# Jim-Maar/Gaussian-Processes-after-pre-processing-with-Normalising-Flows-2

Hardware: NVIDIA B200
Metric: mAR-SCF CIFAR10 MixLogCDF fwd+logdet images/s (higher is better)
Workload: dtype f32

## Files before the change

gaussian-processes-after-pre-processing-with-normalising-flows-2_b200/_lib.py:

```python
import ctypes
import os
import re

_HERE = os.path.dirname(os.path.abspath(__file__))
LIB_PATH = os.path.join(_HERE, "libflowk.so")
HEADER_PATH = os.path.join(os.path.dirname(_HERE), "include", "flowk.h")

FLOWK_OK = 0
FLOWK_ERR_SHAPE = 1
FLOWK_ERR_ALIGN = 2
FLOWK_ERR_ARG = 3
FLOWK_ERR_CUDA_BASE = 1000

_fp = ctypes.c_void_p
_i = ctypes.c_int
_f = ctypes.c_float
_st = ctypes.c_void_p

SIGNATURES = {
    "flowk_abi_version": ([], _i),
    "flowk_error_string": ([_i], ctypes.c_char_p),
    "flowk_ldj_workspace_bytes": ([_i], ctypes.c_size_t),
    "flowk_squeeze2d": ([_fp, _fp, _i, _i, _i, _i, _i, _st], _i),
    "flowk_unsqueeze2d": ([_fp, _fp, _i, _i, _i, _i, _i, _st], _i),
    "flowk_actnorm_init": ([_fp, _fp, _fp, _i, _i, _i, _f, _f, _st], _i),
    "flowk_channel_scale": ([_fp, _fp, _fp, _fp, _fp, _fp, _fp, _fp, _i, _i, _i, _st], _i),
    "flowk_channel_mix": ([_fp, _fp, _fp, _fp, _fp, _fp, _fp, _i, _i, _i, _i, _i, _i, _st], _i),
    "flowk_affine_coupling_fwd": ([_fp, _fp, _fp, _fp, _fp, _fp, _i, _i, _i, _st], _i),
    "flowk_affine_coupling_inv": ([_fp, _fp, _fp, _fp, _fp, _fp, _i, _i, _i, _st], _i),
    "flowk_affine_coupling_bwd": ([_fp, _fp, _fp, _fp, _fp, _fp, _i, _i, _i, _st], _i),
    "flowk_mixlogcdf_fwd": ([_fp, _fp, _fp, _fp, _fp, _fp, _fp, _i, _i, _i, _i, _i, _st], _i),
    "flowk_mixlogcdf_inv": ([_fp, _fp, _fp, _fp, _fp, _fp, _fp, _i, _i, _i, _i, _i, _st], _i),
    "flowk_mixlogcdf_bwd": ([_fp, _fp, _fp, _fp, _fp, _fp, _fp, _fp, _i, _i, _i, _i, _i, _st], _i),
    "flowk_mixture_log_cdf": ([_fp, _fp, _fp, _fp, _fp, _i, _i, _i, _st], _i),
    "flowk_mixture_log_pdf": ([_fp, _fp, _fp, _fp, _fp, _i, _i, _i, _st], _i),
    "flowk_mixture_inv_cdf": ([_fp, _fp, _fp, _fp, _fp, _i, _i, _i, _st], _i),
    "flowk_conv_gemm": ([ctypes.c_void_p, _st], _i),
    "flowk_nchw_to_nhwc_hilo": ([_fp, ctypes.c_longlong, _i, _i, _i, _i, _fp, _fp, _st], _i),
    "flowk_split_hilo": ([_fp, _fp, _fp, ctypes.c_longlong, _st], _i),
    "flowk_nchw_to_nhwc_hilo_f16": ([_fp, ctypes.c_longlong, _i, _i, _i, _i, _fp, _fp, _st], _i),
    "flowk_split_hilo_f16": ([_fp, _fp, _fp, ctypes.c_longlong, ctypes.c_float, _st], _i),
    "flowk_attention_f16": ([_fp, _fp, _fp, _i, _i, _i, _i, _st], _i),
    "flowk_std_normal_logp": ([_fp, ctypes.c_longlong, _fp, _fp, _i, ctypes.c_longlong, _st], _i),
    "flowk_pack_weight_f16": ([_fp, _fp, _i, ctypes.c_float, _fp, _fp, _i, _i, _i, _i, _fp, _fp, _fp, _st], _i),
    "flowk_fold_actnorm_invconv": ([_fp] * 7 + [_i, _i, _i, _i, _fp, _fp, _fp, _st], _i),
    "flowk_patch_attention": ([_fp, _fp, _fp, _fp, _fp, _fp, _i, _i, _i, _i, _i, _i, _st], _i),
    "flowk_patch_attention_train_fwd": ([_fp] * 7 + [_i] * 5 + [_st], _i),
    "flowk_patch_attention_bwd": ([_fp] * 8 + [_i] * 5 + [_st], _i),
    "flowk_attention_tc": ([_fp, _fp, _fp, _i, _i, _i, _i, _i, _fp, _fp, _st], _i),
    "flowk_attention_tc_v2": ([_fp, _fp, _fp, _i, _i, _i, _i, _i, _fp, _fp, _st], _i),
    "flowk_attention_tc_v2_occupancy": ([_i, _i, _i, ctypes.POINTER(ctypes.c_int), ctypes.POINTER(ctypes.c_int)], _i),
    "flowk_attention_inproj_tc": ([_fp, _fp, _fp, _fp, _f, _fp, _fp, _i, _i, _i, _i, _fp, _fp, _st], _i),
    "flowk_attention_inproj_tc_occupancy": ([_i, _i, _i, ctypes.POINTER(ctypes.c_int), ctypes.POINTER(ctypes.c_int)], _i),
    "flowk_attention": ([_fp, _fp, _fp, _i, _i, _i, _i, _st], _i),
    "flowk_concat_elu_fwd": ([_fp, _fp, _fp, ctypes.c_longlong, _i, ctypes.c_longlong, _st], _i),
    "flowk_concat_elu_bwd": ([_fp, _fp, _fp, _fp, ctypes.c_longlong, _i, ctypes.c_longlong, _st], _i),
    "flowk_glu_fwd": ([_fp, _fp, ctypes.c_longlong, _i, ctypes.c_longlong, _st], _i),
    "flowk_weight_norm_operands": ([_fp, _fp, _i, _i, _i, _i, _i, _fp, _fp, _fp, _fp, _fp, _fp, _st], _i),
    "flowk_weight_norm_operands_batched": ([_fp, _i, _i, _st], _i),
    "flowk_weight_norm_bwd": ([_fp, _fp, _fp, _fp, _fp, _fp, _i, _i, _st], _i),
    "flowk_add_layernorm_workspace_bytes": ([ctypes.c_longlong, _i], ctypes.c_longlong),
    "flowk_add_layernorm_fwd": ([_fp, _fp, _fp, _fp, _fp, _fp, _fp, _fp, ctypes.c_longlong, _i, _i, _i, _i,
                                 ctypes.c_float, _st], _i),
    "flowk_add_layernorm_bwd": ([_fp, _fp, _fp, _fp, _fp, _fp, _fp, _fp, _fp, ctypes.c_longlong, _i, _i, _i, _i, _st], _i),
    "flowk_channel_sum_workspace_bytes": ([_i], ctypes.c_longlong),
    "flowk_channel_sum": ([_fp, _fp, _fp, ctypes.c_longlong, _i, ctypes.c_longlong, _st], _i),
    "flowk_conv_wgrad_splits": ([_i, _i, _i, _i, _i, _i, ctypes.POINTER(ctypes.c_int)], _i),
    "flowk_conv_wgrad": ([_fp, _fp, _fp, _fp, _fp, _fp, _i, _i, _i, _i, _i, _i, _st], _i),
    "flowk_linear_wgrad_splits": ([ctypes.c_longlong, _i, _i, ctypes.POINTER(ctypes.c_int)], _i),
    "flowk_linear_wgrad": ([_fp, _fp, _fp, _fp, ctypes.c_longlong, _i, _i, _st], _i),
    "flowk_shift_columns": ([_fp, _fp, _fp, ctypes.c_longlong, _i, _st], _i),
    "flowk_weight_norm_bwd_partials": ([_fp, _fp, _fp, _fp, _fp, _fp, _i, _i, _i, _i, _i, _st], _i),
    "flowk_conv_gemm_splitk_slices": ([_fp], _i),
    "flowk_attention_train_fwd": ([_fp, _fp, _fp, _fp, ctypes.c_uint, ctypes.c_float, _i, _i, _i, _i, _st], _i),
    "flowk_attention_train_bwd": ([_i, _fp, _fp, _fp, _fp, _fp, _fp, ctypes.c_uint, ctypes.c_float, _i, _i, _i, _i, _st], _i),
    "flowk_attention_dropout_mask": ([_fp, ctypes.c_uint, ctypes.c_float, _i, _i, _fp, _st], _i),
    "flowk_adamax_step": ([_fp, _i, _fp, ctypes.c_float, ctypes.c_float, ctypes.c_float, _st], _i),
    "flowk_glu_bwd": ([_fp, _fp, _fp, ctypes.c_longlong, _i, ctypes.c_longlong, _st], _i),
    "flowk_mar_step": ([ctypes.c_void_p, _st], _i),
}


class ConvGemmArgs(ctypes.Structure):
    _fields_ = [(n, ctypes.c_void_p) for n in
                ("a_hi", "a_lo", "w_hi", "w_lo", "bias", "res", "gamma", "beta", "pos",
                 "out_f32", "out_hi", "out_lo", "out_nchw", "status", "trace")] + \
               [(n, ctypes.c_int) for n in ("B", "H", "W", "Cin", "N", "taps", "pre", "out_mask")] + \
               [(n, ctypes.c_void_p) for n in ("w2_hi", "w2_lo", "out2_f32")] + [("N2", ctypes.c_int)] + \
               [("splitk_ws", ctypes.c_void_p), ("operand_format", ctypes.c_int), ("acc_scale", ctypes.c_float),
                ("dilation", ctypes.c_int), ("acc_scale2", ctypes.c_float), ("acc_scale_ptr", ctypes.c_void_p)]


class MarStepArgs(ctypes.Structure):
    _fields_ = [(n, ctypes.c_void_p) for n in ("a_hi", "a_lo", "w_hi", "w_lo", "bias", "dst0_hi", "dst0_lo", "dst1_hi",
                                                "dst1_lo", "c", "noise", "z")] + \
               [("z_stride", ctypes.c_longlong), ("status", ctypes.c_void_p)] + \
               [(n, ctypes.c_int) for n in ("mode", "B", "H", "W", "Cin", "taps", "dilation", "hid", "dst0_pitch",
                                            "dst0_col", "dst1_pitch", "dst1_col")] + [("acc_scale", ctypes.c_float)]


class WnJob(ctypes.Structure):
    _fields_ = [(n, ctypes.c_void_p) for n in ("v", "g", "norm", "w", "fwd_hi", "fwd_lo", "dg_hi", "dg_lo")] + \
               [(n, ctypes.c_int) for n in ("N", "cin", "taps", "cin_pad", "n_pad", "fwd_f16")]


class AdamaxChunk(ctypes.Structure):
    _fields_ = [(n, ctypes.c_void_p) for n in ("p", "g", "m", "u")] + [("n", ctypes.c_longlong)]


OPERAND_TF32, OPERAND_F16 = 0, 1
PRE_BIAS, PRE_GLU_RES_LN, PRE_LSTM = 0, 1, 2
MAR_EMBED, MAR_LSTM, MAR_SAMPLE = 0, 1, 2
PACK_PLAIN, PACK_WEIGHT_NORM, PACK_EXP_GAIN = 0, 1, 2
OUT_F32, OUT_HILO, OUT_HILO_POS, OUT_HILO_CELU, OUT_NCHW, OUT_HILO_RELU = 1, 2, 4, 8, 16, 32


DIMS = {
    "flowk_squeeze2d": slice(2, 6), "flowk_unsqueeze2d": slice(2, 6), "flowk_actnorm_init": slice(3, 6),
    "flowk_channel_scale": slice(8, 11), "flowk_channel_mix": slice(7, 11),
    "flowk_affine_coupling_fwd": slice(6, 9), "flowk_affine_coupling_inv": slice(6, 9),
    "flowk_affine_coupling_bwd": slice(6, 9),
    "flowk_mixlogcdf_fwd": slice(7, 10), "flowk_mixlogcdf_inv": slice(7, 10), "flowk_mixlogcdf_bwd": slice(8, 11),
    "flowk_mixture_log_cdf": slice(5, 8), "flowk_mixture_log_pdf": slice(5, 8), "flowk_mixture_inv_cdf": slice(5, 8),
    "flowk_nchw_to_nhwc_hilo": slice(2, 6), "flowk_split_hilo": slice(3, 4), "flowk_attention": slice(3, 7),
    "flowk_nchw_to_nhwc_hilo_f16": slice(2, 6), "flowk_split_hilo_f16": slice(3, 4), "flowk_attention_f16": slice(3, 7),
    "flowk_attention_tc": slice(4, 8), "flowk_attention_tc_v2": slice(4, 8), "flowk_attention_inproj_tc": slice(7, 11),
    "flowk_patch_attention": slice(6, 10),
    "flowk_patch_attention_train_fwd": slice(7, 11), "flowk_patch_attention_bwd": slice(8, 12),
    "flowk_pack_weight_f16": slice(6, 10), "flowk_fold_actnorm_invconv": slice(7, 11),
}


def declared_symbols(header_path=HEADER_PATH):
    with open(header_path) as f:
        text = re.sub(r"/\*.*?\*/", "", f.read(), flags=re.S)
    return sorted(set(re.findall(r"\b(flowk_[a-z0-9_]+)\s*\(", text)))


def _load():
    if not os.path.exists(LIB_PATH):
        raise ImportError(
            "libflowk.so not found at %s - the CUDA extension is the product and there is no fallback; "
            "build it with `python __graft_entry__.py build`" % LIB_PATH)
    import torch
    lib = ctypes.CDLL(LIB_PATH)
    for name, (argtypes, restype) in SIGNATURES.items():
        fn = getattr(lib, name)
        fn.argtypes = argtypes
        fn.restype = restype
    return lib


lib = _load()

GENERATION = 0


def bump_generation():
    global GENERATION
    GENERATION += 1


def check_device(t, what="flowk"):
    import torch
    if t.is_cuda and t.device.index != torch.cuda.current_device():
        raise RuntimeError("%s: tensor lives on %s but the current CUDA device is cuda:%d; select the tensor's device "
                           "first (torch.cuda.set_device or `with torch.cuda.device(t.device)`)"
                           % (what, t.device, torch.cuda.current_device()))


ALLOW_LIBRARY = os.environ.get("FLOWK_ALLOW_LIBRARY", "0") == "1"
LIBRARY_FALLBACKS = 0


def library_fallback(what, t=None):
    global LIBRARY_FALLBACKS
    if t is not None and (not t.is_cuda or t.dtype != torch_float32()):
        return
    if not ALLOW_LIBRARY:
        raise RuntimeError("flowk: %s has no flowk kernel for this shape/mode and would fall back to a library kernel; "
                           "set FLOWK_ALLOW_LIBRARY=1 to allow it" % what)
    LIBRARY_FALLBACKS += 1


def torch_float32():
    import torch
    return torch.float32


def param_key(params):
    return (GENERATION,) + tuple((p.data_ptr(), p._version) for p in params)

LAUNCHES = 0
TIMING = None


def check(status, what=""):
    if status == FLOWK_OK:
        return
    msg = "%s: %s (flowk status %d)" % (what, lib.flowk_error_string(status).decode(), status)
    if status == FLOWK_ERR_SHAPE:
        raise AssertionError(msg)
    raise RuntimeError(msg)


def call(name, *args, meta=None):
    global LAUNCHES
    LAUNCHES += 1
    if TIMING is None:
        check(getattr(lib, name)(*args), name)
        return
    import torch
    start, end = torch.cuda.Event(enable_timing=True), torch.cuda.Event(enable_timing=True)
    start.record()
    status = getattr(lib, name)(*args)
    end.record()
    check(status, name)
    TIMING.setdefault(name, []).append((start, end, meta if meta is not None else tuple(args[DIMS.get(name, slice(0, 0))])))
```

gaussian-processes-after-pre-processing-with-normalising-flows-2_b200/csrc/attention_tc.cu:

```cuda
#include <cuda.h>
#include "common.cuh"
#include "umma.cuh"

namespace flowk {
namespace tc {

constexpr int ATT_THREADS = 512;
constexpr int ROW_B = 128;

__device__ __forceinline__ uint32_t sw_off(int r, int chunk) { return (uint32_t)(r * ROW_B + ((chunk ^ (r & 7)) << 4)); }

__device__ __forceinline__ uint32_t pack_h2(float a, float b) {
  uint32_t r;
  asm("cvt.rn.f16x2.f32 %0, %1, %2;" : "=r"(r) : "f"(b), "f"(a));
  return r;
}
__device__ __forceinline__ void unpack_h2(uint32_t v, float& a, float& b) {
  unsigned short lo16 = (unsigned short)(v & 0xffffu), hi16 = (unsigned short)(v >> 16);
  asm("cvt.f32.f16 %0, %1;" : "=f"(a) : "h"(lo16));
  asm("cvt.f32.f16 %0, %1;" : "=f"(b) : "h"(hi16));
}
__device__ __forceinline__ void cvt8(const float* v, uint4& hi, uint4& lo) {
  uint32_t h[4], l[4];
#pragma unroll
// ... 362 lines not shown
    const int kb = key >> 6, kk = key & 63;
    uint8_t* tile = v_t + (size_t)kb * vt_tile;
#pragma unroll
    for (int jj = 0; jj < 8; ++jj) {
      const int dim = ch * 8 + jj;
      unsigned short hh, ll;
      split_f16(v[jj], hh, ll);
      *reinterpret_cast<unsigned short*>(tile + sw_off(dim, kk >> 3) + ((kk & 7) << 1)) = hh;
      *reinterpret_cast<unsigned short*>(tile + sw_off(DK + dim, kk >> 3) + ((kk & 7) << 1)) = ll;
    }
  };
  if constexpr (INPROJ) {
    constexpr int STAGE_B = pj_stage_bytes(HW);
    const int nsl = p.kslices;
    const uint32_t leader = warp == 0 ? elect_one() : 0u;
    auto load_slice = [&](int ks) {
      uint8_t* st = smem + (ks & 1) * STAGE_B;
      uint64_t* bar = &bar_full[ks & 1];
      mbar_expect_tx(bar, (uint32_t)STAGE_B);
      tma_load_2d(st, &map_p_hi, bar, ks * 32, b * HW);
      tma_load_2d(st + HW * V2_ROW_B, &map_p_lo, bar, ks * 32, b * HW);
#pragma unroll
      for (int g = 0; g < 3; ++g) {
        tma_load_2d(st + 2 * HW * V2_ROW_B + g * 32 * V2_ROW_B, &map_w_hi, bar, ks * 32, g * C + h * D);
        tma_load_2d(st + 2 * HW * V2_ROW_B + PJ_W_B + g * 32 * V2_ROW_B, &map_w_lo, bar, ks * 32, g * C + h * D);
      }
    };
    if (warp == 0) {
      if (leader) {
        load_slice(0);
        if (nsl > 1) load_slice(1);
      }
      const uint32_t idesc = make_idesc_f16(PJ_N);
      for (int ks = 0; ks < nsl; ++ks) {
        mbar_wait(&bar_full[ks & 1], (uint32_t)((ks >> 1) & 1), failed);
        tc_fence_after();
        const uint8_t* st = smem + (ks & 1) * STAGE_B;
        const uint64_t dw_hi = make_smem_desc_sw64(smem_u32(st + 2 * HW * V2_ROW_B));
        const uint64_t dw_lo = make_smem_desc_sw64(smem_u32(st + 2 * HW * V2_ROW_B + PJ_W_B));
#pragma unroll
        for (int t = 0; t < tiles; ++t) {
          const uint64_t dp_hi = make_smem_desc_sw64(smem_u32(st + t * 128 * V2_ROW_B));
          const uint64_t dp_lo = make_smem_desc_sw64(smem_u32(st + (HW + t * 128) * V2_ROW_B));
          const uint32_t d = tmem_base + (uint32_t)(t * PJ_N);
#pragma unroll
          for (int k = 0; k < 2; ++k) {
            const uint64_t ko = (uint64_t)(k * 2);
            umma_elect<true>(d, dp_hi + ko, dw_hi + ko, idesc, (ks | k) == 0 ? 0u : 1u, leader);
            umma_elect<true>(d, dp_lo + ko, dw_hi + ko, idesc, 1u, leader);
            umma_elect<true>(d, dp_hi + ko, dw_lo + ko, idesc, 1u, leader);
          }
        }
        umma_commit_elect(&bar_empty[ks & 1], leader);
        if (ks >= 1 && ks + 1 < nsl) {
          mbar_wait(&bar_empty[(ks + 1) & 1], (uint32_t)(((ks - 1) >> 1) & 1), failed);
          if (leader) load_slice(ks + 1);
        }
      }
      umma_commit_elect(&bar_proj, leader);
    }
    mbar_wait(&bar_proj, 0, failed);
    tc_fence_after();
    if (tracing) p.trace[1] = clock64();
    const int lane_grp = warp & 3, ch = warp >> 2;
    const int row = lane_grp * 32 + lane;
    const uint32_t lane_addr = tmem_base + ((uint32_t)(lane_grp * 32) << 16);
    const float sc = p.acc_scale;
#pragma unroll 1
    for (int t = 0; t < tiles; ++t) {
      const uint32_t col = lane_addr + (uint32_t)(t * PJ_N + ch * 8);
      const int key = t * 128 + row;
      float v[8];
      uint4 hi, lo;
      if (ch < chunks) {
        tmem_ld8(col, v);
#pragma unroll
        for (int i = 0; i < 8; ++i) v[i] *= sc;
      } else {
#pragma unroll
        for (int i = 0; i < 8; ++i) v[i] = 0.f;
      }
      cvt8(v, hi, lo);
      *reinterpret_cast<uint4*>(k_hi + sw64_off(key, ch)) = hi;
      *reinterpret_cast<uint4*>(k_lo + sw64_off(key, ch)) = lo;
      if (ch < chunks) {
        tmem_ld8(col + 64, v);
#pragma unroll
        for (int i = 0; i < 8; ++i) v[i] = v[i] * sc * p.qscale;
      }
      cvt8(v, hi, lo);
      *reinterpret_cast<uint4*>(q_t + t * V2_QTILE_B + sw64_off(row, ch)) = hi;
      *reinterpret_cast<uint4*>(q_t + t * V2_QTILE_B + 128 * V2_ROW_B + sw64_off(row, ch)) = lo;
      if (ch < chunks) {
        tmem_ld8(col + 32, v);
#pragma unroll
        for (int i = 0; i < 8; ++i) v[i] *= sc;
      }
      store_vt(key, ch, v);
    }
    tc_fence_before();
  } else {
    const float* base = p.qkv + (size_t)b * HW * row_stride + h * D;
    const int nk = HW * KCH, total = 3 * nk;
    constexpr int MAXI = 3;
    for (int i0 = threadIdx.x; i0 < total; i0 += MAXI * V2_THREADS) {
      float4 a[MAXI], c[MAXI];
#pragma unroll
      for (int u = 0; u < MAXI; ++u) {
        const int i = i0 + u * V2_THREADS;
        a[u] = c[u] = make_float4(0.f, 0.f, 0.f, 0.f);
        if (i < total) {
          int r, ch, col;
          if (i < nk) { r = i / KCH; ch = i % KCH; col = 2 * C; }
          else if (i < 2 * nk) { r = (i - nk) / KCH; ch = (i - nk) % KCH; col = 0; }
          else { r = (i - 2 * nk) & (HW - 1); ch = (i - 2 * nk) >> hw_shift; col = C; }
          if (ch < chunks) {
            const float4* g = reinterpret_cast<const float4*>(base + (size_t)r * row_stride + col + ch * 8);
            a[u] = __ldg(g);
            c[u] = __ldg(g + 1);
          }
        }
      }
#pragma unroll
      for (int u = 0; u < MAXI; ++u) {
        const int i = i0 + u * V2_THREADS;
        if (i >= total) continue;
        if (i < 2 * nk) {
          const bool isq = i < nk;
          const int j = isq ? i : i - nk;
          const int r = j / KCH, ch = j % KCH;
          const float sc = isq ? p.qscale : 1.f;
          const float v[8] = {a[u].x * sc, a[u].y * sc, a[u].z * sc, a[u].w * sc, c[u].x * sc, c[u].y * sc, c[u].z * sc, c[u].w * sc};
          uint4 hi, lo;
          cvt8(v, hi, lo);
          uint8_t* dst_hi = isq ? q_t + (r >> 7) * V2_QTILE_B : k_hi;
          uint8_t* dst_lo = isq ? dst_hi + 128 * V2_ROW_B : k_lo;
          const int rr = isq ? (r & 127) : r;
          *reinterpret_cast<uint4*>(dst_hi + sw64_off(rr, ch)) = hi;
          *reinterpret_cast<uint4*>(dst_lo + sw64_off(rr, ch)) = lo;
        } else {
          const int j = i - 2 * nk, key = j & (HW - 1), ch = j >> hw_shift;
          const float v[8] = {a[u].x, a[u].y, a[u].z, a[u].w, c[u].x, c[u].y, c[u].z, c[u].w};
          store_vt(key, ch, v);
        }
      }
    }
  }
  fence_proxy_async();
  __syncthreads();
  if (tracing) p.trace[TR + 1] = clock64();

  const uint32_t leader = warp == 0 ? elect_one() : 0u;
  const int lane_grp = warp & 3, quarter = warp >> 2;
  const int row = lane_grp * 32 + lane;
  const uint32_t lane_addr = tmem_base + ((uint32_t)(lane_grp * 32) << 16);
  auto o_col = [&](int t, int kb) { return (uint32_t)(128 + (t * tiles + kb) * DK); };

  auto issue_s = [&](int t, int kb) {
    tc_fence_after();
    const uint32_t idesc = make_idesc_f16(128);
    const uint64_t dq_hi = make_smem_desc_sw64(smem_u32(q_t + t * V2_QTILE_B));
    const uint64_t dq_lo = make_smem_desc_sw64(smem_u32(q_t + t * V2_QTILE_B + 128 * V2_ROW_B));
    const uint64_t dk_hi = make_smem_desc_sw64(smem_u32(k_hi + kb * 128 * V2_ROW_B));
    const uint64_t dk_lo = make_smem_desc_sw64(smem_u32(k_lo + kb * 128 * V2_ROW_B));
#pragma unroll
    for (int ks = 0; ks < DK / 16; ++ks) {
      const uint64_t ko = (uint64_t)(ks * 2);
      umma_elect<true>(tmem_base, dq_hi + ko, dk_hi + ko, idesc, ks == 0 ? 0u : 1u, leader);
      umma_elect<true>(tmem_base, dq_lo + ko, dk_hi + ko, idesc, 1u, leader);
      umma_elect<true>(tmem_base, dq_hi + ko, dk_lo + ko, idesc, 1u, leader);
    }
    umma_commit_elect(&bar_s, leader);
  };

  if (warp == 0) issue_s(0, 0);
  int it = 0;
#pragma unroll 1
  for (int t = 0; t < tiles; ++t) {
    float m0 = 0.f, m1 = 0.f, l0 = 0.f, l1 = 0.f;
    for (int kb = 0; kb < tiles; ++kb, ++it) {
      mbar_wait(&bar_s, (uint32_t)(it & 1), failed);
      tc_fence_after();
      if (tracing && it == 0) p.trace[TR + 2] = clock64();
      float s[32];
      tmem_ld32(lane_addr + (uint32_t)(quarter * 32), s);
      float mx = s[0];
#pragma unroll
      for (int i = 1; i < 32; ++i) mx = fmaxf(mx, s[i]);
      red_max[quarter][row] = mx;
      tc_fence_before();
      __syncthreads();
      tc_fence_after();
      if (tracing && it == 0) p.trace[TR + 3] = clock64();
      mx = fmaxf(fmaxf(red_max[0][row], red_max[1][row]), fmaxf(red_max[2][row], red_max[3][row]));
      float sum = 0.f;
#pragma unroll
      for (int half = 0; half < 2; ++half) {
        uint32_t ph[8], pl[8];
#pragma unroll
        for (int i = 0; i < 8; ++i) {
          const float e0 = ex2_fast(s[16 * half + 2 * i] - mx), e1 = ex2_fast(s[16 * half + 2 * i + 1] - mx);
          sum += e0 + e1;
          ph[i] = pack_h2(e0, e1);
          float a0, a1;
          unpack_h2(ph[i], a0, a1);
          pl[i] = pack_h2(e0 - a0, e1 - a1);
        }
        tmem_st8u(lane_addr + (uint32_t)(quarter * 16 + half * 8), ph);
        tmem_st8u(lane_addr + (uint32_t)(64 + quarter * 16 + half * 8), pl);
      }
      red_sum[quarter][row] = sum;
      asm volatile("tcgen05.wait::st.sync.aligned;" ::: "memory");
      tc_fence_before();
      __syncthreads();
      if (tracing && it == 0) p.trace[TR + 4] = clock64();
      const float l = (red_sum[0][row] + red_sum[1][row]) + (red_sum[2][row] + red_sum[3][row]);
      if (kb == 0) { m0 = mx; l0 = l; }
      else { m1 = mx; l1 = l; }

      if (warp == 0) {
        tc_fence_after();
        const uint32_t idesc = make_idesc_f16(DK);
        const uint32_t d = tmem_base + o_col(t, kb);
#pragma unroll
        for (int j = 0; j < 8; ++j) {
          const int key = kb * 128 + j * 16;
          const uint8_t* vb = v_t + (size_t)(key >> 6) * vt_tile;
          const uint64_t ko = (uint64_t)(((key & 63) >> 4) * 2);
          const uint64_t dv_hi = make_smem_desc(smem_u32(vb)) + ko, dv_lo = make_smem_desc(smem_u32(vb + DK * ROW_B)) + ko;
          const uint32_t a_hi = tmem_base + (uint32_t)(j * 8), a_lo = tmem_base + (uint32_t)(64 + j * 8);
          umma_f16_ts_elect(d, a_hi, dv_hi, idesc, j == 0 ? 0u : 1u, leader);
          umma_f16_ts_elect(d, a_lo, dv_hi, idesc, 1u, leader);
          umma_f16_ts_elect(d, a_hi, dv_lo, idesc, 1u, leader);
        }
        umma_commit_elect(&bar_o, leader);
        const int nt = kb + 1 < tiles ? t : t + 1, nkb = kb + 1 < tiles ? kb + 1 : 0;
        if (nt < tiles) {
          mbar_wait(&bar_o, (uint32_t)(it & 1), failed);
          issue_s(nt, nkb);
        }
      }
    }
    if (tracing && t == tiles - 1) p.trace[TR + 5] = clock64();

    mbar_wait(&bar_o, (uint32_t)((it - 1) & 1), failed);
    tc_fence_after();
    float w0 = 1.f, w1 = 0.f;
    if (tiles == 2) {
      const float m = fmaxf(m0, m1);
      w0 = ex2_fast(m0 - m);
      w1 = ex2_fast(m1 - m);
    }
    const float inv = 1.0f / (l0 * w0 + l1 * w1);
    w0 *= inv;
    w1 *= inv;
    const int q0 = t * 128;
    const size_t out0 = (size_t)(cta_index() / p.heads) * HW * C + (size_t)(cta_index() % p.heads) * D;
    const size_t o0 = out0 + (size_t)(q0 + row) * C;
    uint8_t* stage = q_t + t * V2_QTILE_B;
    for (int ch = quarter; ch < chunks; ch += 4) {
      float a[8], c[8];
      tmem_ld8(lane_addr + o_col(t, 0) + ch * 8, a);
      if (tiles == 2) tmem_ld8(lane_addr + o_col(t, 1) + ch * 8, c);
      else {
#pragma unroll
        for (int i = 0; i < 8; ++i) c[i] = 0.f;
      }
#pragma unroll
      for (int i = 0; i < 8; ++i) c[i] = a[i] * w0 + c[i] * w1;
      if (p.out_f16) {
        uint4 hi, lo;
        cvt8(c, hi, lo);
        *reinterpret_cast<uint4*>(stage + ((size_t)row * chunks + ch) * 16) = hi;
        *reinterpret_cast<uint4*>(stage + ((size_t)(128 + row) * chunks + ch) * 16) = lo;
      } else {
#pragma unroll
        for (int i = 0; i < 8; i += 2) store_pair(p.out_hi, p.out_lo, o0 + ch * 8 + i, c[i], c[i + 1], 0);
      }
    }
    if (p.out_f16) {
      __syncthreads();
      const int items = 2 * 128 * chunks;
      for (int i = threadIdx.x; i < items; i += V2_THREADS) {
        const int mat = i / (128 * chunks), rr = (i / chunks) % 128, ch = i % chunks;
        const uint4 v = *reinterpret_cast<const uint4*>(stage + (size_t)i * 16);
        unsigned short* dst = reinterpret_cast<unsigned short*>(mat ? p.out_lo : p.out_hi);
        *reinterpret_cast<uint4*>(dst + out0 + (size_t)(q0 + rr) * C + ch * 8) = v;
      }
    }
  }
  tc_fence_before();
  __syncthreads();
  if (tracing) p.trace[TR + 6] = clock64();
  if (warp == 0) tmem_dealloc(tmem_base, (uint32_t)V2_TMEM_COLS);
  if (threadIdx.x == 0 && failed_flag && p.status) *p.status = 1;
}

}
}

using namespace flowk;
using namespace flowk::tc;

extern "C" int flowk_attention_tc(const float* qkv, void* out_hi, void* out_lo, int out_f16, int B, int HW, int C, int heads,
                                  int* status, long long* trace, flowk_stream_t stream) {
  if (B < 0 || HW < 1 || C < 1 || heads < 1 || C % heads) return FLOWK_ERR_SHAPE;
  const int D = C / heads;
  if ((HW != 128 && HW != 256) || D % 8 || D > 64 || C % 4) return FLOWK_ERR_SHAPE;
  if (B == 0) return FLOWK_OK;
  if (!qkv || !out_hi || !out_lo) return FLOWK_ERR_ARG;
  if ((long long)B * heads > 0x7fffffffLL) return FLOWK_ERR_SHAPE;
  AttParams p{};
  p.qkv = qkv;
  p.out_hi = reinterpret_cast<float*>(out_hi);
  p.out_lo = reinterpret_cast<float*>(out_lo);
  p.out_f16 = out_f16;
  p.HW = HW;
  p.C = C;
  p.heads = heads;
  p.D = D;
  p.dk = (D + 15) / 16 * 16;
  p.qscale = 1.4426950408889634f / sqrtf((float)D);
  p.status = status;
  p.trace = trace;
  const int p_bytes = 2 * (HW / 64) * 128 * ROW_B;
  const int qk_bytes = 2 * HW * ROW_B + 2 * HW * ROW_B;
  const int first = p_bytes > qk_bytes ? p_bytes : qk_bytes;
  p.p_off = 0;
  p.q_off = 0;
  p.k_off = 2 * HW * ROW_B;
  p.v_off = first;
  p.o_off = first + 2 * (HW / 64) * p.dk * ROW_B;
  const size_t smem = (size_t)p.o_off + (size_t)2 * 128 * (D / 8) * 16 + 1024;
  if (smem + 8 * 1024 > 227 * 1024) return FLOWK_ERR_SHAPE;
#define FLOWK_LAUNCH_ATT(KCH_)                                                                                          \
  do {                                                                                                                 \
    static size_t smem_set = 0;                                                                                        \
    if (smem > smem_set) {                                                                                             \
      FLOWK_CUDA_OK(cudaFuncSetAttribute(attention_tc_kernel<KCH_>, cudaFuncAttributeMaxDynamicSharedMemorySize, (int)smem)); \
      smem_set = smem;                                                                                                 \
    }                                                                                                                  \
    FLOWK_CUDA_OK(launch_pdl(attention_tc_kernel<KCH_>, dim3(B * heads), dim3(ATT_THREADS), smem, stream, p));          \
  } while (0)
  switch (p.dk >> 3) {
    case 2: FLOWK_LAUNCH_ATT(2); break;
    case 4: FLOWK_LAUNCH_ATT(4); break;
    case 6: FLOWK_LAUNCH_ATT(6); break;
    default: FLOWK_LAUNCH_ATT(8); break;
  }
#undef FLOWK_LAUNCH_ATT
  return launch_status();
}

namespace {
bool attention_tc_v2_plan(int HW, int C, int heads, bool inproj, AttParams& p, size_t& smem) {
  if (HW != 128 && HW != 256) return false;
  if (heads < 1 || C < 1 || C % heads) return false;
  const int D = C / heads;
  if (D != 24 && D != 32) return false;
  p.HW = HW;
  p.C = C;
  p.heads = heads;
  p.D = D;
  p.dk = (D + 15) / 16 * 16;
  p.qscale = 1.4426950408889634f / sqrtf((float)D);
  p.q_off = 0;
  p.k_off = (HW / 128) * V2_QTILE_B;
  p.v_off = p.k_off + 2 * HW * V2_ROW_B;
  p.kslices = (C + 31) / 32;
  size_t bytes = (size_t)p.v_off + (size_t)2 * (HW / 64) * p.dk * ROW_B;
  if (inproj && (size_t)2 * pj_stage_bytes(HW) > bytes) bytes = (size_t)2 * pj_stage_bytes(HW);
  smem = bytes + 1024;
  return true;
}

template <int KCH, int TILES, bool INPROJ>
cudaError_t attention_tc_v2_prepare(size_t smem) {
  static size_t smem_set = 0;
  if (smem > smem_set) {
    cudaError_t e = cudaFuncSetAttribute(attention_tc_v2_kernel<KCH, TILES, INPROJ>,
                                         cudaFuncAttributeMaxDynamicSharedMemorySize, (int)smem);
    if (e != cudaSuccess) return e;
    e = cudaFuncSetAttribute(attention_tc_v2_kernel<KCH, TILES, INPROJ>, cudaFuncAttributePreferredSharedMemoryCarveout,
                             (int)cudaSharedmemCarveoutMaxShared);
    if (e != cudaSuccess) return e;
    smem_set = smem;
  }
  return cudaSuccess;
}

template <bool INPROJ>
int attention_tc_v2_launch(const AttParams& p, int B, size_t smem, const CUtensorMap* maps, cudaStream_t stream) {
#define FLOWK_LAUNCH_ATT_V2(KCH_, TILES_)                                                                             \
  do {                                                                                                                 \
    FLOWK_CUDA_OK((attention_tc_v2_prepare<KCH_, TILES_, INPROJ>(smem)));                                               \
    FLOWK_CUDA_OK(launch_pdl(attention_tc_v2_kernel<KCH_, TILES_, INPROJ>, dim3(B * p.heads), dim3(V2_THREADS), smem,    \
                             stream, p, maps[0], maps[1], maps[2], maps[3]));                                          \
  } while (0)
  if (p.HW == 256) FLOWK_LAUNCH_ATT_V2(4, 2);
  else FLOWK_LAUNCH_ATT_V2(4, 1);
#undef FLOWK_LAUNCH_ATT_V2
  return launch_status();
}

bool make_map_sw64(CUtensorMap* map, const void* base, long long rows, long long cols, int box_rows) {
  if (!encode_fn()) return false;
  cuuint64_t dims[2] = {(cuuint64_t)cols, (cuuint64_t)rows};
  cuuint64_t strides[1] = {(cuuint64_t)cols * 2};
  cuuint32_t box[2] = {32u, (cuuint32_t)box_rows};
  cuuint32_t estr[2] = {1, 1};
  return encode_fn()(map, CU_TENSOR_MAP_DATA_TYPE_FLOAT16, 2, const_cast<void*>(base), dims, strides, box, estr,
                     CU_TENSOR_MAP_INTERLEAVE_NONE, CU_TENSOR_MAP_SWIZZLE_64B, CU_TENSOR_MAP_L2_PROMOTION_L2_256B,
                     CU_TENSOR_MAP_FLOAT_OOB_FILL_NONE) == CUDA_SUCCESS;
}
}

extern "C" int flowk_attention_tc_v2(const float* qkv, void* out_hi, void* out_lo, int out_f16, int B, int HW, int C,
                                     int heads, int* status, long long* trace, flowk_stream_t stream) {
  AttParams p{};
  size_t smem = 0;
  if (B < 0 || !attention_tc_v2_plan(HW, C, heads, false, p, smem)) return FLOWK_ERR_SHAPE;
  if (B == 0) return FLOWK_OK;
  if (!qkv || !out_hi || !out_lo) return FLOWK_ERR_ARG;
  if ((long long)B * heads > 0x7fffffffLL) return FLOWK_ERR_SHAPE;
  p.qkv = qkv;
  p.out_hi = reinterpret_cast<float*>(out_hi);
  p.out_lo = reinterpret_cast<float*>(out_lo);
  p.out_f16 = out_f16;
  p.status = status;
  p.trace = trace;
  const CUtensorMap unused[4] = {};
  return attention_tc_v2_launch<false>(p, B, smem, unused, stream);
}

extern "C" int flowk_attention_inproj_tc(const void* p_hi, const void* p_lo, const void* w_hi, const void* w_lo,
                                         float acc_scale, void* out_hi, void* out_lo, int B, int HW, int C, int heads,
                                         int* status, long long* trace, flowk_stream_t stream) {
  AttParams p{};
  size_t smem = 0;
  if (B < 0 || !attention_tc_v2_plan(HW, C, heads, true, p, smem)) return FLOWK_ERR_SHAPE;
  if (B == 0) return FLOWK_OK;
  if (!p_hi || !p_lo || !w_hi || !w_lo || !out_hi || !out_lo || !(acc_scale > 0.f)) return FLOWK_ERR_ARG;
  if (!aligned16(p_hi) || !aligned16(p_lo) || !aligned16(w_hi) || !aligned16(w_lo)) return FLOWK_ERR_ALIGN;
  if ((long long)B * HW > 0x7fffffffLL) return FLOWK_ERR_SHAPE;
  p.out_hi = reinterpret_cast<float*>(out_hi);
  p.out_lo = reinterpret_cast<float*>(out_lo);
  p.out_f16 = 1;
  p.acc_scale = acc_scale;
  p.status = status;
  p.trace = trace;
  const long long rows = (long long)B * HW, kw = (C + 63) / 64 * 64;
  CUtensorMap maps[4];
  if (!make_map_sw64(&maps[0], p_hi, rows, C, HW) || !make_map_sw64(&maps[1], p_lo, rows, C, HW) ||
      !make_map_sw64(&maps[2], w_hi, 3LL * C, kw, 32) || !make_map_sw64(&maps[3], w_lo, 3LL * C, kw, 32))
    return FLOWK_ERR_ARG;
  return attention_tc_v2_launch<true>(p, B, smem, maps, stream);
}

namespace {
template <int KCH, int TILES, bool INPROJ>
int attention_tc_v2_fit(size_t smem, int* blocks_per_sm) {
  FLOWK_CUDA_OK((attention_tc_v2_prepare<KCH, TILES, INPROJ>(smem)));
  cudaFuncAttributes fa;
  FLOWK_CUDA_OK(cudaFuncGetAttributes(&fa, attention_tc_v2_kernel<KCH, TILES, INPROJ>));
  int dev = 0, regs_sm = 0, smem_sm = 0, reserved = 0, threads_sm = 0;
  FLOWK_CUDA_OK(cudaGetDevice(&dev));
  FLOWK_CUDA_OK(cudaDeviceGetAttribute(&regs_sm, cudaDevAttrMaxRegistersPerMultiprocessor, dev));
  FLOWK_CUDA_OK(cudaDeviceGetAttribute(&smem_sm, cudaDevAttrMaxSharedMemoryPerMultiprocessor, dev));
  FLOWK_CUDA_OK(cudaDeviceGetAttribute(&reserved, cudaDevAttrReservedSharedMemoryPerBlock, dev));
  FLOWK_CUDA_OK(cudaDeviceGetAttribute(&threads_sm, cudaDevAttrMaxThreadsPerMultiProcessor, dev));
  const int warp_regs = (fa.numRegs * 32 + 255) / 256 * 256;
  const int by_regs = regs_sm / (warp_regs * (V2_THREADS / 32));
  const int by_smem = smem_sm / (int)(smem + fa.sharedSizeBytes + (size_t)reserved);
  const int by_threads = threads_sm / V2_THREADS;
  *blocks_per_sm = by_regs < by_smem ? (by_regs < by_threads ? by_regs : by_threads) : (by_smem < by_threads ? by_smem : by_threads);
  return FLOWK_OK;
}

template <bool INPROJ>
int attention_tc_v2_occupancy(int HW, int C, int heads, int* blocks_per_sm, int* smem_bytes) {
  AttParams p{};
  size_t smem = 0;
  if (!attention_tc_v2_plan(HW, C, heads, INPROJ, p, smem)) return FLOWK_ERR_SHAPE;
  if (!blocks_per_sm) return FLOWK_ERR_ARG;
  if (smem_bytes) *smem_bytes = (int)smem;
  return HW == 256 ? attention_tc_v2_fit<4, 2, INPROJ>(smem, blocks_per_sm) : attention_tc_v2_fit<4, 1, INPROJ>(smem, blocks_per_sm);
}
}

extern "C" int flowk_attention_tc_v2_occupancy(int HW, int C, int heads, int* blocks_per_sm, int* smem_bytes) {
  return attention_tc_v2_occupancy<false>(HW, C, heads, blocks_per_sm, smem_bytes);
}

extern "C" int flowk_attention_inproj_tc_occupancy(int HW, int C, int heads, int* blocks_per_sm, int* smem_bytes) {
  return attention_tc_v2_occupancy<true>(HW, C, heads, blocks_per_sm, smem_bytes);
}
```

gaussian-processes-after-pre-processing-with-normalising-flows-2_b200/csrc/common.cuh:

```cuda
#pragma once
#include <cuda_runtime.h>
#include <stdint.h>
#include "flowk.h"

namespace flowk {

constexpr int kMaxParts = 64;
constexpr int kThreads = 128;

#define FLOWK_CUDA_OK(expr)                                          \
  do {                                                               \
    cudaError_t e_ = (expr);                                         \
    if (e_ != cudaSuccess) return FLOWK_ERR_CUDA_BASE + (int)e_;     \
  } while (0)

inline int launch_status() {
  cudaError_t e = cudaGetLastError();
  return e == cudaSuccess ? FLOWK_OK : FLOWK_ERR_CUDA_BASE + (int)e;
}

inline bool aligned16(const void* p) { return (reinterpret_cast<uintptr_t>(p) & 15u) == 0; }
inline bool aligned4(const void* p) { return (reinterpret_cast<uintptr_t>(p) & 3u) == 0; }

constexpr int kSlotWords = kMaxParts + 1;
struct LdjWs {
  unsigned* base;
  __host__ __device__ unsigned* ticket(int b) const { return base + (size_t)b * kSlotWords; }
  __host__ __device__ float* partial(int b) const { return reinterpret_cast<float*>(base + (size_t)b * kSlotWords + 1); }
};
inline LdjWs carve_ws(void* ws, int ) {
  LdjWs w;
  w.base = reinterpret_cast<unsigned*>(ws);
  return w;
}

__device__ __forceinline__ float warp_sum(float v) {
#pragma unroll
  for (int o = 16; o > 0; o >>= 1) v += __shfl_xor_sync(0xffffffffu, v, o);
  return v;
}

__device__ __forceinline__ float ld_stream(const float* p) { return __ldcs(p); }
__device__ __forceinline__ float4 ld_stream4(const float* p) { return __ldcs(reinterpret_cast<const float4*>(p)); }
__device__ __forceinline__ void st_stream4(float* p, float4 v) { __stcs(reinterpret_cast<float4*>(p), v); }

__device__ __forceinline__ float ex2_fast(float x) {
  float y;
  asm("ex2.approx.ftz.f32 %0, %1;" : "=f"(y) : "f"(x));
  return y;
}
__device__ __forceinline__ float rcp_fast(float x) {
  float y;
  asm("rcp.approx.ftz.f32 %0, %1;" : "=f"(y) : "f"(x));
  return y;
}
__device__ __forceinline__ void split_f16(float x, unsigned short& hi, unsigned short& lo) {
  unsigned short h, l;
  asm("cvt.rn.satfinite.f16.f32 %0, %1;" : "=h"(h) : "f"(x));
  float hf;
  asm("cvt.f32.f16 %0, %1;" : "=f"(hf) : "h"(h));
  asm("cvt.rn.satfinite.f16.f32 %0, %1;" : "=h"(l) : "f"(x - hf));
  hi = h;
  lo = l;
}
__device__ __forceinline__ void store_pair(float* out_hi, float* out_lo, size_t off, float v0, float v1, int out_f16) {
  if (out_f16) {
    unsigned short h0, l0, h1, l1;
    split_f16(v0, h0, l0);
    split_f16(v1, h1, l1);
    *reinterpret_cast<uint32_t*>(reinterpret_cast<unsigned short*>(out_hi) + off) = (uint32_t)h0 | ((uint32_t)h1 << 16);
    *reinterpret_cast<uint32_t*>(reinterpret_cast<unsigned short*>(out_lo) + off) = (uint32_t)l0 | ((uint32_t)l1 << 16);
  } else {
    const float a0 = __uint_as_float((__float_as_uint(v0) + 0x1000u) & 0xffffe000u);
    const float a1 = __uint_as_float((__float_as_uint(v1) + 0x1000u) & 0xffffe000u);
    const float b0 = __uint_as_float((__float_as_uint(v0 - a0) + 0x1000u) & 0xffffe000u);
    const float b1 = __uint_as_float((__float_as_uint(v1 - a1) + 0x1000u) & 0xffffe000u);
    *reinterpret_cast<float2*>(out_hi + off) = make_float2(a0, a1);
    *reinterpret_cast<float2*>(out_lo + off) = make_float2(b0, b1);
  }
}

constexpr float kLog2e = 1.4426950408889634f;
constexpr float kLn2 = 0.6931471805599453f;

template <int THREADS>
__device__ __forceinline__ void finish_sample_ldj(float local, const float* __restrict__ ldj_in,
                                                  float* __restrict__ ldj_out, float sign, LdjWs ws) {
  __shared__ float warp_part[THREADS / 32];
  __shared__ bool is_last;
  const int b = blockIdx.y, part = blockIdx.x, parts = gridDim.x;
  local = warp_sum(local);
  if ((threadIdx.x & 31) == 0) warp_part[threadIdx.x >> 5] = local;
  __syncthreads();
  if (threadIdx.x == 0) {
    float s = 0.f;
#pragma unroll
    for (int w = 0; w < THREADS / 32; ++w) s += warp_part[w];
    if (parts == 1) {
      ldj_out[b] = (ldj_in ? ldj_in[b] : 0.f) + sign * s;
      is_last = false;
    } else {
      __stcg(ws.partial(b) + part, s);
      __threadfence();
      unsigned ticket = atomicAdd(ws.ticket(b), 1u);
      is_last = (ticket == (unsigned)parts - 1u);
    }
  }
  __syncthreads();
  if (is_last && threadIdx.x == 0) {
    __threadfence();
    float tot = 0.f;
    for (int p = 0; p < parts; ++p) tot += __ldcg(ws.partial(b) + p);
    ldj_out[b] = (ldj_in ? ldj_in[b] : 0.f) + sign * tot;
    *ws.ticket(b) = 0u;
  }
}

__device__ __forceinline__ void griddep_wait() { asm volatile("griddepcontrol.wait;" ::: "memory"); }
__device__ __forceinline__ void griddep_launch() { asm volatile("griddepcontrol.launch_dependents;" ::: "memory"); }

template <typename... KArgs, typename... Args>
inline cudaError_t launch_pdl(void (*kernel)(KArgs...), dim3 grid, dim3 block, size_t smem, cudaStream_t stream,
                              Args... args) {
  cudaLaunchConfig_t cfg = {};
  cfg.gridDim = grid;
  cfg.blockDim = block;
  cfg.dynamicSmemBytes = smem;
  cfg.stream = stream;
  cudaLaunchAttribute attr[1];
  attr[0].id = cudaLaunchAttributeProgrammaticStreamSerialization;
  attr[0].val.programmaticStreamSerializationAllowed = 1;
  cfg.attrs = attr;
  cfg.numAttrs = 1;
  return cudaLaunchKernelEx(&cfg, kernel, static_cast<KArgs>(args)...);
}

template <typename... KArgs, typename... Args>
inline cudaError_t launch_pdl_cluster(void (*kernel)(KArgs...), dim3 grid, dim3 block, size_t smem, cudaStream_t stream,
                                      int cluster_x, Args... args) {
  cudaLaunchConfig_t cfg = {};
  cfg.gridDim = grid;
  cfg.blockDim = block;
  cfg.dynamicSmemBytes = smem;
  cfg.stream = stream;
  cudaLaunchAttribute attr[2];
  attr[0].id = cudaLaunchAttributeProgrammaticStreamSerialization;
  attr[0].val.programmaticStreamSerializationAllowed = 1;
  cfg.numAttrs = 1;
  if (cluster_x > 1) {
    attr[1].id = cudaLaunchAttributeClusterDimension;
    attr[1].val.clusterDim.x = (unsigned)cluster_x;
    attr[1].val.clusterDim.y = 1;
    attr[1].val.clusterDim.z = 1;
    cfg.numAttrs = 2;
  }
  cfg.attrs = attr;
  return cudaLaunchKernelEx(&cfg, kernel, static_cast<KArgs>(args)...);
}

inline int parts_for(long long work_items, int per_cta) {
  long long p = (work_items + per_cta - 1) / per_cta;
  if (p < 1) p = 1;
  if (p > kMaxParts) p = kMaxParts;
  return (int)p;
}

}
```

gaussian-processes-after-pre-processing-with-normalising-flows-2_b200/csrc/tc_gemm.cu:

```cuda
#include <cuda.h>
#include <stdlib.h>
#include "common.cuh"
#include "umma.cuh"

namespace flowk {
namespace tc {

constexpr int ROW_BYTES = 128;
constexpr int A_TILE_BYTES = BLOCK_M * ROW_BYTES;
constexpr int EPI_WARPS = 16;
constexpr int NUM_THREADS = 64 + 32 * EPI_WARPS;
constexpr int MAX_CHUNKS = 2;

__device__ __forceinline__ float elu1(float x) { return x > 0.f ? x : ex2_fast(x * kLog2e) - 1.f; }
__device__ __forceinline__ float sigmoid_fast(float x) { return __fdividef(1.f, 1.f + ex2_fast(-x * kLog2e)); }

enum { PRE_BIAS = 0, PRE_GLU_RES_LN = 1, PRE_LSTM = 2 };
enum { PRE_MAR_EMBED = 3, PRE_MAR_LSTM = 4, PRE_MAR_SAMPLE = 5 };
enum { OUT_F32 = 1, OUT_HILO = 2, OUT_HILO_POS = 4, OUT_HILO_CELU = 8, OUT_NCHW = 16, OUT_HILO_RELU = 32 };

struct Params {
  int M, N, HW, W, H;
  int taps, kblocks_per_tap;
  int ksz, dil;
  int wt, ht, bt;
  int n_chunk, n_chunks;
  int tmem_cols, stages;
  int bar_offset;
  int dxsplit, a_slots, w_slots;
  int pair, w_unit, pair_nmma;
  int pre, out_mask;
  const float* bias;
  const float* res;
  const float* gamma;
  const float* beta;
  const float* pos;
  float* out_f32;
  float* out_hi;
  float* out_lo;
  float* out_nchw;
  int chain, n2, n2_chunk, n2_chunks, a3_offset, w2_offset;
  float* out2_f32;
  float acc_scale;
  float acc_scale2;
  const float* acc_scale_ptr;
  int ksplit;
  int* status;
  long long* trace;
  void* dst_hi[2];
  void* dst_lo[2];
  int dst_pitch[2], dst_col[2];
  float* cell;
  const float* noise;
  float* z;
  long long z_stride;
};

template <int PRE, int NV, bool F16, bool PAIR = false>
__global__ void __launch_bounds__(NUM_THREADS, 1)
conv_gemm_kernel(const __grid_constant__ CUtensorMap map_a_hi, const __grid_constant__ CUtensorMap map_a_lo,
                 const __grid_constant__ CUtensorMap map_w_hi, const __grid_constant__ CUtensorMap map_w_lo,
                 const __grid_constant__ CUtensorMap map_w2_hi, const __grid_constant__ CUtensorMap map_w2_lo,
                 const Params p) {
  extern __shared__ __align__(1024) uint8_t smem_raw[];
  uint8_t* smem = reinterpret_cast<uint8_t*>((reinterpret_cast<uintptr_t>(smem_raw) + 1023) & ~(uintptr_t)1023);
  constexpr int BK = F16 ? 64 : BLOCK_K;
  const int w_tile_bytes = p.n_chunk * p.n_chunks * ROW_BYTES;
  const int stage_bytes = 2 * A_TILE_BYTES + 2 * w_tile_bytes;
  uint64_t* full_bar = reinterpret_cast<uint64_t*>(smem + p.bar_offset);
  uint64_t* empty_bar = full_bar + (p.dxsplit ? p.a_slots : p.stages);
  uint64_t* wfull_bar = empty_bar + p.a_slots;
  uint64_t* wempty_bar = wfull_bar + p.w_slots;
  uint64_t* tmem_full_bar = p.dxsplit ? wempty_bar + p.w_slots : empty_bar + p.stages;
  uint64_t* a3_full_bar = tmem_full_bar + 1;
  uint64_t* w2_full_bar = tmem_full_bar + 2;
  uint64_t* w2_empty_bar = tmem_full_bar + 3;
  uint64_t* acc2_full_bar = tmem_full_bar + 4;
  uint32_t* tmem_slot = reinterpret_cast<uint32_t*>(tmem_full_bar + 5);
  volatile int* failed = reinterpret_cast<volatile int*>(tmem_slot + 1);

  const int warp = threadIdx.x >> 5, lane = threadIdx.x & 31;
  const int m_tile = blockIdx.x, n_tile = blockIdx.y;
  const int n_base = n_tile * p.n_chunk * p.n_chunks;
  const int ksp = p.ksplit > 1 ? p.ksplit : 1;
  const int cb0 = (int)((long long)p.kblocks_per_tap * blockIdx.z / ksp);
  const int kpt = (int)((long long)p.kblocks_per_tap * (blockIdx.z + 1) / ksp) - cb0;
  const int num_kb = p.taps * kpt;
  float* const out_f32 = p.out_f32 ? p.out_f32 + (size_t)blockIdx.z * p.M * p.N : nullptr;

  if (threadIdx.x == 0) {
    *failed = 0;
    if (p.dxsplit) {
      for (int s = 0; s < p.a_slots; ++s) { mbar_init(&full_bar[s], 1); mbar_init(&empty_bar[s], 1); }
      for (int s = 0; s < p.w_slots; ++s) { mbar_init(&wfull_bar[s], 1); mbar_init(&wempty_bar[s], 1); }
    } else {
      for (int s = 0; s < p.stages; ++s) { mbar_init(&full_bar[s], 1); mbar_init(&empty_bar[s], 1); }
    }
    mbar_init(tmem_full_bar, 1);
    mbar_init(a3_full_bar, EPI_WARPS);
    mbar_init(w2_full_bar, 1);
    mbar_init(w2_empty_bar, 1);
    mbar_init(acc2_full_bar, 1);
    fence_barrier_init();
    prefetch_tmap(&map_a_hi);
    prefetch_tmap(&map_a_lo);
    prefetch_tmap(&map_w_hi);
    prefetch_tmap(&map_w_lo);
  }
  const uint32_t cta_rank = PAIR ? cluster_ctarank() : 0u;
  if (warp == 1) {
    if (PAIR) tmem_alloc_pair(tmem_slot, (uint32_t)p.tmem_cols);
    else tmem_alloc(tmem_slot, (uint32_t)p.tmem_cols);
  }
  tc_fence_before();
  if (PAIR) cluster_sync_all();
  else __syncthreads();
  tc_fence_after();
  const uint32_t tmem_base = *tmem_slot;
  const bool tracing = p.trace && blockIdx.x == 0 && blockIdx.y == 0;
  if (tracing && threadIdx.x == 0) p.trace[0] = clock64();
  griddep_launch();

  if (warp == 0) {
    if (lane == 0) {
      const int tiles_per_img = (p.H * p.W) / (p.ht * p.wt);
      int b0, h0;
      if (p.bt > 1) { b0 = m_tile * p.bt; h0 = 0; }
      else { b0 = m_tile / tiles_per_img; h0 = (m_tile % tiles_per_img) * p.ht; }
      griddep_wait();
      if (PAIR && p.dxsplit) {
        uint8_t* w_ring = smem + (size_t)p.a_slots * 2 * A_TILE_BYTES;
        const int groups = 3 * p.kblocks_per_tap;
        const int n_total = 3 * p.n_chunk;
        int n_mma = (n_total + 255) / 256;
        if ((n_total / n_mma) % 16 || n_total % n_mma) n_mma = 3;
        if (p.pair_nmma) n_mma = p.pair_nmma;
        const int half = n_total / n_mma / 2;
        const int lo_off = (n_total / 2) * ROW_BYTES;
        for (int g = 0; g < groups; ++g) {
          const int dyi = g / p.kblocks_per_tap, cb = g % p.kblocks_per_tap;
          const int sa = g % p.a_slots;
          mbar_wait(&empty_bar[sa], (((uint32_t)(g / p.a_slots)) & 1u) ^ 1u, failed);
          uint8_t* at = smem + (size_t)sa * 2 * A_TILE_BYTES;
          const uint32_t afull = mapa_rank(&full_bar[sa], 0);
          if (cta_rank == 0) mbar_expect_tx(&full_bar[sa], 4u * A_TILE_BYTES);
          tma_load_4d_pair(at, &map_a_hi, afull, cb * BK, 0, h0 + dyi - 1, b0);
          tma_load_4d_pair(at + A_TILE_BYTES, &map_a_lo, afull, cb * BK, 0, h0 + dyi - 1, b0);
          const int sw = g % p.w_slots;
          mbar_wait(&wempty_bar[sw], (((uint32_t)(g / p.w_slots)) & 1u) ^ 1u, failed);
          uint8_t* wt = w_ring + (size_t)sw * 3 * w_tile_bytes;
          const uint32_t wfull = mapa_rank(&wfull_bar[sw], 0);
          if (cta_rank == 0) mbar_expect_tx(&wfull_bar[sw], 6u * (uint32_t)w_tile_bytes);
          for (int q = 0; q < n_mma; ++q)
            for (int j = 0; j < half; j += p.w_unit) {
              const int r = q * 2 * half + (int)cta_rank * half + j;
              const int dxi = r / p.n_chunk, n = r - dxi * p.n_chunk;
              const int kcol = ((dyi * 3 + dxi) * p.kblocks_per_tap + cb) * BK;
              uint8_t* dst = wt + (size_t)(q * half + j) * ROW_BYTES;
              tma_load_2d_pair(dst, &map_w_hi, wfull, kcol, n_base + n);
              tma_load_2d_pair(dst + lo_off, &map_w_lo, wfull, kcol, n_base + n);
            }
        }
      } else if (p.dxsplit) {
        uint8_t* w_ring = smem + (size_t)p.a_slots * 2 * A_TILE_BYTES;
        const int groups = 3 * p.kblocks_per_tap;
        for (int g = 0; g < groups; ++g) {
          const int dyi = g / p.kblocks_per_tap, cb = g % p.kblocks_per_tap;
          const int sa = g % p.a_slots;
          mbar_wait(&empty_bar[sa], (((uint32_t)(g / p.a_slots)) & 1u) ^ 1u, failed);
          uint8_t* at = smem + (size_t)sa * 2 * A_TILE_BYTES;
          mbar_expect_tx(&full_bar[sa], 2u * A_TILE_BYTES);
          tma_load_4d(at, &map_a_hi, &full_bar[sa], cb * BK, 0, h0 + dyi - 1, b0);
          tma_load_4d(at + A_TILE_BYTES, &map_a_lo, &full_bar[sa], cb * BK, 0, h0 + dyi - 1, b0);
          const int sw = g % p.w_slots;
          mbar_wait(&wempty_bar[sw], (((uint32_t)(g / p.w_slots)) & 1u) ^ 1u, failed);
          uint8_t* wt = w_ring + (size_t)sw * 6 * w_tile_bytes;
          mbar_expect_tx(&wfull_bar[sw], 6u * (uint32_t)w_tile_bytes);
          for (int dxi = 0; dxi < 3; ++dxi) {
            const int kcol = ((dyi * 3 + dxi) * p.kblocks_per_tap + cb) * BK;
            tma_load_2d(wt + dxi * w_tile_bytes, &map_w_hi, &wfull_bar[sw], kcol, n_base);
            tma_load_2d(wt + (3 + dxi) * w_tile_bytes, &map_w_lo, &wfull_bar[sw], kcol, n_base);
          }
        }
      } else
      for (int kb = 0; kb < num_kb; ++kb) {
        const int s = kb % p.stages;
        const uint32_t ph = (uint32_t)(kb / p.stages) & 1u;
        mbar_wait(&empty_bar[s], ph ^ 1u, failed);
        uint8_t* st = smem + (size_t)s * stage_bytes;
        const int tap = kb / kpt, cb = cb0 + kb % kpt;
        const int dy = (tap / p.ksz - (p.ksz >> 1)) * p.dil, dx = (tap % p.ksz - (p.ksz >> 1)) * p.dil;
        mbar_expect_tx(&full_bar[s], (uint32_t)stage_bytes);
        tma_load_4d(st, &map_a_hi, &full_bar[s], cb * BK, dx, h0 + dy, b0);
        tma_load_4d(st + A_TILE_BYTES, &map_a_lo, &full_bar[s], cb * BK, dx, h0 + dy, b0);
        const int kcol = (tap * p.kblocks_per_tap + cb) * BK;
        for (int c = 0; c < p.n_chunks; ++c) {
          const int chunk_bytes = p.n_chunk * ROW_BYTES;
          tma_load_2d(st + 2 * A_TILE_BYTES + c * chunk_bytes, &map_w_hi, &full_bar[s], kcol, n_base + c * p.n_chunk);
          tma_load_2d(st + 2 * A_TILE_BYTES + w_tile_bytes + c * chunk_bytes, &map_w_lo, &full_bar[s], kcol,
                      n_base + c * p.n_chunk);
        }
      }
      if (p.chain) {
        mbar_wait(tmem_full_bar, 0, failed);
        const int w2_chunk_bytes = p.n2_chunk * ROW_BYTES, w2_half = w2_chunk_bytes * p.n2_chunks;
        const int kb2 = ((p.N >> 1) + BK - 1) / BK;
        for (int kb = 0; kb < kb2; ++kb) {
          mbar_wait(w2_empty_bar, ((uint32_t)kb & 1u) ^ 1u, failed);
          mbar_expect_tx(w2_full_bar, 2u * (uint32_t)w2_half);
          for (int c = 0; c < p.n2_chunks; ++c) {
            tma_load_2d(smem + p.w2_offset + c * w2_chunk_bytes, &map_w2_hi, w2_full_bar, kb * BK, c * p.n2_chunk);
            tma_load_2d(smem + p.w2_offset + w2_half + c * w2_chunk_bytes, &map_w2_lo, w2_full_bar, kb * BK,
                        c * p.n2_chunk);
          }
        }
      }
    }
  } else if (warp == 1) {
    const uint32_t leader = elect_one();
    {
      const uint32_t idesc = make_idesc_t<F16>(p.n_chunk);
      if (PAIR && p.dxsplit) {
        if (cta_rank == 0) {
          const uint32_t w_ring = smem_u32(smem + (size_t)p.a_slots * 2 * A_TILE_BYTES);
          const int groups = 3 * p.kblocks_per_tap;
          const int n_total = 3 * p.n_chunk;
          int n_mma = (n_total + 255) / 256;
          if ((n_total / n_mma) % 16 || n_total % n_mma) n_mma = 3;
          if (p.pair_nmma) n_mma = p.pair_nmma;
          const int n_per = n_total / n_mma;
          const uint32_t idesc_w = make_idesc_f16_pair(n_per);
          const uint64_t per_units = (uint64_t)((uint32_t)((n_per / 2) * ROW_BYTES) >> 4);
          const uint64_t lo_units = (uint64_t)((uint32_t)((n_total / 2) * ROW_BYTES) >> 4);
          for (int g = 0; g < groups; ++g) {
            const int sa = g % p.a_slots, sw = g % p.w_slots;
            mbar_wait(&full_bar[sa], ((uint32_t)(g / p.a_slots)) & 1u, failed);
            mbar_wait(&wfull_bar[sw], ((uint32_t)(g / p.w_slots)) & 1u, failed);
            tc_fence_after();
            if (tracing && lane == 0 && g == 0) p.trace[1] = clock64();
            if (tracing && lane == 0 && g == groups - 1) p.trace[2] = clock64();
            const uint32_t a_hi = smem_u32(smem + (size_t)sa * 2 * A_TILE_BYTES);
            const uint32_t w_hi = w_ring + (uint32_t)sw * 3u * (uint32_t)w_tile_bytes;
            const uint64_t da_hi = make_smem_desc(a_hi), da_lo = da_hi + (A_TILE_BYTES >> 4);
            const uint64_t db_hi = make_smem_desc(w_hi), db_lo = db_hi + lo_units;
#pragma unroll
            for (int k = 0; k < 4; ++k) {
              const uint64_t ko = (uint64_t)(k * 2);
              for (int q = 0; q < n_mma; ++q) {
                const uint64_t bo = ko + q * per_units;
                const uint32_t d = tmem_base + q * n_per;
                umma_f16_pair_elect(d, da_hi + ko, db_hi + bo, idesc_w, (g | k) == 0 ? 0u : 1u, leader);
                umma_f16_pair_elect(d, da_lo + ko, db_hi + bo, idesc_w, 1u, leader);
                umma_f16_pair_elect(d, da_hi + ko, db_lo + bo, idesc_w, 1u, leader);
              }
            }
            umma_commit_pair_elect(&wempty_bar[sw], leader);
            umma_commit_pair_elect(&empty_bar[sa], leader);
          }
          umma_commit_pair_elect(tmem_full_bar, leader);
        }
      } else if (p.dxsplit) {
        const uint32_t w_ring = smem_u32(smem + (size_t)p.a_slots * 2 * A_TILE_BYTES);
        const int groups = 3 * p.kblocks_per_tap;
        const int n_total = 3 * p.n_chunk;
        int n_mma = (n_total + 255) / 256;
        if ((n_total / n_mma) % 16 || n_total % n_mma) n_mma = 3;
        const int n_per = n_total / n_mma;
        const uint32_t idesc_w = make_idesc_t<F16>(n_per);
        const uint64_t per_units = (uint64_t)((uint32_t)(n_per * ROW_BYTES) >> 4);
        for (int g = 0; g < groups; ++g) {
          const int sa = g % p.a_slots, sw = g % p.w_slots;
          mbar_wait(&full_bar[sa], ((uint32_t)(g / p.a_slots)) & 1u, failed);
          mbar_wait(&wfull_bar[sw], ((uint32_t)(g / p.w_slots)) & 1u, failed);
          tc_fence_after();
          if (tracing && lane == 0 && g == 0) p.trace[1] = clock64();
          if (tracing && lane == 0 && g == groups - 1) p.trace[2] = clock64();
          const uint32_t a_hi = smem_u32(smem + (size_t)sa * 2 * A_TILE_BYTES);
          const uint32_t w_hi = w_ring + (uint32_t)sw * 6u * (uint32_t)w_tile_bytes;
          const uint64_t da_hi = make_smem_desc(a_hi), da_lo = da_hi + (A_TILE_BYTES >> 4);
          const uint64_t db_hi = make_smem_desc(w_hi), db_lo = db_hi + ((3u * (uint32_t)w_tile_bytes) >> 4);
#pragma unroll
          for (int k = 0; k < 4; ++k) {
            const uint64_t ko = (uint64_t)(k * 2);
            for (int q = 0; q < n_mma; ++q) {
              const uint64_t bo = ko + q * per_units;
              const uint32_t d = tmem_base + q * n_per;
              umma_elect<F16>(d, da_hi + ko, db_hi + bo, idesc_w, (g | k) == 0 ? 0u : 1u, leader);
              umma_elect<F16>(d, da_lo + ko, db_hi + bo, idesc_w, 1u, leader);
              umma_elect<F16>(d, da_hi + ko, db_lo + bo, idesc_w, 1u, leader);
            }
          }
          umma_commit_elect(&wempty_bar[sw], leader);
          umma_commit_elect(&empty_bar[sa], leader);
        }
        umma_commit_elect(tmem_full_bar, leader);
      } else {
      for (int kb = 0; kb < num_kb; ++kb) {
        const int s = kb % p.stages;
        const uint32_t ph = (uint32_t)(kb / p.stages) & 1u;
        mbar_wait(&full_bar[s], ph, failed);
        tc_fence_after();
        if (tracing && lane == 0 && kb == 0) p.trace[1] = clock64();
        if (tracing && lane == 0 && kb == num_kb - 1) p.trace[2] = clock64();
        const uint32_t a_hi = smem_u32(smem + (size_t)s * stage_bytes);
        const uint64_t da_hi0 = make_smem_desc(a_hi), da_lo0 = da_hi0 + (A_TILE_BYTES >> 4);
        const uint64_t db_hi0 = da_hi0 + (2 * A_TILE_BYTES >> 4), db_lo0 = db_hi0 + ((uint32_t)w_tile_bytes >> 4);
        const uint64_t chunk_units = (uint64_t)((uint32_t)(p.n_chunk * ROW_BYTES) >> 4);
#pragma unroll
        for (int k = 0; k < 4; ++k) {
          const uint64_t ko = (uint64_t)(k * 2);
          for (int c = 0; c < p.n_chunks; ++c) {
            const uint64_t co = ko + c * chunk_units;
            const uint32_t d = tmem_base + c * p.n_chunk;
            umma_elect<F16>(d, da_hi0 + ko, db_hi0 + co, idesc, (kb | k) == 0 ? 0u : 1u, leader);
            umma_elect<F16>(d, da_lo0 + ko, db_hi0 + co, idesc, 1u, leader);
            umma_elect<F16>(d, da_hi0 + ko, db_lo0 + co, idesc, 1u, leader);
          }
        }
        umma_commit_elect(&empty_bar[s], leader);
      }
      umma_commit_elect(tmem_full_bar, leader);
      }
      if (p.chain) {
        mbar_wait(a3_full_bar, 0, failed);
        tc_fence_after();
        const uint32_t idesc2 = make_idesc_t<F16>(p.n2_chunk);
        const int kb2 = ((p.N >> 1) + BK - 1) / BK;
        const uint32_t w2_half = (uint32_t)(p.n2_chunk * ROW_BYTES * p.n2_chunks);
        const uint64_t chunk2_units = (uint64_t)((uint32_t)(p.n2_chunk * ROW_BYTES) >> 4);
        for (int kb = 0; kb < kb2; ++kb) {
          mbar_wait(w2_full_bar, (uint32_t)kb & 1u, failed);
          tc_fence_after();
          const uint64_t da_hi = make_smem_desc(smem_u32(smem + p.a3_offset + (size_t)kb * 2 * A_TILE_BYTES));
          const uint64_t da_lo = da_hi + (A_TILE_BYTES >> 4);
          const uint64_t db_hi = make_smem_desc(smem_u32(smem + p.w2_offset)), db_lo = db_hi + (w2_half >> 4);
#pragma unroll
          for (int k = 0; k < 4; ++k) {
            const uint64_t ko = (uint64_t)(k * 2);
            for (int c = 0; c < p.n2_chunks; ++c) {
              const uint64_t co = ko + c * chunk2_units;
              const uint32_t d = tmem_base + p.N + c * p.n2_chunk;
              umma_elect<F16>(d, da_hi + ko, db_hi + co, idesc2, (kb | k) == 0 ? 0u : 1u, leader);
              umma_elect<F16>(d, da_lo + ko, db_hi + co, idesc2, 1u, leader);
              umma_elect<F16>(d, da_hi + ko, db_lo + co, idesc2, 1u, leader);
            }
          }
          umma_commit_elect(w2_empty_bar, leader);
        }
        umma_commit_elect(acc2_full_bar, leader);
      }
    }
  } else {
    const int lane_grp = warp & 3;
    const int sub = (warp - 2) >> 2;
    const int slab_row0 = m_tile * BLOCK_M + lane_grp * 32;
    const uint32_t trow = tmem_base + ((uint32_t)(lane_grp * 32) << 16);
    const int ncols_cta = p.n_chunk * p.n_chunks;
    mbar_wait(tmem_full_bar, 0, failed);
    tc_fence_after();
    const float sc = F16 ? (p.acc_scale_ptr ? __ldg(p.acc_scale_ptr) : p.acc_scale) : 1.f;
    if (tracing && threadIdx.x == 64) p.trace[3] = clock64();

    if (PRE == PRE_BIAS) {
      if (p.out_mask & OUT_NCHW) {
        const int m = slab_row0 + lane;
        const bool valid = m < p.M;
        const int hw = valid ? m % p.HW : 0, img = valid ? m / p.HW : 0;
        for (int j = sub * 16; j < ncols_cta; j += 16 * (EPI_WARPS / 4)) {
          const int n0 = n_base + j;
          if (n0 >= p.N) break;
          float v[16];
          if (p.dxsplit) {
            float vm[16], vp[16];
            tmem_ld16(trow + j, vm);
            tmem_ld16(trow + p.n_chunk + j, v);
            tmem_ld16(trow + 2 * p.n_chunk + j, vp);
            const int wcol = (slab_row0 + lane) % p.W;
            const bool has_l = wcol > 0, has_r = wcol < p.W - 1;
#pragma unroll
            for (int i = 0; i < 16; ++i) {
              const float l = __shfl_up_sync(0xffffffffu, vm[i], 1), r = __shfl_down_sync(0xffffffffu, vp[i], 1);
              v[i] += (has_l ? l : 0.f) + (has_r ? r : 0.f);
            }
          } else {
            tmem_ld16(trow + j, v);
          }
          if (!valid) continue;
          float* o = p.out_nchw + ((size_t)img * p.N + n0) * p.HW + hw;
#pragma unroll
          for (int i = 0; i < 16; ++i)
            if (n0 + i < p.N) o[(size_t)i * p.HW] = fmaf(v[i], sc, p.bias ? __ldg(p.bias + n0 + i) : 0.f);
        }
      }
      if (p.out_mask & (OUT_F32 | OUT_HILO | OUT_HILO_CELU | OUT_HILO_RELU)) {
        const int pitch = ncols_cta + 4;
        float* slab = reinterpret_cast<float*>(smem) + lane_grp * (32 * pitch);
        const int bar_id = 1 + lane_grp;
        for (int j = sub * 16; j < ncols_cta; j += 16 * (EPI_WARPS / 4)) {
          float v[16];
          if (p.dxsplit) {
            float vm[16], vp[16];
            tmem_ld16(trow + j, vm);
            tmem_ld16(trow + p.n_chunk + j, v);
            tmem_ld16(trow + 2 * p.n_chunk + j, vp);
            const int wcol = (slab_row0 + lane) % p.W;
            const bool has_l = wcol > 0, has_r = wcol < p.W - 1;
#pragma unroll
            for (int i = 0; i < 16; ++i) {
              const float l = __shfl_up_sync(0xffffffffu, vm[i], 1), r = __shfl_down_sync(0xffffffffu, vp[i], 1);
              v[i] += (has_l ? l : 0.f) + (has_r ? r : 0.f);
            }
          } else {
            tmem_ld16(trow + j, v);
          }
#pragma unroll
          for (int i = 0; i < 16; i += 4) {
            const int n = n_base + j + i;
            float4 bv = make_float4(0.f, 0.f, 0.f, 0.f);
            if (p.bias && n < p.N) bv = __ldg(reinterpret_cast<const float4*>(p.bias + n));
            *reinterpret_cast<float4*>(slab + lane * pitch + j + i) =
                make_float4(fmaf(v[i], sc, bv.x), fmaf(v[i + 1], sc, bv.y), fmaf(v[i + 2], sc, bv.z), fmaf(v[i + 3], sc, bv.w));
          }
        }
        asm volatile("bar.sync %0, 128;" ::"r"(bar_id) : "memory");
        for (int c4 = lane * 4; c4 < ncols_cta; c4 += 128) {
          const int n = n_base + c4;
          if (n >= p.N) break;
#pragma unroll
          for (int rr = 0; rr < 8; ++rr) {
            const int r = sub * 8 + rr, m = slab_row0 + r;
            if (m >= p.M) break;
            const float4 y = *reinterpret_cast<const float4*>(slab + r * pitch + c4);
            const float ys[4] = {y.x, y.y, y.z, y.w};
            const size_t o = (size_t)m * p.N + n;
            if (p.out_mask & OUT_F32) *reinterpret_cast<float4*>(out_f32 + o) = y;
            if (p.out_mask & (OUT_HILO | OUT_HILO_RELU)) {
              float t[4];
#pragma unroll
              for (int i = 0; i < 4; ++i) t[i] = (p.out_mask & OUT_HILO_RELU) ? fmaxf(ys[i], 0.f) : ys[i];
              store_hilo4<F16>(p.out_hi, p.out_lo, o, t);
            }
            if (p.out_mask & OUT_HILO_CELU) {
              const size_t o2 = (size_t)m * 2 * p.N + n;
              float t[4], t2[4];
#pragma unroll
              for (int i = 0; i < 4; ++i) {
                t[i] = elu1(ys[i]);
                t2[i] = elu1(-ys[i]);
              }
              store_hilo4<F16>(p.out_hi, p.out_lo, o2, t);
              store_hilo4<F16>(p.out_hi, p.out_lo, o2 + p.N, t2);
            }
          }
        }
      }
    } else if (PRE == PRE_LSTM) {
      const int hid = p.N >> 2;
      const int m = slab_row0 + lane;
      if (sub == 0 && m < p.M) {
        const float* gi = p.res + (size_t)m * p.N;
        const float* cp = p.gamma + (size_t)m * hid;
        for (int j = 0; j < hid; j += 8) {
          float acc[4][8];
#pragma unroll
          for (int gte = 0; gte < 4; ++gte) {
            tmem_ld8(trow + gte * hid + j, acc[gte]);
            const float4 g0 = __ldg(reinterpret_cast<const float4*>(gi + gte * hid + j));
            const float4 g1 = __ldg(reinterpret_cast<const float4*>(gi + gte * hid + j + 4));
            const float4 b0 = __ldg(reinterpret_cast<const float4*>(p.bias + gte * hid + j));
            const float4 b1 = __ldg(reinterpret_cast<const float4*>(p.bias + gte * hid + j + 4));
            const float gv[8] = {g0.x, g0.y, g0.z, g0.w, g1.x, g1.y, g1.z, g1.w};
            const float bv[8] = {b0.x, b0.y, b0.z, b0.w, b1.x, b1.y, b1.z, b1.w};
#pragma unroll
            for (int i = 0; i < 8; ++i) acc[gte][i] = fmaf(acc[gte][i], sc, bv[i]) + gv[i];
          }
          const float4 c0 = __ldg(reinterpret_cast<const float4*>(cp + j)), c1 = __ldg(reinterpret_cast<const float4*>(cp + j + 4));
          const float cv[8] = {c0.x, c0.y, c0.z, c0.w, c1.x, c1.y, c1.z, c1.w};
          float cn[8], hn[8];
#pragma unroll
          for (int i = 0; i < 8; ++i) {
            const float ig = 1.f / (1.f + expf(-acc[0][i])), fg = 1.f / (1.f + expf(-acc[1][i]));
            const float gg = tanhf(acc[2][i]), og = 1.f / (1.f + expf(-acc[3][i]));
            cn[i] = fg * cv[i] + ig * gg;
            hn[i] = og * tanhf(cn[i]);
          }
          float* co = out_f32 + (size_t)m * hid + j;
          *reinterpret_cast<float4*>(co) = make_float4(cn[0], cn[1], cn[2], cn[3]);
          *reinterpret_cast<float4*>(co + 4) = make_float4(cn[4], cn[5], cn[6], cn[7]);
          store_hilo4<F16>(p.out_hi, p.out_lo, (size_t)m * hid + j, hn);
          store_hilo4<F16>(p.out_hi, p.out_lo, (size_t)m * hid + j + 4, hn + 4);
        }
      }
    } else if (PRE == PRE_MAR_EMBED || PRE == PRE_MAR_LSTM) {
      const int m = slab_row0 + lane;
      const bool row_ok = m < p.M;
      const int hid = PRE == PRE_MAR_LSTM ? p.N >> 2 : p.N;
      for (int j = sub * 8; j < hid; j += 32) {
        __syncwarp();
        float hn[8];
        if (PRE == PRE_MAR_EMBED) {
          tmem_ld8(trow + j, hn);
#pragma unroll
          for (int i = 0; i < 8; ++i) hn[i] = fmaf(hn[i], sc, __ldg(p.bias + j + i));
        } else {
          float acc[4][8];
#pragma unroll
          for (int gte = 0; gte < 4; ++gte) {
            tmem_ld8(trow + gte * hid + j, acc[gte]);
#pragma unroll
            for (int i = 0; i < 8; ++i) acc[gte][i] = fmaf(acc[gte][i], sc, __ldg(p.bias + gte * hid + j + i));
          }
          if (row_ok) {
            float* cp = p.cell + (size_t)m * hid + j;
            const float4 c0 = *reinterpret_cast<const float4*>(cp), c1 = *reinterpret_cast<const float4*>(cp + 4);
            const float cv[8] = {c0.x, c0.y, c0.z, c0.w, c1.x, c1.y, c1.z, c1.w};
            float cn[8];
#pragma unroll
            for (int i = 0; i < 8; ++i) {
              const float ig = 1.f / (1.f + expf(-acc[0][i])), fg = 1.f / (1.f + expf(-acc[1][i]));
              const float gg = tanhf(acc[2][i]), og = 1.f / (1.f + expf(-acc[3][i]));
              cn[i] = fg * cv[i] + ig * gg;
              hn[i] = og * tanhf(cn[i]);
            }
            *reinterpret_cast<float4*>(cp) = make_float4(cn[0], cn[1], cn[2], cn[3]);
            *reinterpret_cast<float4*>(cp + 4) = make_float4(cn[4], cn[5], cn[6], cn[7]);
          }
        }
        if (row_ok) {
#pragma unroll
          for (int d = 0; d < 2; ++d) {
            if (!p.dst_hi[d]) continue;
            const size_t o = (size_t)m * p.dst_pitch[d] + p.dst_col[d] + j;
            store_hilo4_f16(reinterpret_cast<float*>(p.dst_hi[d]), reinterpret_cast<float*>(p.dst_lo[d]), o, hn);
            store_hilo4_f16(reinterpret_cast<float*>(p.dst_hi[d]), reinterpret_cast<float*>(p.dst_lo[d]), o + 4, hn + 4);
          }
        }
      }
    } else if (PRE == PRE_MAR_SAMPLE) {
      if (sub == 0) {
        float v[8];
        tmem_ld8(trow, v);
        const int m = slab_row0 + lane;
        if (m < p.M) {
          const float mean = fmaf(v[0], sc, __ldg(p.bias)), logs = fmaf(v[1], sc, __ldg(p.bias + 1));
          const float s = __fadd_rn(__fmul_rn(__ldg(p.noise + m), expf(logs)), mean);
          p.z[(size_t)(m / p.HW) * p.z_stride + m % p.HW] = s;
          unsigned short h, l;
          split_f16(s, h, l);
          const size_t o = (size_t)m * p.dst_pitch[0] + p.dst_col[0];
          reinterpret_cast<unsigned short*>(p.dst_hi[0])[o] = h;
          reinterpret_cast<unsigned short*>(p.dst_lo[0])[o] = l;
        }
      }
    } else {
      const int C = p.N >> 1;
      const int pitch = C + 4;
      float* slab = reinterpret_cast<float*>(smem) + lane_grp * (32 * pitch);
      const int bar_id = 1 + lane_grp;
      const int nv = (C + 127) / 128;
      float g[8][NV][4], pe[8][NV][4];
      float mean[8], rstd[8];
      bool normalized = false;
      if (NV == 1) {
        __shared__ float ln_part[2][4][4][32];
        const int m_row = slab_row0 + lane;
        const bool row_ok = m_row < p.M;
        float gb[2][16];
        float psum = 0.f;
#pragma unroll
        for (int ci = 0; ci < 2; ++ci) {
          const int j = sub * 16 + ci * 64;
          if (j < C) {
            float a[16], b[16];
            tmem_ld16(trow + j, a);
            tmem_ld16(trow + C + j, b);
#pragma unroll
            for (int i = 0; i < 16; i += 4) {
              const float4 ba = __ldg(reinterpret_cast<const float4*>(p.bias + j + i));
              const float4 bb = __ldg(reinterpret_cast<const float4*>(p.bias + C + j + i));
              const float4 rs = row_ok ? __ldg(reinterpret_cast<const float4*>(p.res + (size_t)m_row * C + j + i))
                                       : make_float4(0.f, 0.f, 0.f, 0.f);
              gb[ci][i] = fmaf(a[i], sc, ba.x) * sigmoid_fast(fmaf(b[i], sc, bb.x)) + rs.x;
              gb[ci][i + 1] = fmaf(a[i + 1], sc, ba.y) * sigmoid_fast(fmaf(b[i + 1], sc, bb.y)) + rs.y;
              gb[ci][i + 2] = fmaf(a[i + 2], sc, ba.z) * sigmoid_fast(fmaf(b[i + 2], sc, bb.z)) + rs.z;
              gb[ci][i + 3] = fmaf(a[i + 3], sc, ba.w) * sigmoid_fast(fmaf(b[i + 3], sc, bb.w)) + rs.w;
              psum += (gb[ci][i] + gb[ci][i + 1]) + (gb[ci][i + 2] + gb[ci][i + 3]);
            }
          }
        }
        ln_part[0][lane_grp][sub][lane] = psum;
        asm volatile("bar.sync %0, 128;" ::"r"(bar_id) : "memory");
        const float mu = ((ln_part[0][lane_grp][0][lane] + ln_part[0][lane_grp][1][lane]) +
                          (ln_part[0][lane_grp][2][lane] + ln_part[0][lane_grp][3][lane])) / (float)C;
        float pvar = 0.f;
#pragma unroll
        for (int ci = 0; ci < 2; ++ci)
          if (sub * 16 + ci * 64 < C) {
#pragma unroll
            for (int i = 0; i < 16; ++i) pvar = fmaf(gb[ci][i] - mu, gb[ci][i] - mu, pvar);
          }
        ln_part[1][lane_grp][sub][lane] = pvar;
        asm volatile("bar.sync %0, 128;" ::"r"(bar_id) : "memory");
        const float rs_ = rsqrtf(((ln_part[1][lane_grp][0][lane] + ln_part[1][lane_grp][1][lane]) +
                                  (ln_part[1][lane_grp][2][lane] + ln_part[1][lane_grp][3][lane])) / (float)C + 1e-5f);
        if (tracing && threadIdx.x == 64) p.trace[6] = clock64();
#pragma unroll
        for (int ci = 0; ci < 2; ++ci) {
          const int j = sub * 16 + ci * 64;
          if (j < C) {
#pragma unroll
            for (int i = 0; i < 16; i += 4) {
              const float4 ga = __ldg(reinterpret_cast<const float4*>(p.gamma + j + i));
              const float4 be = __ldg(reinterpret_cast<const float4*>(p.beta + j + i));
              *reinterpret_cast<float4*>(slab + lane * pitch + j + i) =
                  make_float4(fmaf((gb[ci][i] - mu) * rs_, ga.x, be.x), fmaf((gb[ci][i + 1] - mu) * rs_, ga.y, be.y),
                              fmaf((gb[ci][i + 2] - mu) * rs_, ga.z, be.z), fmaf((gb[ci][i + 3] - mu) * rs_, ga.w, be.w));
            }
          }
        }
        asm volatile("bar.sync %0, 128;" ::"r"(bar_id) : "memory");
        if (tracing && threadIdx.x == 64) p.trace[7] = clock64();
        normalized = true;
#pragma unroll
        for (int rr = 0; rr < 8; ++rr) {
          const int r = sub * 8 + rr, m = slab_row0 + r;
          const int c4 = lane * 4;
          float4 ps = make_float4(0.f, 0.f, 0.f, 0.f), gv = ps;
          if (c4 < C) {
            gv = *reinterpret_cast<const float4*>(slab + r * pitch + c4);
            if (((p.out_mask & OUT_HILO_POS) || (p.chain && p.pos)) && m < p.M)
              ps = __ldg(reinterpret_cast<const float4*>(p.pos + (size_t)(m % p.HW) * C + c4));
          }
          g[rr][0][0] = gv.x; g[rr][0][1] = gv.y; g[rr][0][2] = gv.z; g[rr][0][3] = gv.w;
          pe[rr][0][0] = ps.x; pe[rr][0][1] = ps.y; pe[rr][0][2] = ps.z; pe[rr][0][3] = ps.w;
          mean[rr] = 0.f;
          rstd[rr] = 1.f;
        }
      } else {
        __shared__ float ln_part2[2][4][4][32];
        const int m_row = slab_row0 + lane;
        const bool row_ok = m_row < p.M;
        float gb[4][16];
        float psum = 0.f;
#pragma unroll
        for (int ci = 0; ci < 4; ++ci) {
          const int j = sub * 16 + ci * 64;
          if (j < C) {
            float a[16], b[16];
            tmem_ld16(trow + j, a);
            tmem_ld16(trow + C + j, b);
#pragma unroll
            for (int i = 0; i < 16; i += 4) {
              const float4 ba = __ldg(reinterpret_cast<const float4*>(p.bias + j + i));
              const float4 bb = __ldg(reinterpret_cast<const float4*>(p.bias + C + j + i));
              const float4 rs = row_ok ? __ldg(reinterpret_cast<const float4*>(p.res + (size_t)m_row * C + j + i))
                                       : make_float4(0.f, 0.f, 0.f, 0.f);
              gb[ci][i] = fmaf(a[i], sc, ba.x) * sigmoid_fast(fmaf(b[i], sc, bb.x)) + rs.x;
              gb[ci][i + 1] = fmaf(a[i + 1], sc, ba.y) * sigmoid_fast(fmaf(b[i + 1], sc, bb.y)) + rs.y;
              gb[ci][i + 2] = fmaf(a[i + 2], sc, ba.z) * sigmoid_fast(fmaf(b[i + 2], sc, bb.z)) + rs.z;
              gb[ci][i + 3] = fmaf(a[i + 3], sc, ba.w) * sigmoid_fast(fmaf(b[i + 3], sc, bb.w)) + rs.w;
              psum += (gb[ci][i] + gb[ci][i + 1]) + (gb[ci][i + 2] + gb[ci][i + 3]);
            }
          }
        }
        ln_part2[0][lane_grp][sub][lane] = psum;
        asm volatile("bar.sync %0, 128;" ::"r"(bar_id) : "memory");
        const float mu = ((ln_part2[0][lane_grp][0][lane] + ln_part2[0][lane_grp][1][lane]) +
                          (ln_part2[0][lane_grp][2][lane] + ln_part2[0][lane_grp][3][lane])) / (float)C;
        float pvar = 0.f;
#pragma unroll
        for (int ci = 0; ci < 4; ++ci)
          if (sub * 16 + ci * 64 < C) {
#pragma unroll
            for (int i = 0; i < 16; ++i) pvar = fmaf(gb[ci][i] - mu, gb[ci][i] - mu, pvar);
          }
        ln_part2[1][lane_grp][sub][lane] = pvar;
        asm volatile("bar.sync %0, 128;" ::"r"(bar_id) : "memory");
        const float rs_ = rsqrtf(((ln_part2[1][lane_grp][0][lane] + ln_part2[1][lane_grp][1][lane]) +
                                  (ln_part2[1][lane_grp][2][lane] + ln_part2[1][lane_grp][3][lane])) / (float)C + 1e-5f);
        if (tracing && threadIdx.x == 64) p.trace[6] = clock64();
#pragma unroll
        for (int ci = 0; ci < 4; ++ci) {
          const int j = sub * 16 + ci * 64;
          if (j < C) {
#pragma unroll
            for (int i = 0; i < 16; i += 4) {
              const float4 ga = __ldg(reinterpret_cast<const float4*>(p.gamma + j + i));
              const float4 be = __ldg(reinterpret_cast<const float4*>(p.beta + j + i));
              *reinterpret_cast<float4*>(slab + lane * pitch + j + i) =
                  make_float4(fmaf((gb[ci][i] - mu) * rs_, ga.x, be.x), fmaf((gb[ci][i + 1] - mu) * rs_, ga.y, be.y),
                              fmaf((gb[ci][i + 2] - mu) * rs_, ga.z, be.z), fmaf((gb[ci][i + 3] - mu) * rs_, ga.w, be.w));
            }
          }
        }
        asm volatile("bar.sync %0, 128;" ::"r"(bar_id) : "memory");
        if (tracing && threadIdx.x == 64) p.trace[7] = clock64();
        normalized = true;
#pragma unroll
        for (int rr = 0; rr < 8; ++rr) {
          mean[rr] = 0.f;
          rstd[rr] = 1.f;
        }
      }
      if (tracing && threadIdx.x == 64) p.trace[8] = clock64();
#pragma unroll
      for (int v = 0; v < NV; ++v) {
        const int c4 = v * 128 + lane * 4;
        if (v >= nv || c4 >= C) {
          if (F16 && p.chain && v < nv && c4 < ((C + 63) & ~63)) {
#pragma unroll
            for (int rr = 0; rr < 8; ++rr) {
              const int R = lane_grp * 32 + sub * 8 + rr;
              uint8_t* t = smem + p.a3_offset + (size_t)(c4 >> 6) * 2 * A_TILE_BYTES + R * 128 + ((((c4 & 63) >> 3) ^ (R & 7)) << 4) +
                           ((c4 & 7) << 1);
              *reinterpret_cast<uint2*>(t) = make_uint2(0u, 0u);
              *reinterpret_cast<uint2*>(t + A_TILE_BYTES) = make_uint2(0u, 0u);
            }
          }
          continue;
        }
        const float4 ga = __ldg(reinterpret_cast<const float4*>(p.gamma + c4));
        const float4 be = __ldg(reinterpret_cast<const float4*>(p.beta + c4));
        const float gs[4] = {ga.x, ga.y, ga.z, ga.w}, bs[4] = {be.x, be.y, be.z, be.w};
#pragma unroll
        for (int rr = 0; rr < 8; ++rr) {
          const int m = slab_row0 + sub * 8 + rr;
          if (m >= p.M) {
            if (p.chain) {
              const int R = lane_grp * 32 + sub * 8 + rr;
              if (F16) {
                uint8_t* t = smem + p.a3_offset + (size_t)(c4 >> 6) * 2 * A_TILE_BYTES + R * 128 +
                             ((((c4 & 63) >> 3) ^ (R & 7)) << 4) + ((c4 & 7) << 1);
                *reinterpret_cast<uint2*>(t) = make_uint2(0u, 0u);
                *reinterpret_cast<uint2*>(t + A_TILE_BYTES) = make_uint2(0u, 0u);
              } else {
                const int kb = c4 >> 5, chunk = (c4 & 31) >> 2;
                uint8_t* t = smem + p.a3_offset + (size_t)kb * 2 * A_TILE_BYTES + R * 128 + ((chunk ^ (R & 7)) << 4);
                *reinterpret_cast<float4*>(t) = make_float4(0.f, 0.f, 0.f, 0.f);
                *reinterpret_cast<float4*>(t + A_TILE_BYTES) = make_float4(0.f, 0.f, 0.f, 0.f);
              }
            }
            continue;
          }
          float y[4];
          if (NV == 1) {
#pragma unroll
            for (int i = 0; i < 4; ++i) y[i] = normalized ? g[rr][v][i] : (g[rr][v][i] - mean[rr]) * rstd[rr] * gs[i] + bs[i];
          } else {
            const float4 gv = *reinterpret_cast<const float4*>(slab + (sub * 8 + rr) * pitch + c4);
            float4 ps = make_float4(0.f, 0.f, 0.f, 0.f);
            if ((p.out_mask & OUT_HILO_POS) || (p.chain && p.pos))
              ps = __ldg(reinterpret_cast<const float4*>(p.pos + (size_t)(m % p.HW) * C + c4));
            y[0] = gv.x; y[1] = gv.y; y[2] = gv.z; y[3] = gv.w;
            pe[rr][v][0] = ps.x; pe[rr][v][1] = ps.y; pe[rr][v][2] = ps.z; pe[rr][v][3] = ps.w;
          }
          const size_t o = (size_t)m * C + c4;
          if (p.out_mask & OUT_F32) *reinterpret_cast<float4*>(out_f32 + o) = make_float4(y[0], y[1], y[2], y[3]);
          if (p.out_mask & (OUT_HILO | OUT_HILO_POS)) {
            float t[4];
#pragma unroll
            for (int i = 0; i < 4; ++i) t[i] = y[i] + pe[rr][v][i];
            store_hilo4<F16>(p.out_hi, p.out_lo, o, t);
          }
          if (p.out_mask & OUT_HILO_CELU) {
            const size_t o2 = (size_t)m * 2 * C + c4;
            float t[4], t2[4];
#pragma unroll
            for (int i = 0; i < 4; ++i) {
              t[i] = elu1(y[i]);
              t2[i] = elu1(-y[i]);
            }
            store_hilo4<F16>(p.out_hi, p.out_lo, o2, t);
            store_hilo4<F16>(p.out_hi, p.out_lo, o2 + C, t2);
          }
          if (p.chain) {
            const int R = lane_grp * 32 + sub * 8 + rr;
            if (F16) {
              unsigned short h[4], l[4];
#pragma unroll
              for (int i = 0; i < 4; ++i) split_f16(y[i] + pe[rr][v][i], h[i], l[i]);
              uint8_t* t = smem + p.a3_offset + (size_t)(c4 >> 6) * 2 * A_TILE_BYTES + R * 128 +
                           ((((c4 & 63) >> 3) ^ (R & 7)) << 4) + ((c4 & 7) << 1);
              *reinterpret_cast<uint2*>(t) = make_uint2((uint32_t)h[0] | ((uint32_t)h[1] << 16), (uint32_t)h[2] | ((uint32_t)h[3] << 16));
              *reinterpret_cast<uint2*>(t + A_TILE_BYTES) =
                  make_uint2((uint32_t)l[0] | ((uint32_t)l[1] << 16), (uint32_t)l[2] | ((uint32_t)l[3] << 16));
            } else {
              const int kb = c4 >> 5, chunk = (c4 & 31) >> 2;
              float h[4], l[4];
#pragma unroll
              for (int i = 0; i < 4; ++i) split_tf32(y[i] + pe[rr][v][i], h[i], l[i]);
              uint8_t* t = smem + p.a3_offset + (size_t)kb * 2 * A_TILE_BYTES + R * 128 + ((chunk ^ (R & 7)) << 4);
              *reinterpret_cast<float4*>(t) = make_float4(h[0], h[1], h[2], h[3]);
              *reinterpret_cast<float4*>(t + A_TILE_BYTES) = make_float4(l[0], l[1], l[2], l[3]);
            }
          }
        }
      }
      if (p.chain) {
        fence_proxy_async();
        __syncwarp();
        if (lane == 0) asm volatile("mbarrier.arrive.shared::cta.b64 _, [%0];" ::"r"(smem_u32(a3_full_bar)) : "memory");
        if (tracing && threadIdx.x == 64) p.trace[9] = clock64();
        mbar_wait(acc2_full_bar, 0, failed);
        tc_fence_after();
        if (tracing && threadIdx.x == 64) p.trace[10] = clock64();
        const int n2 = p.n2, pitch2 = n2 + 4;
        const float sc2 = F16 ? p.acc_scale2 : 1.f;
        float* slab2 = reinterpret_cast<float*>(smem) + lane_grp * (32 * pitch2);
        for (int j = sub * 16; j < n2; j += 16 * (EPI_WARPS / 4)) {
          float v16[16];
          tmem_ld16(trow + p.N + j, v16);
#pragma unroll
          for (int i = 0; i < 16; i += 4)
            *reinterpret_cast<float4*>(slab2 + lane * pitch2 + j + i) =
                make_float4(v16[i] * sc2, v16[i + 1] * sc2, v16[i + 2] * sc2, v16[i + 3] * sc2);
        }
        asm volatile("bar.sync %0, 128;" ::"r"(bar_id) : "memory");
        for (int c4 = lane * 4; c4 < n2; c4 += 128) {
#pragma unroll
          for (int rr = 0; rr < 8; ++rr) {
            const int r = sub * 8 + rr, m = slab_row0 + r;
            if (m >= p.M) break;
            *reinterpret_cast<float4*>(p.out2_f32 + (size_t)m * n2 + c4) = *reinterpret_cast<const float4*>(slab2 + r * pitch2 + c4);
          }
        }
      }
    }
  }
  if (tracing && threadIdx.x == 64) p.trace[4] = clock64();
  tc_fence_before();
  if (PAIR) cluster_sync_all();
  else __syncthreads();
  if (tracing && threadIdx.x == 0) p.trace[5] = clock64();
  if (warp == 1) {
    if (PAIR) tmem_dealloc_pair(tmem_base, (uint32_t)p.tmem_cols);
    else tmem_dealloc(tmem_base, (uint32_t)p.tmem_cols);
  }
  if (threadIdx.x == 0 && *failed && p.status) *p.status = 1;
}

template <bool F16>
__global__ void __launch_bounds__(256) nchw_to_nhwc_hilo_kernel(const float* __restrict__ x, long long batch_stride, int c,
                                                               int hw, int c_pad, float* __restrict__ hi,
                                                               float* __restrict__ lo) {
  __shared__ float tile[32][33];
  griddep_launch();
  griddep_wait();
  const int tx = threadIdx.x & 31, ty = threadIdx.x >> 5;
  const int p0 = blockIdx.x * 32, c0 = blockIdx.y * 32;
  const float* src = x + (size_t)blockIdx.z * batch_stride;
#pragma unroll
  for (int r = 0; r < 4; ++r) {
    const int ch = c0 + ty + 8 * r, p = p0 + tx;
    tile[ty + 8 * r][tx] = (ch < c && p < hw) ? __ldg(src + (size_t)ch * hw + p) : 0.f;
  }
  __syncthreads();
#pragma unroll
  for (int r = 0; r < 4; ++r) {
    const int p = p0 + ty + 8 * r, ch = c0 + tx;
    if (p < hw && ch < c_pad) {
      const size_t o = ((size_t)blockIdx.z * hw + p) * c_pad + ch;
      if (F16) {
        unsigned short h, l;
        split_f16(tile[tx][ty + 8 * r], h, l);
        reinterpret_cast<unsigned short*>(hi)[o] = h;
        reinterpret_cast<unsigned short*>(lo)[o] = l;
      } else {
        float h, l;
        split_tf32(tile[tx][ty + 8 * r], h, l);
        hi[o] = h;
        lo[o] = l;
      }
    }
  }
}

template <bool F16>
__global__ void split_hilo_kernel(const float* __restrict__ x, float* __restrict__ hi, float* __restrict__ lo,
                                  long long total, float scale) {
  griddep_launch();
  griddep_wait();
  for (long long i = blockIdx.x * (long long)blockDim.x + threadIdx.x; i < total;
       i += (long long)gridDim.x * blockDim.x) {
    if (F16) {
      unsigned short h, l;
      split_f16(x[i] * scale, h, l);
      reinterpret_cast<unsigned short*>(hi)[i] = h;
      reinterpret_cast<unsigned short*>(lo)[i] = l;
    } else {
      float h, l;
      split_tf32(x[i], h, l);
      hi[i] = h;
      lo[i] = l;
    }
  }
}

static bool make_map_act(CUtensorMap* map, const float* base, int B, int H, int W, int C, int bt, int ht, int wt, int es) {
  cuuint64_t dims[4] = {(cuuint64_t)C, (cuuint64_t)W, (cuuint64_t)H, (cuuint64_t)B};
  cuuint64_t strides[3] = {(cuuint64_t)C * es, (cuuint64_t)W * C * es, (cuuint64_t)H * W * C * es};
  cuuint32_t box[4] = {(cuuint32_t)(ROW_BYTES / es), (cuuint32_t)wt, (cuuint32_t)ht, (cuuint32_t)bt};
  cuuint32_t estr[4] = {1, 1, 1, 1};
  return encode_fn()(map, es == 2 ? CU_TENSOR_MAP_DATA_TYPE_FLOAT16 : CU_TENSOR_MAP_DATA_TYPE_FLOAT32, 4, const_cast<float*>(base), dims, strides, box, estr,
                     CU_TENSOR_MAP_INTERLEAVE_NONE, CU_TENSOR_MAP_SWIZZLE_128B, CU_TENSOR_MAP_L2_PROMOTION_L2_256B,
                     CU_TENSOR_MAP_FLOAT_OOB_FILL_NONE) == CUDA_SUCCESS;
}
static bool make_map_w(CUtensorMap* map, const float* base, int N, int Ktot, int rows, int es) {
  cuuint64_t dims[2] = {(cuuint64_t)Ktot, (cuuint64_t)N};
  cuuint64_t strides[1] = {(cuuint64_t)Ktot * es};
  cuuint32_t box[2] = {(cuuint32_t)(ROW_BYTES / es), (cuuint32_t)rows};
  cuuint32_t estr[2] = {1, 1};
  return encode_fn()(map, es == 2 ? CU_TENSOR_MAP_DATA_TYPE_FLOAT16 : CU_TENSOR_MAP_DATA_TYPE_FLOAT32, 2, const_cast<float*>(base), dims, strides, box, estr,
                     CU_TENSOR_MAP_INTERLEAVE_NONE, CU_TENSOR_MAP_SWIZZLE_128B, CU_TENSOR_MAP_L2_PROMOTION_L2_256B,
                     CU_TENSOR_MAP_FLOAT_OOB_FILL_NONE) == CUDA_SUCCESS;
}

__global__ void __launch_bounds__(256) splitk_reduce_kernel(const float* __restrict__ partial, const float* __restrict__ bias,
                                                            float* __restrict__ out_f32, float* __restrict__ out_nchw,
                                                            int M, int N, int HW, int splits) {
  __shared__ float tile[32][33];
  griddep_wait();
  const int tx = threadIdx.x & 31, ty = threadIdx.x >> 5;
  const int m0 = blockIdx.x * 32, n0 = blockIdx.y * 32;
  const size_t slice = (size_t)M * N;
#pragma unroll
  for (int r = 0; r < 4; ++r) {
    const int m = m0 + ty + 8 * r, n = n0 + tx;
    float acc = 0.f;
    if (m < M && n < N) {
      const float* q = partial + (size_t)m * N + n;
      acc = bias ? bias[n] : 0.f;
      for (int s = 0; s < splits; ++s) acc += q[s * slice];
      if (out_f32) out_f32[(size_t)m * N + n] = acc;
    }
    tile[ty + 8 * r][tx] = acc;
  }
  if (!out_nchw) return;
  __syncthreads();
#pragma unroll
  for (int r = 0; r < 4; ++r) {
    const int n = n0 + ty + 8 * r, m = m0 + tx;
    if (m < M && n < N) {
      const int b = m / HW, hw = m - b * HW;
      out_nchw[((size_t)b * N + n) * HW + hw] = tile[tx][ty + 8 * r];
    }
  }
}

static int plan_ksplit(int m_tiles, int n_tiles, int kpt, int taps) {
  const int ctas = m_tiles * n_tiles, num_kb = taps * kpt;
  if (ctas * 2 > 148 || num_kb < 32) return 1;
  int ks = 148 / ctas;
  if (ks > kpt) ks = kpt;
  if (ks > num_kb / 8) ks = num_kb / 8;
  return ks < 2 ? 1 : ks;
}

}
}

using namespace flowk;
using namespace flowk::tc;

static int conv_gemm_impl(const flowk_conv_gemm_args* a, flowk_stream_t stream, int* plan_only);

extern "C" int flowk_conv_gemm(const flowk_conv_gemm_args* a, flowk_stream_t stream) {
  return conv_gemm_impl(a, stream, nullptr);
}

extern "C" int flowk_conv_gemm_splitk_slices(const flowk_conv_gemm_args* a) {
  int ks = 1;
  const int st = conv_gemm_impl(a, nullptr, &ks);
  return st == FLOWK_OK ? ks : 1;
}

static int conv_gemm_impl(const flowk_conv_gemm_args* a, flowk_stream_t stream, int* plan_only) {
  if (!a) return FLOWK_ERR_ARG;
  if (!plan_only && (!a->a_hi || !a->a_lo || !a->w_hi || !a->w_lo)) return FLOWK_ERR_ARG;
  const int B = a->B, H = a->H, W = a->W, Cin = a->Cin, N = a->N;
  const bool f16 = a->operand_format == FLOWK_OPERAND_F16;
  if (a->operand_format != FLOWK_OPERAND_TF32 && !f16) return FLOWK_ERR_ARG;
  const int es = f16 ? 2 : 4, bk = ROW_BYTES / es;
  if (B < 1 || H < 1 || W < 1 || N < 1) return FLOWK_ERR_SHAPE;
  if (f16 ? (Cin < 8 || Cin % 8) : (Cin < BLOCK_K || Cin % BLOCK_K)) return FLOWK_ERR_SHAPE;
  if (f16 && !(a->acc_scale > 0.f)) return FLOWK_ERR_ARG;
  if (a->taps != 1 && a->taps != 9 && a->taps != 25) return FLOWK_ERR_ARG;
  const int dil = a->dilation > 0 ? a->dilation : 1;
  if (a->pre != PRE_BIAS && a->pre != PRE_GLU_RES_LN && a->pre != PRE_LSTM) return FLOWK_ERR_ARG;
  if (!plan_only && !encode_fn()) return FLOWK_ERR_ARG;
  int wt = W, ht, bt;
  if (W > BLOCK_M || BLOCK_M % W) return FLOWK_ERR_SHAPE;
  if (H * W >= BLOCK_M) {
    if ((H * W) % BLOCK_M) return FLOWK_ERR_SHAPE;
    ht = BLOCK_M / W;
    bt = 1;
  } else {
    if (BLOCK_M % (H * W)) return FLOWK_ERR_SHAPE;
    ht = H;
    bt = BLOCK_M / (H * W);
  }
  Params p{};
  p.M = B * H * W;
  p.N = N;
  p.HW = H * W;
  p.W = W;
  p.H = H;
  p.taps = a->taps;
  p.ksz = a->taps == 25 ? 5 : a->taps == 9 ? 3 : 1;
  p.dil = dil;
  p.kblocks_per_tap = (Cin + bk - 1) / bk;
  p.acc_scale = f16 ? a->acc_scale : 1.f;
  p.acc_scale_ptr = f16 ? a->acc_scale_ptr : nullptr;
  p.wt = wt;
  p.ht = ht;
  p.bt = bt;
  p.pre = a->pre;
  p.out_mask = a->out_mask;
  p.bias = a->bias;
  p.res = a->res;
  p.gamma = a->gamma;
  p.beta = a->beta;
  p.pos = a->pos;
  p.out_f32 = a->out_f32;
  p.out_hi = a->out_hi;
  p.out_lo = a->out_lo;
  p.out_nchw = a->out_nchw;
  p.status = a->status;
  p.trace = a->trace;
  p.out2_f32 = a->out2_f32;
  int n_tiles;
  if (a->pre == PRE_GLU_RES_LN) {
    const int C = N / 2;
    if ((N & 1) || C % 16 || C > 256 || !a->res || !a->gamma || !a->beta || !a->bias) return FLOWK_ERR_SHAPE;
    if (N <= 256) { p.n_chunk = N; p.n_chunks = 1; }
    else { p.n_chunk = C; p.n_chunks = 2; }
    n_tiles = 1;
  } else if (a->pre == PRE_LSTM) {
    if (N % 32 || N > 256 || !a->res || !a->gamma || !a->bias || !a->out_f32 || !a->out_hi || !a->out_lo) return FLOWK_ERR_SHAPE;
    p.n_chunk = N;
    p.n_chunks = 1;
    n_tiles = 1;
  } else {
    const int n16 = (N + 15) / 16 * 16;
    n_tiles = (n16 + 255) / 256;
    int per = (n16 / 16 + n_tiles - 1) / n_tiles * 16;
    p.n_chunk = per;
    p.n_chunks = 1;
    const int m_tiles = (B * H * W + BLOCK_M - 1) / BLOCK_M;
    if (n_tiles == 2 && !(a->out_mask & OUT_NCHW) && m_tiles * 2 > 148 && n16 <= 384) {
      n_tiles = 1;
      p.n_chunks = 2;
    }
    if (a->taps == 9 && !(a->out_mask & OUT_NCHW) && W <= 32 && 32 % W == 0 && p.n_chunks == 1)
      while (3 * p.n_chunk > 512 && p.n_chunk % 32 == 0) { p.n_chunk /= 2; n_tiles *= 2; }
    while (p.n_chunks == 1 && p.n_chunk % 32 == 0 && p.n_chunk >= 64 && m_tiles * n_tiles * 2 <= 148) {
      p.n_chunk /= 2;
      n_tiles *= 2;
    }
    if (a->taps == 9 && p.n_chunks == 1 && N % 16 == 0 && p.n_chunk * n_tiles == N) {
      const int units = N / 16;
      for (int d = units; d > n_tiles; --d)
        if (units % d == 0 && m_tiles * d <= 148) {
          n_tiles = d;
          p.n_chunk = N / d;
          break;
        }
    }
  }
  if (p.n_chunk % 16 || p.n_chunk > 256) return FLOWK_ERR_SHAPE;
  p.ksplit = 1;
  if (a->pre == PRE_BIAS && p.n_chunks == 1 && (a->out_mask == OUT_NCHW || a->out_mask == OUT_F32) && !(N & 3) &&
      (plan_only || a->splitk_ws))
    p.ksplit = plan_ksplit((B * H * W + BLOCK_M - 1) / BLOCK_M, n_tiles, p.kblocks_per_tap, a->taps);
  if (plan_only) {
    *plan_only = p.ksplit;
    return FLOWK_OK;
  }
  if (p.ksplit > 1) {
    p.out_mask = OUT_F32;
    p.out_f32 = a->splitk_ws;
    p.out_nchw = nullptr;
    p.bias = nullptr;
  }
  const int cols = p.n_chunk * p.n_chunks;
  p.tmem_cols = cols <= 32 ? 32 : cols <= 64 ? 64 : cols <= 128 ? 128 : cols <= 256 ? 256 : 512;
  const int stage_bytes = 2 * A_TILE_BYTES + 2 * cols * ROW_BYTES;
  int stages = (int)((220 * 1024 - 2048) / stage_bytes);
  if (stages > 6) stages = 6;
  if (stages < 1) return FLOWK_ERR_SHAPE;
  static int smem_cap_kb = -1;
  if (smem_cap_kb < 0) { const char* e = getenv("FLOWK_GEMM_SMEM_CAP_KB"); smem_cap_kb = e ? atoi(e) : 0; }
  if (smem_cap_kb > 0 && p.tmem_cols <= 256)
    while (stages > 1 && (size_t)stages * stage_bytes > (size_t)smem_cap_kb * 1024) --stages;
  p.dxsplit = (a->taps == 9 && dil == 1 && a->pre == PRE_BIAS && W <= 32 && 32 % W == 0 && p.n_chunks == 1 &&
               3 * p.n_chunk <= 512 && p.ksplit == 1) ? 1 : 0;
  p.pair = 0;
  if (p.dxsplit && f16) {
    static int pair_env = -1, nmma_env = 0;
    if (pair_env < 0) {
      const char* e = getenv("FLOWK_PAIR");
      pair_env = e ? atoi(e) : 0;
      e = getenv("FLOWK_PAIR_NMMA");
      nmma_env = e ? atoi(e) : 0;
    }
    const int m_tiles = (p.M + BLOCK_M - 1) / BLOCK_M;
    const int n_total = 3 * p.n_chunk;
    int n_mma = (n_total + 255) / 256;
    if ((n_total / n_mma) % 16 || n_total % n_mma) n_mma = 3;
    if (nmma_env == 3) n_mma = p.pair_nmma = 3;
    const int half = n_total / n_mma / 2;
    int unit = half;
    while (unit > 0 && (half % unit || p.n_chunk % unit || unit % 8)) unit -= 8;
    if (pair_env && m_tiles % 2 == 0 && p.M % BLOCK_M == 0 && m_tiles * n_tiles >= 64 && (n_total / n_mma) % 16 == 0 &&
        half % 8 == 0 && unit >= 8) {
      p.pair = 1;
      p.w_unit = unit;
    }
  }
  if (p.dxsplit) {
    p.tmem_cols = 3 * p.n_chunk <= 256 ? 256 : 512;
    if (3 * p.n_chunk <= 128) p.tmem_cols = 128;
    const int w_slot_bytes = (p.pair ? 3 : 6) * cols * ROW_BYTES;
    p.a_slots = (220 * 1024 - 2048 - 4 * 2 * A_TILE_BYTES) / w_slot_bytes >= 3 ? 4 : 2;
    if (const char* e = getenv("FLOWK_A_SLOTS")) p.a_slots = atoi(e);
    int ws = (int)((220 * 1024 - 2048 - p.a_slots * 2 * A_TILE_BYTES) / w_slot_bytes);
    p.w_slots = ws > 4 ? 4 : ws;
    if (p.w_slots < 2) p.dxsplit = 0;
  }
  size_t epi_bytes = (size_t)4 * 32 * (cols + 4) * sizeof(float);
  if (a->pre == PRE_GLU_RES_LN) epi_bytes = (size_t)4 * 32 * (N / 2 + 4) * sizeof(float);
  if ((p.out_mask & (OUT_F32 | OUT_HILO | OUT_HILO_POS | OUT_HILO_CELU | OUT_HILO_RELU)) && (N & 3)) return FLOWK_ERR_SHAPE;
  while (stages > 1 && (size_t)stages * stage_bytes + 2048 > 227 * 1024) --stages;
  size_t region = (size_t)stages * stage_bytes;
  if (p.dxsplit) region = (size_t)p.a_slots * 2 * A_TILE_BYTES + (size_t)p.w_slots * (p.pair ? 3 : 6) * cols * ROW_BYTES;
  if (epi_bytes > region) region = (epi_bytes + 1023) / 1024 * 1024;
  if (region + 2048 > 227 * 1024) return FLOWK_ERR_SHAPE;
  p.chain = 0;
  if (a->w2_hi && a->w2_lo && a->out2_f32 && a->N2 > 0) {
    const int C = N / 2, n2 = a->N2;
    if (a->pre != PRE_GLU_RES_LN || p.n_chunks != 1 || C % (f16 ? 8 : BLOCK_K) || n2 % 16 || N + n2 > 512) return FLOWK_ERR_SHAPE;
    if (f16 && !(a->acc_scale2 > 0.f)) return FLOWK_ERR_ARG;
    const int kb2 = (C + bk - 1) / bk;
    p.acc_scale2 = f16 ? a->acc_scale2 : 1.f;
    p.n2 = n2;
    p.n2_chunks = n2 <= 256 ? 1 : 2;
    p.n2_chunk = n2 / p.n2_chunks;
    if (p.n2_chunk % 16 || p.n2_chunk > 256) return FLOWK_ERR_SHAPE;
    const size_t slab = (size_t)4 * 32 * (C + 4) * sizeof(float);
    p.a3_offset = (int)((slab + 1023) / 1024 * 1024);
    p.w2_offset = p.a3_offset + kb2 * 2 * A_TILE_BYTES;
    const size_t chain_end = (size_t)p.w2_offset + (size_t)2 * n2 * ROW_BYTES;
    const size_t slab2 = (size_t)4 * 32 * (n2 + 4) * sizeof(float);
    if (chain_end > region) region = (chain_end + 1023) / 1024 * 1024;
    if (slab2 > region) region = (slab2 + 1023) / 1024 * 1024;
    if (region + 2048 > 227 * 1024) return FLOWK_ERR_SHAPE;
    p.tmem_cols = 512;
    p.chain = 1;
  }
  p.stages = stages;
  p.bar_offset = (int)region;
  const size_t smem_bytes = region + 1024 + 256;

  alignas(64) CUtensorMap ma_hi, ma_lo, mw_hi, mw_lo, mw2_hi, mw2_lo;
  const int Ktot = a->taps * p.kblocks_per_tap * bk;
  if (!make_map_act(&ma_hi, a->a_hi, B, H, W, Cin, bt, ht, wt, es) || !make_map_act(&ma_lo, a->a_lo, B, H, W, Cin, bt, ht, wt, es) ||
      !make_map_w(&mw_hi, a->w_hi, N, Ktot, p.pair ? p.w_unit : p.n_chunk, es) ||
      !make_map_w(&mw_lo, a->w_lo, N, Ktot, p.pair ? p.w_unit : p.n_chunk, es))
    return FLOWK_ERR_ARG;
  if (p.chain) {
    const int k2tot = f16 ? ((N / 2 + bk - 1) / bk) * bk : N / 2;
    if (!make_map_w(&mw2_hi, a->w2_hi, p.n2, k2tot, p.n2_chunk, es) || !make_map_w(&mw2_lo, a->w2_lo, p.n2, k2tot, p.n2_chunk, es))
      return FLOWK_ERR_ARG;
  } else {
    mw2_hi = mw_hi;
    mw2_lo = mw_lo;
  }

  dim3 grid((p.M + BLOCK_M - 1) / BLOCK_M, n_tiles, p.ksplit);
#define FLOWK_LAUNCH_GEMM(PRE_, NV_, F16_, PAIR_)                                                                         \
  do {                                                                                                              \
    static size_t smem_set = 0;                                                                                     \
    if (smem_bytes > smem_set) {                                                                                    \
      FLOWK_CUDA_OK(cudaFuncSetAttribute(conv_gemm_kernel<PRE_, NV_, F16_, PAIR_>, cudaFuncAttributeMaxDynamicSharedMemorySize, \
                                         (int)smem_bytes));                                                         \
      smem_set = smem_bytes;                                                                                        \
    }                                                                                                               \
    FLOWK_CUDA_OK(launch_pdl_cluster(conv_gemm_kernel<PRE_, NV_, F16_, PAIR_>, grid, dim3(NUM_THREADS), smem_bytes, stream,          \
                                     PAIR_ ? 2 : 1, ma_hi, ma_lo, mw_hi, mw_lo, mw2_hi, mw2_lo, p));               \
  } while (0)
  if (a->pre == PRE_LSTM) {
    if (f16) FLOWK_LAUNCH_GEMM(PRE_LSTM, 1, true, false); else FLOWK_LAUNCH_GEMM(PRE_LSTM, 1, false, false);
  } else if (a->pre == PRE_GLU_RES_LN && N / 2 > 128) {
    if (f16) FLOWK_LAUNCH_GEMM(PRE_GLU_RES_LN, 2, true, false); else FLOWK_LAUNCH_GEMM(PRE_GLU_RES_LN, 2, false, false);
  } else if (a->pre == PRE_GLU_RES_LN) {
    if (f16) FLOWK_LAUNCH_GEMM(PRE_GLU_RES_LN, 1, true, false); else FLOWK_LAUNCH_GEMM(PRE_GLU_RES_LN, 1, false, false);
  } else if (p.pair) {
    FLOWK_LAUNCH_GEMM(PRE_BIAS, 1, true, true);
  } else {
    if (f16) FLOWK_LAUNCH_GEMM(PRE_BIAS, 1, true, false); else FLOWK_LAUNCH_GEMM(PRE_BIAS, 1, false, false);
  }
#undef FLOWK_LAUNCH_GEMM
  if (p.ksplit > 1) {
    FLOWK_CUDA_OK(launch_pdl(splitk_reduce_kernel, dim3((p.M + 31) / 32, (N + 31) / 32), dim3(256), 0, stream, (const float*)a->splitk_ws, a->bias,
                             a->out_mask == OUT_F32 ? a->out_f32 : (float*)nullptr,
                             a->out_mask == OUT_NCHW ? a->out_nchw : (float*)nullptr, p.M, N, p.HW, p.ksplit));
  }
  return launch_status();
}

static int check_mar_dst(const void* hi, const void* lo, int pitch, int col, int width) {
  if (!hi || !lo) return FLOWK_ERR_ARG;
  if (pitch < 1 || col < 0 || col + width > pitch || (width > 1 && (pitch % 4 || col % 4))) return FLOWK_ERR_SHAPE;
  return FLOWK_OK;
}

extern "C" int flowk_mar_step(const flowk_mar_step_args* a, flowk_stream_t stream) {
  if (!a) return FLOWK_ERR_ARG;
  const int mode = a->mode;
  if (mode != FLOWK_MAR_EMBED && mode != FLOWK_MAR_LSTM && mode != FLOWK_MAR_SAMPLE) return FLOWK_ERR_ARG;
  if (!a->a_hi || !a->a_lo || !a->w_hi || !a->w_lo || !a->bias) return FLOWK_ERR_ARG;
  if (mode == FLOWK_MAR_LSTM && !a->c) return FLOWK_ERR_ARG;
  if (mode == FLOWK_MAR_SAMPLE && (!a->noise || !a->z)) return FLOWK_ERR_ARG;
  if (a->taps != 1 && a->taps != 9 && a->taps != 25) return FLOWK_ERR_ARG;
  if (!(a->acc_scale > 0.f)) return FLOWK_ERR_ARG;
  const int B = a->B, H = a->H, W = a->W, Cin = a->Cin, hid = a->hid;
  if (B < 1 || H < 1 || W < 1 || Cin < 8 || Cin % 8) return FLOWK_ERR_SHAPE;
  if (hid < 8 || hid % 8 || 4 * hid > 256) return FLOWK_ERR_SHAPE;
  const int width = mode == FLOWK_MAR_SAMPLE ? 1 : hid;
  int st = check_mar_dst(a->dst0_hi, a->dst0_lo, a->dst0_pitch, a->dst0_col, width);
  if (st != FLOWK_OK) return st;
  const bool dst1 = mode == FLOWK_MAR_LSTM && (a->dst1_hi || a->dst1_lo);
  if (dst1 && (st = check_mar_dst(a->dst1_hi, a->dst1_lo, a->dst1_pitch, a->dst1_col, width)) != FLOWK_OK) return st;
  if (mode == FLOWK_MAR_SAMPLE && a->z_stride < (long long)H * W) return FLOWK_ERR_SHAPE;
  if (W > BLOCK_M || BLOCK_M % W) return FLOWK_ERR_SHAPE;
  if (H * W >= BLOCK_M ? (H * W) % BLOCK_M != 0 : BLOCK_M % (H * W) != 0) return FLOWK_ERR_SHAPE;
  if (!encode_fn()) return FLOWK_ERR_ARG;

  const int N = mode == FLOWK_MAR_LSTM ? 4 * hid : mode == FLOWK_MAR_EMBED ? hid : 2;
  constexpr int bk = 64;
  Params p{};
  p.M = B * H * W;
  p.N = N;
  p.HW = H * W;
  p.W = W;
  p.H = H;
  p.taps = a->taps;
  p.ksz = a->taps == 25 ? 5 : a->taps == 9 ? 3 : 1;
  p.dil = a->dilation > 0 ? a->dilation : 1;
  p.kblocks_per_tap = (Cin + bk - 1) / bk;
  p.wt = W;
  p.ht = H * W >= BLOCK_M ? BLOCK_M / W : H;
  p.bt = H * W >= BLOCK_M ? 1 : BLOCK_M / (H * W);
  p.n_chunk = (N + 15) / 16 * 16;
  p.n_chunks = 1;
  p.ksplit = 1;
  p.pre = PRE_MAR_EMBED + mode;
  p.bias = a->bias;
  p.acc_scale = a->acc_scale;
  p.status = a->status;
  p.dst_hi[0] = a->dst0_hi;
  p.dst_lo[0] = a->dst0_lo;
  p.dst_pitch[0] = a->dst0_pitch;
  p.dst_col[0] = a->dst0_col;
  if (dst1) {
    p.dst_hi[1] = a->dst1_hi;
    p.dst_lo[1] = a->dst1_lo;
    p.dst_pitch[1] = a->dst1_pitch;
    p.dst_col[1] = a->dst1_col;
  }
  p.cell = a->c;
  p.noise = a->noise;
  p.z = a->z;
  p.z_stride = a->z_stride;
  p.tmem_cols = p.n_chunk <= 32 ? 32 : p.n_chunk <= 64 ? 64 : p.n_chunk <= 128 ? 128 : 256;
  const int stage_bytes = 2 * A_TILE_BYTES + 2 * p.n_chunk * ROW_BYTES;
  int stages = (220 * 1024 - 2048) / stage_bytes;
  if (stages > 6) stages = 6;
  p.stages = stages;
  p.bar_offset = stages * stage_bytes;
  const size_t smem_bytes = (size_t)p.bar_offset + 1024 + 256;

  alignas(64) CUtensorMap ma_hi, ma_lo, mw_hi, mw_lo;
  const int Ktot = p.taps * p.kblocks_per_tap * bk;
  if (!make_map_act(&ma_hi, (const float*)a->a_hi, B, H, W, Cin, p.bt, p.ht, p.wt, 2) ||
      !make_map_act(&ma_lo, (const float*)a->a_lo, B, H, W, Cin, p.bt, p.ht, p.wt, 2) ||
      !make_map_w(&mw_hi, (const float*)a->w_hi, N, Ktot, p.n_chunk, 2) ||
      !make_map_w(&mw_lo, (const float*)a->w_lo, N, Ktot, p.n_chunk, 2))
    return FLOWK_ERR_ARG;
  const dim3 grid((p.M + BLOCK_M - 1) / BLOCK_M, 1, 1);
#define FLOWK_LAUNCH_MAR(PRE_)                                                                                          \
  do {                                                                                                                  \
    static size_t smem_set = 0;                                                                                         \
    if (smem_bytes > smem_set) {                                                                                        \
      FLOWK_CUDA_OK(cudaFuncSetAttribute(conv_gemm_kernel<PRE_, 1, true, false>,                                        \
                                         cudaFuncAttributeMaxDynamicSharedMemorySize, (int)smem_bytes));                \
      smem_set = smem_bytes;                                                                                            \
    }                                                                                                                   \
    FLOWK_CUDA_OK(launch_pdl_cluster(conv_gemm_kernel<PRE_, 1, true, false>, grid, dim3(NUM_THREADS), smem_bytes,       \
                                     stream, 1, ma_hi, ma_lo, mw_hi, mw_lo, mw_hi, mw_lo, p));                          \
  } while (0)
  if (mode == FLOWK_MAR_EMBED) FLOWK_LAUNCH_MAR(PRE_MAR_EMBED);
  else if (mode == FLOWK_MAR_LSTM) FLOWK_LAUNCH_MAR(PRE_MAR_LSTM);
  else FLOWK_LAUNCH_MAR(PRE_MAR_SAMPLE);
#undef FLOWK_LAUNCH_MAR
  return launch_status();
}

extern "C" int flowk_nchw_to_nhwc_hilo(const float* x, long long batch_stride, int B, int C, int HW, int C_pad,
                                       float* hi, float* lo, flowk_stream_t stream) {
  if (B < 0 || C < 1 || HW < 1 || C_pad < C) return FLOWK_ERR_SHAPE;
  if (B == 0) return FLOWK_OK;
  if (!x || !hi || !lo) return FLOWK_ERR_ARG;
  if (B > 65535) return FLOWK_ERR_SHAPE;
  FLOWK_CUDA_OK(launch_pdl(nchw_to_nhwc_hilo_kernel<false>, dim3((HW + 31) / 32, (C_pad + 31) / 32, B), dim3(256), 0, stream, x,
                           batch_stride, C, HW, C_pad, hi, lo));
  return launch_status();
}

extern "C" int flowk_nchw_to_nhwc_hilo_f16(const float* x, long long batch_stride, int B, int C, int HW, int C_pad,
                                           void* hi, void* lo, flowk_stream_t stream) {
  if (B < 0 || C < 1 || HW < 1 || C_pad < C || C_pad % 8) return FLOWK_ERR_SHAPE;
  if (B == 0) return FLOWK_OK;
  if (!x || !hi || !lo) return FLOWK_ERR_ARG;
  if (B > 65535) return FLOWK_ERR_SHAPE;
  FLOWK_CUDA_OK(launch_pdl(nchw_to_nhwc_hilo_kernel<true>, dim3((HW + 31) / 32, (C_pad + 31) / 32, B), dim3(256), 0, stream, x,
                           batch_stride, C, HW, C_pad, reinterpret_cast<float*>(hi), reinterpret_cast<float*>(lo)));
  return launch_status();
}

extern "C" int flowk_split_hilo(const float* x, float* hi, float* lo, long long n, flowk_stream_t stream) {
  if (n < 0) return FLOWK_ERR_SHAPE;
  if (n == 0) return FLOWK_OK;
  if (!x || !hi || !lo) return FLOWK_ERR_ARG;
  const int blocks = (int)((n + 255) / 256 < 148 * 8 ? (n + 255) / 256 : 148 * 8);
  FLOWK_CUDA_OK(launch_pdl(split_hilo_kernel<false>, dim3(blocks), dim3(256), 0, stream, x, hi, lo, (long long)n, 1.f));
  return launch_status();
}

extern "C" int flowk_split_hilo_f16(const float* x, void* hi, void* lo, long long n, float scale, flowk_stream_t stream) {
  if (n < 0) return FLOWK_ERR_SHAPE;
  if (n == 0) return FLOWK_OK;
  if (!x || !hi || !lo) return FLOWK_ERR_ARG;
  const int blocks = (int)((n + 255) / 256 < 148 * 8 ? (n + 255) / 256 : 148 * 8);
  FLOWK_CUDA_OK(launch_pdl(split_hilo_kernel<true>, dim3(blocks), dim3(256), 0, stream, x, reinterpret_cast<float*>(hi),
                           reinterpret_cast<float*>(lo), (long long)n, scale));
  return launch_status();
}
```

gaussian-processes-after-pre-processing-with-normalising-flows-2_b200/tc.py:

```python
import ctypes

import torch

from . import _lib
from ._lib import (OUT_F32, OUT_HILO, OUT_HILO_CELU, OUT_HILO_POS, OUT_HILO_RELU, OUT_NCHW, PRE_BIAS,
                   PRE_GLU_RES_LN, PRE_LSTM)


def _stream():
    return torch.cuda.current_stream().cuda_stream


def split_hilo(t):
    t = t.contiguous().float()
    if t.is_cuda and t.numel():
        return split_rows(t)

    def rna(v):
        return ((v.view(torch.int32) + 0x1000) & -8192).view(torch.float32)
    hi = rna(t)
    return hi, rna(t - hi)


def conv_weight_operand(w, cin_pad=None):
    if w.dim() == 2:
        w = w[:, :, None, None]
    n, cin, kh, kw = w.shape
    cin_pad = cin_pad or ((cin + 31) // 32 * 32)
    wk = w.permute(0, 2, 3, 1)
    if cin_pad != cin:
        wk = torch.nn.functional.pad(wk, (0, cin_pad - cin))
    return split_hilo(wk.reshape(n, kh * kw * cin_pad))


def conv_weight_operand_f16(w, gain=None, mode=_lib.PACK_PLAIN, factor=1.0, bias=None):
    if w.dim() == 2:
        w = w[:, :, None, None]
    n, cin, kh, kw = w.shape
    cin_pad = (cin + 63) // 64 * 64
    taps = kh * kw
    w = w.detach().contiguous().float()
    _lib.check_device(w, "conv_weight_operand_f16")
    hi = torch.empty(n, taps * cin_pad, device=w.device, dtype=torch.float16)
    lo = torch.empty_like(hi)
    ws = torch.empty(n + 2, device=w.device, dtype=torch.float32)
    g = None if gain is None else gain.detach().reshape(-1).contiguous().float()
    b_in = None if bias is None else bias.detach().reshape(-1).contiguous().float()
    b_out = None if bias is None else torch.empty_like(b_in)
    assert g is None or g.numel() == n
    _lib.call("flowk_pack_weight_f16", w.data_ptr(), _p(g), int(mode), float(factor), _p(b_in), _p(b_out), n, cin, taps,
              cin_pad, hi.data_ptr(), lo.data_ptr(), ws.data_ptr(), _stream())
    acc_scale = float(ws[n + 1])
    return (hi, lo, acc_scale) if bias is None else (hi, lo, acc_scale, b_out)


def split_rows_f16(x, scale=1.0):
    hi = torch.empty(x.shape, device=x.device, dtype=torch.float16)
    lo = torch.empty_like(hi)
    _lib.call("flowk_split_hilo_f16", x.data_ptr(), hi.data_ptr(), lo.data_ptr(), x.numel(), float(scale), _stream())
    return hi, lo


def _p(t):
    return None if t is None else t.data_ptr()


def conv_gemm(a_hi, a_lo, w_hi, w_lo, B, H, W, Cin, N, taps, pre, out_mask, bias=None, res=None, gamma=None,
              beta=None, pos=None, out_f32=None, out_hi=None, out_lo=None, out_nchw=None, status=None, trace=None,
              w2_hi=None, w2_lo=None, out2_f32=None, n2=0, split_k=False, acc_scale=None, dilation=1, acc_scale2=None,
              acc_scale_ptr=None):
    _lib.check_device(a_hi, "conv_gemm")
    args = _lib.ConvGemmArgs(_p(a_hi), _p(a_lo), _p(w_hi), _p(w_lo), _p(bias), _p(res), _p(gamma), _p(beta), _p(pos),
                             _p(out_f32), _p(out_hi), _p(out_lo), _p(out_nchw), _p(status), _p(trace),
                             B, H, W, Cin, N, taps, pre, out_mask, _p(w2_hi), _p(w2_lo), _p(out2_f32), n2, None,
                             _lib.OPERAND_F16 if a_hi.dtype == torch.float16 else _lib.OPERAND_TF32,
                             1.0 if acc_scale is None else float(acc_scale), int(dilation),
                             1.0 if acc_scale2 is None else float(acc_scale2), _p(acc_scale_ptr))
    assert a_hi.dtype == a_lo.dtype == w_hi.dtype == w_lo.dtype, "operand pair formats must agree"
    assert out_hi is None or out_hi.dtype == a_hi.dtype, "out_hi/out_lo are written in the input operand format"
    if split_k:
        slices = _lib.lib.flowk_conv_gemm_splitk_slices(ctypes.addressof(args))
        if slices > 1:
            ws = torch.empty(slices * B * H * W * N, device=a_hi.device, dtype=torch.float32)
            args.splitk_ws = ws.data_ptr()
    _lib.call("flowk_conv_gemm", ctypes.addressof(args), _stream(), meta=(B, H, W, Cin, N, taps, pre))


def nchw_to_nhwc_hilo(x, c_pad, f16=False, out=None):
    b, c, h, w = x.shape
    assert x.stride(3) == 1 and x.stride(2) == w and x.stride(1) == h * w, "channel slice of a contiguous NCHW tensor"
    if out is None:
        hi = torch.empty(b * h * w, c_pad, device=x.device, dtype=torch.float16 if f16 else torch.float32)
        lo = torch.empty_like(hi)
    else:
        hi, lo = out
        assert hi.shape == lo.shape == (b * h * w, c_pad) and hi.is_contiguous() and lo.is_contiguous()
        assert hi.dtype == lo.dtype == (torch.float16 if f16 else torch.float32)
    _lib.call("flowk_nchw_to_nhwc_hilo_f16" if f16 else "flowk_nchw_to_nhwc_hilo", x.data_ptr(), x.stride(0), b, c, h * w,
              c_pad, hi.data_ptr(), lo.data_ptr(), _stream())
    return hi, lo


def mar_step_args(mode, a, w, bias, B, H, W, taps, hid, dst0, dilation=1, dst1=None, c=None, noise=None, z=None,
                  z_stride=0, status=None):
    assert a[0].dtype == a[1].dtype == w[0].dtype == w[1].dtype == torch.float16
    _lib.check_device(a[0], "mar_step")
    d1 = dst1 or (None, None, 0, 0)
    return _lib.MarStepArgs(_p(a[0]), _p(a[1]), _p(w[0]), _p(w[1]), _p(bias), _p(dst0[0]), _p(dst0[1]), _p(d1[0]),
                            _p(d1[1]), _p(c), _p(noise), _p(z), int(z_stride), _p(status), int(mode), B, H, W,
                            a[0].shape[1], taps, int(dilation), hid, dst0[2], dst0[3], d1[2], d1[3], float(w[2]))


def mar_step(args):
    _lib.call("flowk_mar_step", ctypes.addressof(args), _stream(), meta=(args.mode, args.B, args.H, args.W, args.hid))


def split_rows(x):
    hi = torch.empty_like(x)
    lo = torch.empty_like(x)
    _lib.call("flowk_split_hilo", x.data_ptr(), hi.data_ptr(), lo.data_ptr(), x.numel(), _stream())
    return hi, lo


ATTENTION_TC = __import__("os").environ.get("FLOWK_ATTENTION_TC", "1") != "0"


def attention_tc_supported(HW, C, heads):
    d = C // max(heads, 1)
    if not (ATTENTION_TC and C % heads == 0 and HW in (128, 256) and d % 8 == 0 and d <= 64 and C % 4 == 0):
        return False
    dk = (d + 15) // 16 * 16
    smem = max(4 * (HW // 64) * 128 * 64, 4 * HW * 128) + 2 * (HW // 64) * dk * 128 + 2 * 128 * (d // 8) * 16 + 9 * 1024
    return smem <= 227 * 1024


ATTENTION_TC_V2 = __import__("os").environ.get("FLOWK_ATTENTION_TC_V2", "1") != "0"


def attention_tc_v2_supported(HW, C, heads):
    if not (ATTENTION_TC and ATTENTION_TC_V2 and heads >= 1 and C % heads == 0):
        return False
    return HW in (128, 256) and C // heads in (24, 32)


def attention(qkv, B, HW, C, heads, f16=False, status=None, trace=None):
    hi = torch.empty(B * HW, C, device=qkv.device, dtype=torch.float16 if f16 else torch.float32)
    lo = torch.empty_like(hi)
    if attention_tc_v2_supported(HW, C, heads):
        _lib.call("flowk_attention_tc_v2", qkv.data_ptr(), hi.data_ptr(), lo.data_ptr(), int(f16), B, HW, C, heads,
                  _p(status), _p(trace), _stream())
        return hi, lo
    if attention_tc_supported(HW, C, heads):
        _lib.call("flowk_attention_tc", qkv.data_ptr(), hi.data_ptr(), lo.data_ptr(), int(f16), B, HW, C, heads,
                  _p(status), _p(trace), _stream())
        return hi, lo
    _lib.call("flowk_attention_f16" if f16 else "flowk_attention", qkv.data_ptr(), hi.data_ptr(), lo.data_ptr(), B, HW, C,
              heads, _stream())
    return hi, lo


ATTENTION_INPROJ = __import__("os").environ.get("FLOWK_ATTENTION_INPROJ", "1") != "0"


def attention_inproj_supported(HW, C, heads):
    return ATTENTION_INPROJ and attention_tc_v2_supported(HW, C, heads)


def attention_inproj(p_hi, p_lo, w_hi, w_lo, acc_scale, B, HW, C, heads, status=None, trace=None):
    assert p_hi.dtype == p_lo.dtype == w_hi.dtype == w_lo.dtype == torch.float16
    assert p_hi.shape == p_lo.shape == (B * HW, C) and p_hi.is_contiguous() and p_lo.is_contiguous(), \
        "p_hi / p_lo must be contiguous [B*HW, C]"
    assert w_hi.shape == w_lo.shape == (3 * C, (C + 63) // 64 * 64) and w_hi.is_contiguous() and w_lo.is_contiguous(), \
        "w_hi / w_lo must be the contiguous in_proj operand [3C, ceil64(C)]"
    _lib.check_device(p_hi, "attention_inproj")
    hi = torch.empty(B * HW, C, device=p_hi.device, dtype=torch.float16)
    lo = torch.empty_like(hi)
    _lib.call("flowk_attention_inproj_tc", p_hi.data_ptr(), p_lo.data_ptr(), w_hi.data_ptr(), w_lo.data_ptr(),
              float(acc_scale), hi.data_ptr(), lo.data_ptr(), B, HW, C, heads, _p(status), _p(trace), _stream())
    return hi, lo


def attention_supported(HW, C, heads):
    if attention_tc_supported(HW, C, heads):
        return True
    return C % heads == 0 and (C // heads) in (8, 16, 24, 32, 40, 64) and (HW <= 256 or HW % 256 == 0) and HW % 4 == 0 \
        and 2 * min(HW, 1 << 30) * (C // heads) * 4 * max(1, 256 // max(HW, 1)) <= 220 * 1024


def chain_supported(C, n2, f16=False):
    if C % (8 if f16 else 32) or n2 % 16 or 2 * C > 256 or 2 * C + n2 > 512:
        return False
    slab = ((4 * 32 * (C + 4) * 4 + 1023) // 1024) * 1024
    kblocks = (C + 63) // 64 if f16 else C // 32
    return slab + kblocks * 32768 + 2 * n2 * 128 + 2048 <= 227 * 1024
```

include/flowk.h:

```cpp
#ifndef FLOWK_H_
#define FLOWK_H_

#include <stddef.h>

#ifdef __cplusplus
extern "C" {
#endif

typedef struct CUstream_st* flowk_stream_t;

enum {
  FLOWK_OK = 0,
  FLOWK_ERR_SHAPE = 1,
  FLOWK_ERR_ALIGN = 2,
  FLOWK_ERR_ARG = 3,
  FLOWK_ERR_CUDA_BASE = 1000
};

int flowk_abi_version(void);
const char* flowk_error_string(int status);
size_t flowk_ldj_workspace_bytes(int B);

int flowk_squeeze2d(const float* x, float* y, int B, int C, int H, int W, int factor, flowk_stream_t stream);
int flowk_unsqueeze2d(const float* x, float* y, int B, int C, int H, int W, int factor, flowk_stream_t stream);

int flowk_actnorm_init(const float* x, float* bias, float* logs, int B, int C, int HW,
                       float scale, float eps, flowk_stream_t stream);

int flowk_channel_scale(const float* x, const float* pre, const float* mul, const float* post, float* y,
                        const float* ldj_in, const float* ldj_add, float* ldj_out,
                        int B, int C, int HW, flowk_stream_t stream);

int flowk_channel_mix(const float* x, const float* Wm, const float* bias, float* y,
                      const float* ldj_in, const float* ldj_add, float* ldj_out,
                      int B, int C, int H, int W, int in_squeeze, int out_unsqueeze,
                      flowk_stream_t stream);

int flowk_affine_coupling_fwd(const float* x, const float* h, float* y, const float* ldj_in, float* ldj_out,
                              void* ws, int B, int C, int HW, flowk_stream_t stream);
int flowk_affine_coupling_inv(const float* x, const float* h, float* y, const float* ldj_in, float* ldj_out,
                              void* ws, int B, int C, int HW, flowk_stream_t stream);
int flowk_affine_coupling_bwd(const float* x, const float* h, const float* gy, const float* gldj,
                              float* gx, float* gh, int B, int C, int HW, flowk_stream_t stream);

int flowk_mixlogcdf_fwd(const float* x, const float* raw, const float* rescale, float* y,
                        const float* ldj_in, float* ldj_out, void* ws,
                        int B, int C, int HW, int K, int flip, flowk_stream_t stream);
int flowk_mixlogcdf_inv(const float* x, const float* raw, const float* rescale, float* y,
                        const float* ldj_in, float* ldj_out, void* ws,
                        int B, int C, int HW, int K, int flip, flowk_stream_t stream);
int flowk_mixlogcdf_bwd(const float* x, const float* raw, const float* rescale,
                        const float* gy, const float* gldj, float* gx, float* graw, float* ga_tanh,
                        int B, int C, int HW, int K, int flip, flowk_stream_t stream);

int flowk_mixture_log_cdf(const float* x, const float* pi, const float* mu, const float* s, float* out,
                          int B, int K, int N, flowk_stream_t stream);
int flowk_mixture_log_pdf(const float* x, const float* pi, const float* mu, const float* s, float* out,
                          int B, int K, int N, flowk_stream_t stream);
int flowk_mixture_inv_cdf(const float* y, const float* pi, const float* mu, const float* s, float* out,
                          int B, int K, int N, flowk_stream_t stream);

enum { FLOWK_PRE_BIAS = 0, FLOWK_PRE_GLU_RES_LN = 1, FLOWK_PRE_LSTM = 2 };
enum { FLOWK_OUT_F32 = 1, FLOWK_OUT_HILO = 2, FLOWK_OUT_HILO_POS = 4, FLOWK_OUT_HILO_CELU = 8, FLOWK_OUT_NCHW = 16,
       FLOWK_OUT_HILO_RELU = 32 };

typedef struct flowk_conv_gemm_args {
  const float* a_hi;
  const float* a_lo;
  const float* w_hi;
  const float* w_lo;
  const float* bias;
  const float* res;
  const float* gamma;
  const float* beta;
  const float* pos;
  float* out_f32;
  float* out_hi;
  float* out_lo;
  float* out_nchw;
  int* status;
  long long* trace;
  int B, H, W, Cin, N, taps, pre, out_mask;
  const float* w2_hi;
  const float* w2_lo;
  float* out2_f32;
  int N2;
  float* splitk_ws;
  int operand_format;
  float acc_scale;
  int dilation;
  float acc_scale2;
  const float* acc_scale_ptr;
} flowk_conv_gemm_args;
enum { FLOWK_OPERAND_TF32 = 0, FLOWK_OPERAND_F16 = 1 };

int flowk_conv_gemm(const flowk_conv_gemm_args* args, flowk_stream_t stream);
int flowk_conv_gemm_splitk_slices(const flowk_conv_gemm_args* args);

enum { FLOWK_MAR_EMBED = 0, FLOWK_MAR_LSTM = 1, FLOWK_MAR_SAMPLE = 2 };
typedef struct flowk_mar_step_args {
  const void* a_hi;
  const void* a_lo;
  const void* w_hi;
  const void* w_lo;
  const float* bias;
  void* dst0_hi;
  void* dst0_lo;
  void* dst1_hi;
  void* dst1_lo;
  float* c;
  const float* noise;
  float* z;
  long long z_stride;
  int* status;
  int mode, B, H, W, Cin, taps, dilation, hid;
  int dst0_pitch, dst0_col, dst1_pitch, dst1_col;
  float acc_scale;
} flowk_mar_step_args;
int flowk_mar_step(const flowk_mar_step_args* args, flowk_stream_t stream);

int flowk_nchw_to_nhwc_hilo(const float* x, long long batch_stride, int B, int C, int HW, int C_pad,
                            float* hi, float* lo, flowk_stream_t stream);
int flowk_split_hilo(const float* x, float* hi, float* lo, long long n, flowk_stream_t stream);
int flowk_nchw_to_nhwc_hilo_f16(const float* x, long long batch_stride, int B, int C, int HW, int C_pad,
                                void* hi, void* lo, flowk_stream_t stream);
int flowk_split_hilo_f16(const float* x, void* hi, void* lo, long long n, float scale, flowk_stream_t stream);

enum { FLOWK_PACK_PLAIN = 0, FLOWK_PACK_WEIGHT_NORM = 1, FLOWK_PACK_EXP_GAIN = 2 };
int flowk_pack_weight_f16(const float* w, const float* gain, int mode, float factor, const float* bias_in, float* bias_out,
                          int N, int cin, int taps, int cin_pad, void* hi, void* lo, float* ws, flowk_stream_t stream);

int flowk_fold_actnorm_invconv(const float* l, const float* u, const float* log_s, const float* p, const float* sign_s,
                               const float* logs, const float* bias, int C, int H, int W, int reverse, float* mat,
                               float* bias_out, float* ldj, flowk_stream_t stream);

int flowk_concat_elu_fwd(const float* x, float* y, const float* mask, long long outer, int C, long long inner,
                         flowk_stream_t stream);
int flowk_concat_elu_bwd(const float* x, const float* gy, float* gx, const float* mask, long long outer, int C,
                         long long inner, flowk_stream_t stream);
int flowk_glu_fwd(const float* x, float* y, long long outer, int C, long long inner, flowk_stream_t stream);
int flowk_glu_bwd(const float* x, const float* gy, float* gx, long long outer, int C, long long inner,
                  flowk_stream_t stream);

int flowk_weight_norm_operands(const float* v, const float* g, int N, int cin, int taps, int cin_pad, int n_pad,
                               float* norm, float* w, float* fwd_hi, float* fwd_lo, float* dg_hi, float* dg_lo,
                               flowk_stream_t stream);
typedef struct flowk_wn_job {
  const float* v;
  const float* g;
  float* norm;
  float* w;
  float* fwd_hi;
  float* fwd_lo;
  float* dg_hi;
  float* dg_lo;
  int N, cin, taps, cin_pad, n_pad;
  int fwd_f16;
} flowk_wn_job;
int flowk_weight_norm_operands_batched(const flowk_wn_job* jobs_device, int njobs, int max_rows, flowk_stream_t stream);
int flowk_weight_norm_bwd(const float* v, const float* g, const float* norm, const float* gw, float* gv, float* gg,
                          int N, int cols, flowk_stream_t stream);

int flowk_std_normal_logp(const float* z, long long sample_stride, const float* in, float* out, int B, long long n,
                          flowk_stream_t stream);

long long flowk_add_layernorm_workspace_bytes(long long M, int C);
int flowk_add_layernorm_fwd(const float* a, const float* b, const float* gamma, const float* beta, float* y, float* s,
                            float* mean, float* rstd, long long M, int C, int HW, int in_nchw, int out_nchw, float eps,
                            flowk_stream_t stream);
int flowk_add_layernorm_bwd(const float* gy, const float* s, const float* mean, const float* rstd, const float* gamma,
                            float* gs, float* dgamma, float* dbeta, void* workspace, long long M, int C, int HW,
                            int in_nchw, int out_nchw, flowk_stream_t stream);

long long flowk_channel_sum_workspace_bytes(int C);
int flowk_channel_sum(const float* x, float* out, void* workspace, long long outer, int C, long long inner,
                      flowk_stream_t stream);

int flowk_conv_wgrad_splits(int B, int H, int W, int Cin, int N, int taps, int* transposed);
int flowk_conv_wgrad(const float* x, const float* x_left, const float* x_right, const float* gy, float* partial,
                     int* status, int B, int H, int W, int Cin, int N, int taps, flowk_stream_t stream);
int flowk_linear_wgrad_splits(long long M, int K, int N, int* transposed);
int flowk_linear_wgrad(const float* x, const float* gy, float* partial, int* status, long long M, int K, int N,
                       flowk_stream_t stream);
int flowk_shift_columns(const float* x, float* x_left, float* x_right, long long total, int W, flowk_stream_t stream);
int flowk_weight_norm_bwd_partials(const float* v, const float* g, const float* norm, const float* partial, float* gv,
                                   float* gg, int N, int cin, int taps, int splits, int transposed,
                                   flowk_stream_t stream);

int flowk_attention_train_fwd(const float* qkv, float* out, float* lse, const unsigned* seed_device, unsigned salt,
                              float p_drop, int B, int HW, int C, int heads, flowk_stream_t stream);
int flowk_attention_train_bwd(int which, const float* qkv, const float* out, const float* dout, const float* lse,
                              float* dqkv, const unsigned* seed_device, unsigned salt, float p_drop, int B, int HW, int C,
                              int heads, flowk_stream_t stream);
int flowk_attention_dropout_mask(const unsigned* seed_device, unsigned salt, float p_drop, int pairs, int HW, float* mask,
                                 flowk_stream_t stream);

typedef struct flowk_adamax_chunk {
  float* p;
  const float* g;
  float* m;
  float* u;
  long long n;
} flowk_adamax_chunk;
int flowk_adamax_step(const flowk_adamax_chunk* chunks_device, int nchunks, const float* clr_device, float beta1,
                      float beta2, float eps, flowk_stream_t stream);

int flowk_attention(const float* qkv, float* out_hi, float* out_lo, int B, int HW, int C, int heads,
                    flowk_stream_t stream);
int flowk_attention_f16(const float* qkv, void* out_hi, void* out_lo, int B, int HW, int C, int heads,
                        flowk_stream_t stream);

int flowk_patch_attention(const float* x, const float* G, const float* prm, float* y, const float* ldj_in, float* ldj_out,
                          int B, int C, int H, int W, int permute, int reverse, flowk_stream_t stream);

int flowk_patch_attention_train_fwd(const float* x, const float* G, const float* prm, float* y, const float* ldj_in,
                                    float* ldj_out, float* scores, int B, int C, int H, int W, int permute,
                                    flowk_stream_t stream);
int flowk_patch_attention_bwd(const float* x, const float* G, const float* prm, const float* scores, const float* gy,
                              const float* gldj, float* gx, float* partials, int B, int C, int H, int W, int permute,
                              flowk_stream_t stream);

int flowk_attention_tc(const float* qkv, void* out_hi, void* out_lo, int out_f16, int B, int HW, int C, int heads,
                       int* status, long long* trace, flowk_stream_t stream);
int flowk_attention_tc_v2(const float* qkv, void* out_hi, void* out_lo, int out_f16, int B, int HW, int C, int heads,
                          int* status, long long* trace, flowk_stream_t stream);
int flowk_attention_tc_v2_occupancy(int HW, int C, int heads, int* blocks_per_sm, int* smem_bytes);
int flowk_attention_inproj_tc(const void* p_hi, const void* p_lo, const void* w_hi, const void* w_lo, float acc_scale,
                              void* out_hi, void* out_lo, int B, int HW, int C, int heads, int* status, long long* trace,
                              flowk_stream_t stream);
int flowk_attention_inproj_tc_occupancy(int HW, int C, int heads, int* blocks_per_sm, int* smem_bytes);

#ifdef __cplusplus
}
#endif
#endif
```

Measured before the change: 12280.

## Add shared-SM conv GEMM variant with fewer epilogue warps for co-residency

Adds a conv_gemm kernel variant with 8 epilogue warps and launch bounds allowing two CTAs per SM, enabled by default through an env flag. The epilogue store loops are generalized to a variable warp count, with a flattened row/column store loop. The intent is to let independent GEMMs or streams co-reside on an SM rather than each occupying a full SM exclusively. Footprint query APIs and a coresidency probe script are also added. Fewer epilogue warps per CTA may lengthen single-kernel epilogue time.

After: 14710 (median of 6 runs). +19.8%, better.

```diff
diff --git a/gaussian-processes-after-pre-processing-with-normalising-flows-2_b200/_lib.py b/gaussian-processes-after-pre-processing-with-normalising-flows-2_b200/_lib.py
--- a/gaussian-processes-after-pre-processing-with-normalising-flows-2_b200/_lib.py
+++ b/gaussian-processes-after-pre-processing-with-normalising-flows-2_b200/_lib.py
@@ -78,6 +78,9 @@
     "flowk_adamax_step": ([_fp, _i, _fp, ctypes.c_float, ctypes.c_float, ctypes.c_float, _st], _i),
     "flowk_glu_bwd": ([_fp, _fp, _fp, ctypes.c_longlong, _i, ctypes.c_longlong, _st], _i),
     "flowk_mar_step": ([ctypes.c_void_p, _st], _i),
+    "flowk_conv_gemm_footprint": ([ctypes.c_void_p, ctypes.c_void_p], _i),
+    "flowk_conv_gemm_set_shared_sm": ([_i], None),
+    "flowk_attention_tc_footprint": ([_i, _i, _i, _i, ctypes.c_void_p], _i),
 }
 
 
@@ -89,6 +92,10 @@
                [(n, ctypes.c_void_p) for n in ("w2_hi", "w2_lo", "out2_f32")] + [("N2", ctypes.c_int)] + \
                [("splitk_ws", ctypes.c_void_p), ("operand_format", ctypes.c_int), ("acc_scale", ctypes.c_float),
                 ("dilation", ctypes.c_int), ("acc_scale2", ctypes.c_float), ("acc_scale_ptr", ctypes.c_void_p)]
+
+
+class SmFootprint(ctypes.Structure):
+    _fields_ = [(n, ctypes.c_int) for n in ("threads", "regs_per_thread", "smem_bytes", "tmem_cols", "blocks_per_sm")]
 
 
 class MarStepArgs(ctypes.Structure):
diff --git a/gaussian-processes-after-pre-processing-with-normalising-flows-2_b200/csrc/attention_tc.cu b/gaussian-processes-after-pre-processing-with-normalising-flows-2_b200/csrc/attention_tc.cu
--- a/gaussian-processes-after-pre-processing-with-normalising-flows-2_b200/csrc/attention_tc.cu
+++ b/gaussian-processes-after-pre-processing-with-normalising-flows-2_b200/csrc/attention_tc.cu
@@ -688,6 +688,19 @@
 using namespace flowk;
 using namespace flowk::tc;
 
+static size_t attention_tc_smem(AttParams& p) {
+  const int HW = p.HW;
+  const int p_bytes = 2 * (HW / 64) * 128 * ROW_B;
+  const int qk_bytes = 2 * HW * ROW_B + 2 * HW * ROW_B;
+  const int first = p_bytes > qk_bytes ? p_bytes : qk_bytes;
+  p.p_off = 0;
+  p.q_off = 0;
+  p.k_off = 2 * HW * ROW_B;
+  p.v_off = first;
+  p.o_off = first + 2 * (HW / 64) * p.dk * ROW_B;
+  return (size_t)p.o_off + (size_t)2 * 128 * (p.D / 8) * 16 + 1024;
+}
+
 extern "C" int flowk_attention_tc(const float* qkv, void* out_hi, void* out_lo, int out_f16, int B, int HW, int C, int heads,
                                   int* status, long long* trace, flowk_stream_t stream) {
   if (B < 0 || HW < 1 || C < 1 || heads < 1 || C % heads) return FLOWK_ERR_SHAPE;
@@ -709,15 +722,7 @@
   p.qscale = 1.4426950408889634f / sqrtf((float)D);
   p.status = status;
   p.trace = trace;
-  const int p_bytes = 2 * (HW / 64) * 128 * ROW_B;
-  const int qk_bytes = 2 * HW * ROW_B + 2 * HW * ROW_B;
-  const int first = p_bytes > qk_bytes ? p_bytes : qk_bytes;
-  p.p_off = 0;
-  p.q_off = 0;
-  p.k_off = 2 * HW * ROW_B;
-  p.v_off = first;
-  p.o_off = first + 2 * (HW / 64) * p.dk * ROW_B;
-  const size_t smem = (size_t)p.o_off + (size_t)2 * 128 * (D / 8) * 16 + 1024;
+  const size_t smem = attention_tc_smem(p);
   if (smem + 8 * 1024 > 227 * 1024) return FLOWK_ERR_SHAPE;
 #define FLOWK_LAUNCH_ATT(KCH_)                                                                                          \
   do {                                                                                                                 \
@@ -845,32 +850,31 @@
 
 namespace {
 template <int KCH, int TILES, bool INPROJ>
-int attention_tc_v2_fit(size_t smem, int* blocks_per_sm) {
+int attention_tc_v2_fit(size_t smem, flowk_sm_footprint* f) {
   FLOWK_CUDA_OK((attention_tc_v2_prepare<KCH, TILES, INPROJ>(smem)));
-  cudaFuncAttributes fa;
-  FLOWK_CUDA_OK(cudaFuncGetAttributes(&fa, attention_tc_v2_kernel<KCH, TILES, INPROJ>));
-  int dev = 0, regs_sm = 0, smem_sm = 0, reserved = 0, threads_sm = 0;
-  FLOWK_CUDA_OK(cudaGetDevice(&dev));
-  FLOWK_CUDA_OK(cudaDeviceGetAttribute(&regs_sm, cudaDevAttrMaxRegistersPerMultiprocessor, dev));
-  FLOWK_CUDA_OK(cudaDeviceGetAttribute(&smem_sm, cudaDevAttrMaxSharedMemoryPerMultiprocessor, dev));
-  FLOWK_CUDA_OK(cudaDeviceGetAttribute(&reserved, cudaDevAttrReservedSharedMemoryPerBlock, dev));
-  FLOWK_CUDA_OK(cudaDeviceGetAttribute(&threads_sm, cudaDevAttrMaxThreadsPerMultiProcessor, dev));
-  const int warp_regs = (fa.numRegs * 32 + 255) / 256 * 256;
-  const int by_regs = regs_sm / (warp_regs * (V2_THREADS / 32));
-  const int by_smem = smem_sm / (int)(smem + fa.sharedSizeBytes + (size_t)reserved);
-  const int by_threads = threads_sm / V2_THREADS;
-  *blocks_per_sm = by_regs < by_smem ? (by_regs < by_threads ? by_regs : by_threads) : (by_smem < by_threads ? by_smem : by_threads);
-  return FLOWK_OK;
+  return sm_footprint(reinterpret_cast<const void*>(attention_tc_v2_kernel<KCH, TILES, INPROJ>), V2_THREADS, smem,
+                      V2_TMEM_COLS, f);
+}
+
+template <bool INPROJ>
+int attention_tc_v2_footprint(int HW, int C, int heads, flowk_sm_footprint* f, int* smem_bytes) {
+  AttParams p{};
+  size_t smem = 0;
+  if (!attention_tc_v2_plan(HW, C, heads, INPROJ, p, smem)) return FLOWK_ERR_SHAPE;
+  if (smem_bytes) *smem_bytes = (int)smem;
+  return HW == 256 ? attention_tc_v2_fit<4, 2, INPROJ>(smem, f) : attention_tc_v2_fit<4, 1, INPROJ>(smem, f);
 }
 
 template <bool INPROJ>
 int attention_tc_v2_occupancy(int HW, int C, int heads, int* blocks_per_sm, int* smem_bytes) {
+  flowk_sm_footprint f{};
   AttParams p{};
   size_t smem = 0;
   if (!attention_tc_v2_plan(HW, C, heads, INPROJ, p, smem)) return FLOWK_ERR_SHAPE;
   if (!blocks_per_sm) return FLOWK_ERR_ARG;
-  if (smem_bytes) *smem_bytes = (int)smem;
-  return HW == 256 ? attention_tc_v2_fit<4, 2, INPROJ>(smem, blocks_per_sm) : attention_tc_v2_fit<4, 1, INPROJ>(smem, blocks_per_sm);
+  const int st = attention_tc_v2_footprint<INPROJ>(HW, C, heads, &f, smem_bytes);
+  if (st == FLOWK_OK) *blocks_per_sm = f.blocks_per_sm;
+  return st;
 }
 }
 
@@ -881,3 +885,24 @@
 extern "C" int flowk_attention_inproj_tc_occupancy(int HW, int C, int heads, int* blocks_per_sm, int* smem_bytes) {
   return attention_tc_v2_occupancy<true>(HW, C, heads, blocks_per_sm, smem_bytes);
 }
+
+extern "C" int flowk_attention_tc_footprint(int kernel, int HW, int C, int heads, flowk_sm_footprint* f) {
+  if (!f) return FLOWK_ERR_ARG;
+  if (kernel == 1) return attention_tc_v2_footprint<false>(HW, C, heads, f, nullptr);
+  if (kernel == 2) return attention_tc_v2_footprint<true>(HW, C, heads, f, nullptr);
+  if (kernel != 0) return FLOWK_ERR_ARG;
+  if (HW < 1 || C < 1 || heads < 1 || C % heads) return FLOWK_ERR_SHAPE;
+  AttParams p{};
+  p.HW = HW;
+  p.D = C / heads;
+  p.dk = (p.D + 15) / 16 * 16;
+  if ((HW != 128 && HW != 256) || p.D % 8 || p.D > 64 || C % 4) return FLOWK_ERR_SHAPE;
+  const size_t smem = attention_tc_smem(p);
+  if (smem + 8 * 1024 > 227 * 1024) return FLOWK_ERR_SHAPE;
+  const int tmem_cols = HW <= 128 ? 128 : 512;
+  const void* k = p.dk == 16 ? reinterpret_cast<const void*>(attention_tc_kernel<2>)
+                : p.dk == 32 ? reinterpret_cast<const void*>(attention_tc_kernel<4>)
+                : p.dk == 48 ? reinterpret_cast<const void*>(attention_tc_kernel<6>)
+                             : reinterpret_cast<const void*>(attention_tc_kernel<8>);
+  return sm_footprint(k, ATT_THREADS, smem, tmem_cols, f);
+}
diff --git a/gaussian-processes-after-pre-processing-with-normalising-flows-2_b200/csrc/common.cuh b/gaussian-processes-after-pre-processing-with-normalising-flows-2_b200/csrc/common.cuh
--- a/gaussian-processes-after-pre-processing-with-normalising-flows-2_b200/csrc/common.cuh
+++ b/gaussian-processes-after-pre-processing-with-normalising-flows-2_b200/csrc/common.cuh
@@ -17,6 +17,27 @@
 inline int launch_status() {
   cudaError_t e = cudaGetLastError();
   return e == cudaSuccess ? FLOWK_OK : FLOWK_ERR_CUDA_BASE + (int)e;
+}
+
+inline int sm_footprint(const void* kernel, int threads, size_t dyn_smem, int tmem_cols, flowk_sm_footprint* f) {
+  cudaFuncAttributes fa;
+  FLOWK_CUDA_OK(cudaFuncGetAttributes(&fa, kernel));
+  int dev = 0, regs_sm = 0, smem_sm = 0, reserved = 0, threads_sm = 0;
+  FLOWK_CUDA_OK(cudaGetDevice(&dev));
+  FLOWK_CUDA_OK(cudaDeviceGetAttribute(&regs_sm, cudaDevAttrMaxRegistersPerMultiprocessor, dev));
+  FLOWK_CUDA_OK(cudaDeviceGetAttribute(&smem_sm, cudaDevAttrMaxSharedMemoryPerMultiprocessor, dev));
+  FLOWK_CUDA_OK(cudaDeviceGetAttribute(&reserved, cudaDevAttrReservedSharedMemoryPerBlock, dev));
+  FLOWK_CUDA_OK(cudaDeviceGetAttribute(&threads_sm, cudaDevAttrMaxThreadsPerMultiProcessor, dev));
+  f->threads = threads;
+  f->regs_per_thread = fa.numRegs;
+  f->smem_bytes = (int)(dyn_smem + fa.sharedSizeBytes + (size_t)reserved);
+  f->tmem_cols = tmem_cols;
+  const int warp_regs = (fa.numRegs * 32 + 255) / 256 * 256;
+  const int by_regs = regs_sm / (warp_regs * ((threads + 31) / 32));
+  const int by_smem = smem_sm / f->smem_bytes;
+  const int by_threads = threads_sm / threads;
+  f->blocks_per_sm = by_regs < by_smem ? (by_regs < by_threads ? by_regs : by_threads) : (by_smem < by_threads ? by_smem : by_threads);
+  return FLOWK_OK;
 }
 
 inline bool aligned16(const void* p) { return (reinterpret_cast<uintptr_t>(p) & 15u) == 0; }
diff --git a/gaussian-processes-after-pre-processing-with-normalising-flows-2_b200/csrc/tc_gemm.cu b/gaussian-processes-after-pre-processing-with-normalising-flows-2_b200/csrc/tc_gemm.cu
--- a/gaussian-processes-after-pre-processing-with-normalising-flows-2_b200/csrc/tc_gemm.cu
+++ b/gaussian-processes-after-pre-processing-with-normalising-flows-2_b200/csrc/tc_gemm.cu
@@ -9,11 +9,18 @@
 constexpr int ROW_BYTES = 128;
 constexpr int A_TILE_BYTES = BLOCK_M * ROW_BYTES;
 constexpr int EPI_WARPS = 16;
-constexpr int NUM_THREADS = 64 + 32 * EPI_WARPS;
+constexpr int SHARED_EPI_WARPS = 8;
+constexpr int gemm_threads(int epi_warps) { return 64 + 32 * epi_warps; }
+constexpr int SHARED_REGION_BYTES = 108 * 1024;
 constexpr int MAX_CHUNKS = 2;
 
 __device__ __forceinline__ float elu1(float x) { return x > 0.f ? x : ex2_fast(x * kLog2e) - 1.f; }
 __device__ __forceinline__ float sigmoid_fast(float x) { return __fdividef(1.f, 1.f + ex2_fast(-x * kLog2e)); }
+template <int S>
+__device__ __forceinline__ float group_sum(const float (*part)[32], int lane) {
+  if constexpr (S == 4) return (part[0][lane] + part[1][lane]) + (part[2][lane] + part[3][lane]);
+  else return part[0][lane] + part[1][lane];
+}
 
 enum { PRE_BIAS = 0, PRE_GLU_RES_LN = 1, PRE_LSTM = 2 };
 enum { PRE_MAR_EMBED = 3, PRE_MAR_LSTM = 4, PRE_MAR_SAMPLE = 5 };
@@ -56,8 +63,8 @@
   long long z_stride;
 };
 
-template <int PRE, int NV, bool F16, bool PAIR = false>
-__global__ void __launch_bounds__(NUM_THREADS, 1)
+template <int PRE, bool F16, bool PAIR = false, int EW = EPI_WARPS>
+__global__ void __launch_bounds__(gemm_threads(EW), EW == EPI_WARPS ? 1 : 2)
 conv_gemm_kernel(const __grid_constant__ CUtensorMap map_a_hi, const __grid_constant__ CUtensorMap map_a_lo,
                  const __grid_constant__ CUtensorMap map_w_hi, const __grid_constant__ CUtensorMap map_w_lo,
                  const __grid_constant__ CUtensorMap map_w2_hi, const __grid_constant__ CUtensorMap map_w2_lo,
@@ -97,7 +104,7 @@
       for (int s = 0; s < p.stages; ++s) { mbar_init(&full_bar[s], 1); mbar_init(&empty_bar[s], 1); }
     }
     mbar_init(tmem_full_bar, 1);
-    mbar_init(a3_full_bar, EPI_WARPS);
+    mbar_init(a3_full_bar, EW);
     mbar_init(w2_full_bar, 1);
     mbar_init(w2_empty_bar, 1);
     mbar_init(acc2_full_bar, 1);
@@ -351,6 +358,7 @@
       }
     }
   } else {
+    constexpr int SUBS = EW / 4, RPW = 32 / SUBS;
     const int lane_grp = warp & 3;
     const int sub = (warp - 2) >> 2;
     const int slab_row0 = m_tile * BLOCK_M + lane_grp * 32;
@@ -366,7 +374,7 @@
         const int m = slab_row0 + lane;
         const bool valid = m < p.M;
         const int hw = valid ? m % p.HW : 0, img = valid ? m / p.HW : 0;
-        for (int j = sub * 16; j < ncols_cta; j += 16 * (EPI_WARPS / 4)) {
+        for (int j = sub * 16; j < ncols_cta; j += 16 * SUBS) {
           const int n0 = n_base + j;
           if (n0 >= p.N) break;
           float v[16];
@@ -396,7 +404,7 @@
         const int pitch = ncols_cta + 4;
         float* slab = reinterpret_cast<float*>(smem) + lane_grp * (32 * pitch);
         const int bar_id = 1 + lane_grp;
-        for (int j = sub * 16; j < ncols_cta; j += 16 * (EPI_WARPS / 4)) {
+        for (int j = sub * 16; j < ncols_cta; j += 16 * SUBS) {
           float v[16];
           if (p.dxsplit) {
             float vm[16], vp[16];
@@ -422,35 +430,32 @@
                 make_float4(fmaf(v[i], sc, bv.x), fmaf(v[i + 1], sc, bv.y), fmaf(v[i + 2], sc, bv.z), fmaf(v[i + 3], sc, bv.w));
           }
         }
-        asm volatile("bar.sync %0, 128;" ::"r"(bar_id) : "memory");
-        for (int c4 = lane * 4; c4 < ncols_cta; c4 += 128) {
-          const int n = n_base + c4;
-          if (n >= p.N) break;
-#pragma unroll
-          for (int rr = 0; rr < 8; ++rr) {
-            const int r = sub * 8 + rr, m = slab_row0 + r;
-            if (m >= p.M) break;
-            const float4 y = *reinterpret_cast<const float4*>(slab + r * pitch + c4);
-            const float ys[4] = {y.x, y.y, y.z, y.w};
-            const size_t o = (size_t)m * p.N + n;
-            if (p.out_mask & OUT_F32) *reinterpret_cast<float4*>(out_f32 + o) = y;
-            if (p.out_mask & (OUT_HILO | OUT_HILO_RELU)) {
-              float t[4];
-#pragma unroll
-              for (int i = 0; i < 4; ++i) t[i] = (p.out_mask & OUT_HILO_RELU) ? fmaxf(ys[i], 0.f) : ys[i];
-              store_hilo4<F16>(p.out_hi, p.out_lo, o, t);
+        asm volatile("bar.sync %0, %1;" ::"r"(bar_id), "n"(32 * SUBS) : "memory");
+        const int upr = (ncols_cta < p.N - n_base ? ncols_cta : p.N - n_base) >> 2;
+        for (int u = lane; u < RPW * upr; u += 32) {
+          const int rr = u / upr, c4 = (u - rr * upr) * 4;
+          const int r = sub * RPW + rr, m = slab_row0 + r, n = n_base + c4;
+          if (m >= p.M) break;
+          const float4 y = *reinterpret_cast<const float4*>(slab + r * pitch + c4);
+          const float ys[4] = {y.x, y.y, y.z, y.w};
+          const size_t o = (size_t)m * p.N + n;
+          if (p.out_mask & OUT_F32) *reinterpret_cast<float4*>(out_f32 + o) = y;
+          if (p.out_mask & (OUT_HILO | OUT_HILO_RELU)) {
+            float t[4];
+#pragma unroll
+            for (int i = 0; i < 4; ++i) t[i] = (p.out_mask & OUT_HILO_RELU) ? fmaxf(ys[i], 0.f) : ys[i];
+            store_hilo4<F16>(p.out_hi, p.out_lo, o, t);
+          }
+          if (p.out_mask & OUT_HILO_CELU) {
+            const size_t o2 = (size_t)m * 2 * p.N + n;
+            float t[4], t2[4];
+#pragma unroll
+            for (int i = 0; i < 4; ++i) {
+              t[i] = elu1(ys[i]);
+              t2[i] = elu1(-ys[i]);
             }
-            if (p.out_mask & OUT_HILO_CELU) {
-              const size_t o2 = (size_t)m * 2 * p.N + n;
-              float t[4], t2[4];
-#pragma unroll
-              for (int i = 0; i < 4; ++i) {
-                t[i] = elu1(ys[i]);
-                t2[i] = elu1(-ys[i]);
-              }
-              store_hilo4<F16>(p.out_hi, p.out_lo, o2, t);
-              store_hilo4<F16>(p.out_hi, p.out_lo, o2 + p.N, t2);
-            }
+            store_hilo4<F16>(p.out_hi, p.out_lo, o2, t);
+            store_hilo4<F16>(p.out_hi, p.out_lo, o2 + p.N, t2);
           }
         }
       }
@@ -495,7 +500,7 @@
       const int m = slab_row0 + lane;
       const bool row_ok = m < p.M;
       const int hid = PRE == PRE_MAR_LSTM ? p.N >> 2 : p.N;
-      for (int j = sub * 8; j < hid; j += 32) {
+      for (int j = sub * 8; j < hid; j += 8 * SUBS) {
         __syncwarp();
         float hn[8];
         if (PRE == PRE_MAR_EMBED) {
@@ -557,242 +562,142 @@
       const int pitch = C + 4;
       float* slab = reinterpret_cast<float*>(smem) + lane_grp * (32 * pitch);
       const int bar_id = 1 + lane_grp;
-      const int nv = (C + 127) / 128;
-      float g[8][NV][4], pe[8][NV][4];
-      float mean[8], rstd[8];
-      bool normalized = false;
-      if (NV == 1) {
-        __shared__ float ln_part[2][4][4][32];
+      __shared__ float ln_part[2][4][SUBS][32];
+      float* const srow = slab + lane * pitch;
+      {
         const int m_row = slab_row0 + lane;
         const bool row_ok = m_row < p.M;
-        float gb[2][16];
         float psum = 0.f;
-#pragma unroll
-        for (int ci = 0; ci < 2; ++ci) {
-          const int j = sub * 16 + ci * 64;
-          if (j < C) {
-            float a[16], b[16];
-            tmem_ld16(trow + j, a);
-            tmem_ld16(trow + C + j, b);
-#pragma unroll
-            for (int i = 0; i < 16; i += 4) {
-              const float4 ba = __ldg(reinterpret_cast<const float4*>(p.bias + j + i));
-              const float4 bb = __ldg(reinterpret_cast<const float4*>(p.bias + C + j + i));
-              const float4 rs = row_ok ? __ldg(reinterpret_cast<const float4*>(p.res + (size_t)m_row * C + j + i))
-                                       : make_float4(0.f, 0.f, 0.f, 0.f);
-              gb[ci][i] = fmaf(a[i], sc, ba.x) * sigmoid_fast(fmaf(b[i], sc, bb.x)) + rs.x;
-              gb[ci][i + 1] = fmaf(a[i + 1], sc, ba.y) * sigmoid_fast(fmaf(b[i + 1], sc, bb.y)) + rs.y;
-              gb[ci][i + 2] = fmaf(a[i + 2], sc, ba.z) * sigmoid_fast(fmaf(b[i + 2], sc, bb.z)) + rs.z;
-              gb[ci][i + 3] = fmaf(a[i + 3], sc, ba.w) * sigmoid_fast(fmaf(b[i + 3], sc, bb.w)) + rs.w;
-              psum += (gb[ci][i] + gb[ci][i + 1]) + (gb[ci][i + 2] + gb[ci][i + 3]);
-            }
+        for (int j = sub * 16; j < C; j += 16 * SUBS) {
+          float a[16], b[16];
+          tmem_ld16(trow + j, a);
+          tmem_ld16(trow + C + j, b);
+#pragma unroll
+          for (int i = 0; i < 16; i += 4) {
+            const float4 ba = __ldg(reinterpret_cast<const float4*>(p.bias + j + i));
+            const float4 bb = __ldg(reinterpret_cast<const float4*>(p.bias + C + j + i));
+            const float4 rs = row_ok ? __ldg(reinterpret_cast<const float4*>(p.res + (size_t)m_row * C + j + i))
+                                     : make_float4(0.f, 0.f, 0.f, 0.f);
+            float4 g;
+            g.x = fmaf(a[i], sc, ba.x) * sigmoid_fast(fmaf(b[i], sc, bb.x)) + rs.x;
+            g.y = fmaf(a[i + 1], sc, ba.y) * sigmoid_fast(fmaf(b[i + 1], sc, bb.y)) + rs.y;
+            g.z = fmaf(a[i + 2], sc, ba.z) * sigmoid_fast(fmaf(b[i + 2], sc, bb.z)) + rs.z;
+            g.w = fmaf(a[i + 3], sc, ba.w) * sigmoid_fast(fmaf(b[i + 3], sc, bb.w)) + rs.w;
+            psum += (g.x + g.y) + (g.z + g.w);
+            *reinterpret_cast<float4*>(srow + j + i) = g;
           }
         }
         ln_part[0][lane_grp][sub][lane] = psum;
-        asm volatile("bar.sync %0, 128;" ::"r"(bar_id) : "memory");
-        const float mu = ((ln_part[0][lane_grp][0][lane] + ln_part[0][lane_grp][1][lane]) +
-                          (ln_part[0][lane_grp][2][lane] + ln_part[0][lane_grp][3][lane])) / (float)C;
+        asm volatile("bar.sync %0, %1;" ::"r"(bar_id), "n"(32 * SUBS) : "memory");
+        const float mu = group_sum<SUBS>(ln_part[0][lane_grp], lane) / (float)C;
         float pvar = 0.f;
-#pragma unroll
-        for (int ci = 0; ci < 2; ++ci)
-          if (sub * 16 + ci * 64 < C) {
-#pragma unroll
-            for (int i = 0; i < 16; ++i) pvar = fmaf(gb[ci][i] - mu, gb[ci][i] - mu, pvar);
-          }
+        for (int j = sub * 16; j < C; j += 16 * SUBS) {
+#pragma unroll
+          for (int i = 0; i < 16; i += 4) {
+            const float4 g = *reinterpret_cast<const float4*>(srow + j + i);
+            pvar = fmaf(g.x - mu, g.x - mu, pvar);
+            pvar = fmaf(g.y - mu, g.y - mu, pvar);
+            pvar = fmaf(g.z - mu, g.z - mu, pvar);
+            pvar = fmaf(g.w - mu, g.w - mu, pvar);
+          }
+        }
         ln_part[1][lane_grp][sub][lane] = pvar;
-        asm volatile("bar.sync %0, 128;" ::"r"(bar_id) : "memory");
-        const float rs_ = rsqrtf(((ln_part[1][lane_grp][0][lane] + ln_part[1][lane_grp][1][lane]) +
-                                  (ln_part[1][lane_grp][2][lane] + ln_part[1][lane_grp][3][lane])) / (float)C + 1e-5f);
+        asm volatile("bar.sync %0, %1;" ::"r"(bar_id), "n"(32 * SUBS) : "memory");
+        const float rs_ = rsqrtf(group_sum<SUBS>(ln_part[1][lane_grp], lane) / (float)C + 1e-5f);
         if (tracing && threadIdx.x == 64) p.trace[6] = clock64();
-#pragma unroll
-        for (int ci = 0; ci < 2; ++ci) {
-          const int j = sub * 16 + ci * 64;
-          if (j < C) {
-#pragma unroll
-            for (int i = 0; i < 16; i += 4) {
-              const float4 ga = __ldg(reinterpret_cast<const float4*>(p.gamma + j + i));
-              const float4 be = __ldg(reinterpret_cast<const float4*>(p.beta + j + i));
-              *reinterpret_cast<float4*>(slab + lane * pitch + j + i) =
-                  make_float4(fmaf((gb[ci][i] - mu) * rs_, ga.x, be.x), fmaf((gb[ci][i + 1] - mu) * rs_, ga.y, be.y),
-                              fmaf((gb[ci][i + 2] - mu) * rs_, ga.z, be.z), fmaf((gb[ci][i + 3] - mu) * rs_, ga.w, be.w));
-            }
-          }
-        }
-        asm volatile("bar.sync %0, 128;" ::"r"(bar_id) : "memory");
+        for (int j = sub * 16; j < C; j += 16 * SUBS) {
+#pragma unroll
+          for (int i = 0; i < 16; i += 4) {
+            const float4 ga = __ldg(reinterpret_cast<const float4*>(p.gamma + j + i));
+            const float4 be = __ldg(reinterpret_cast<const float4*>(p.beta + j + i));
+            const float4 g = *reinterpret_cast<const float4*>(srow + j + i);
+            *reinterpret_cast<float4*>(srow + j + i) =
+                make_float4(fmaf((g.x - mu) * rs_, ga.x, be.x), fmaf((g.y - mu) * rs_, ga.y, be.y),
+                            fmaf((g.z - mu) * rs_, ga.z, be.z), fmaf((g.w - mu) * rs_, ga.w, be.w));
+          }
+        }
+        asm volatile("bar.sync %0, %1;" ::"r"(bar_id), "n"(32 * SUBS) : "memory");
         if (tracing && threadIdx.x == 64) p.trace[7] = clock64();
-        normalized = true;
-#pragma unroll
-        for (int rr = 0; rr < 8; ++rr) {
-          const int r = sub * 8 + rr, m = slab_row0 + r;
-          const int c4 = lane * 4;
-          float4 ps = make_float4(0.f, 0.f, 0.f, 0.f), gv = ps;
-          if (c4 < C) {
-            gv = *reinterpret_cast<const float4*>(slab + r * pitch + c4);
-            if (((p.out_mask & OUT_HILO_POS) || (p.chain && p.pos)) && m < p.M)
-              ps = __ldg(reinterpret_cast<const float4*>(p.pos + (size_t)(m % p.HW) * C + c4));
-          }
-          g[rr][0][0] = gv.x; g[rr][0][1] = gv.y; g[rr][0][2] = gv.z; g[rr][0][3] = gv.w;
-          pe[rr][0][0] = ps.x; pe[rr][0][1] = ps.y; pe[rr][0][2] = ps.z; pe[rr][0][3] = ps.w;
-          mean[rr] = 0.f;
-          rstd[rr] = 1.f;
-        }
-      } else {
-        __shared__ float ln_part2[2][4][4][32];
-        const int m_row = slab_row0 + lane;
-        const bool row_ok = m_row < p.M;
-        float gb[4][16];
-        float psum = 0.f;
-#pragma unroll
-        for (int ci = 0; ci < 4; ++ci) {
-          const int j = sub * 16 + ci * 64;
-          if (j < C) {
-            float a[16], b[16];
-            tmem_ld16(trow + j, a);
-            tmem_ld16(trow + C + j, b);
-#pragma unroll
-            for (int i = 0; i < 16; i += 4) {
-              const float4 ba = __ldg(reinterpret_cast<const float4*>(p.bias + j + i));
-              const float4 bb = __ldg(reinterpret_cast<const float4*>(p.bias + C + j + i));
-              const float4 rs = row_ok ? __ldg(reinterpret_cast<const float4*>(p.res + (size_t)m_row * C + j + i))
-                                       : make_float4(0.f, 0.f, 0.f, 0.f);
-              gb[ci][i] = fmaf(a[i], sc, ba.x) * sigmoid_fast(fmaf(b[i], sc, bb.x)) + rs.x;
-              gb[ci][i + 1] = fmaf(a[i + 1], sc, ba.y) * sigmoid_fast(fmaf(b[i + 1], sc, bb.y)) + rs.y;
-              gb[ci][i + 2] = fmaf(a[i + 2], sc, ba.z) * sigmoid_fast(fmaf(b[i + 2], sc, bb.z)) + rs.z;
-              gb[ci][i + 3] = fmaf(a[i + 3], sc, ba.w) * sigmoid_fast(fmaf(b[i + 3], sc, bb.w)) + rs.w;
-              psum += (gb[ci][i] + gb[ci][i + 1]) + (gb[ci][i + 2] + gb[ci][i + 3]);
-            }
-          }
-        }
-        ln_part2[0][lane_grp][sub][lane] = psum;
-        asm volatile("bar.sync %0, 128;" ::"r"(bar_id) : "memory");
-        const float mu = ((ln_part2[0][lane_grp][0][lane] + ln_part2[0][lane_grp][1][lane]) +
-                          (ln_part2[0][lane_grp][2][lane] + ln_part2[0][lane_grp][3][lane])) / (float)C;
-        float pvar = 0.f;
-#pragma unroll
-        for (int ci = 0; ci < 4; ++ci)
-          if (sub * 16 + ci * 64 < C) {
-#pragma unroll
-            for (int i = 0; i < 16; ++i) pvar = fmaf(gb[ci][i] - mu, gb[ci][i] - mu, pvar);
-          }
-        ln_part2[1][lane_grp][sub][lane] = pvar;
-        asm volatile("bar.sync %0, 128;" ::"r"(bar_id) : "memory");
-        const float rs_ = rsqrtf(((ln_part2[1][lane_grp][0][lane] + ln_part2[1][lane_grp][1][lane]) +
-                                  (ln_part2[1][lane_grp][2][lane] + ln_part2[1][lane_grp][3][lane])) / (float)C + 1e-5f);
-        if (tracing && threadIdx.x == 64) p.trace[6] = clock64();
-#pragma unroll
-        for (int ci = 0; ci < 4; ++ci) {
-          const int j = sub * 16 + ci * 64;
-          if (j < C) {
-#pragma unroll
-            for (int i = 0; i < 16; i += 4) {
-              const float4 ga = __ldg(reinterpret_cast<const float4*>(p.gamma + j + i));
-              const float4 be = __ldg(reinterpret_cast<const float4*>(p.beta + j + i));
-              *reinterpret_cast<float4*>(slab + lane * pitch + j + i) =
-                  make_float4(fmaf((gb[ci][i] - mu) * rs_, ga.x, be.x), fmaf((gb[ci][i + 1] - mu) * rs_, ga.y, be.y),
-                              fmaf((gb[ci][i + 2] - mu) * rs_, ga.z, be.z), fmaf((gb[ci][i + 3] - mu) * rs_, ga.w, be.w));
-            }
-          }
-        }
-        asm volatile("bar.sync %0, 128;" ::"r"(bar_id) : "memory");
-        if (tracing && threadIdx.x == 64) p.trace[7] = clock64();
-        normalized = true;
-#pragma unroll
-        for (int rr = 0; rr < 8; ++rr) {
-          mean[rr] = 0.f;
-          rstd[rr] = 1.f;
-        }
       }
       if (tracing && threadIdx.x == 64) p.trace[8] = clock64();
-#pragma unroll
-      for (int v = 0; v < NV; ++v) {
-        const int c4 = v * 128 + lane * 4;
-        if (v >= nv || c4 >= C) {
-          if (F16 && p.chain && v < nv && c4 < ((C + 63) & ~63)) {
-#pragma unroll
-            for (int rr = 0; rr < 8; ++rr) {
-              const int R = lane_grp * 32 + sub * 8 + rr;
-              uint8_t* t = smem + p.a3_offset + (size_t)(c4 >> 6) * 2 * A_TILE_BYTES + R * 128 + ((((c4 & 63) >> 3) ^ (R & 7)) << 4) +
-                           ((c4 & 7) << 1);
+      const bool with_pos = (p.out_mask & OUT_HILO_POS) || (p.chain && p.pos);
+      const int upr = C >> 2;
+      if (F16 && p.chain) {
+        const int pad4 = (((C + 63) & ~63) - C) >> 2;
+        for (int u = lane; u < RPW * pad4; u += 32) {
+          const int rr = u / pad4, c4 = C + (u - rr * pad4) * 4;
+          const int R = lane_grp * 32 + sub * RPW + rr;
+          uint8_t* t = smem + p.a3_offset + (size_t)(c4 >> 6) * 2 * A_TILE_BYTES + R * 128 + ((((c4 & 63) >> 3) ^ (R & 7)) << 4) +
+                       ((c4 & 7) << 1);
+          *reinterpret_cast<uint2*>(t) = make_uint2(0u, 0u);
+          *reinterpret_cast<uint2*>(t + A_TILE_BYTES) = make_uint2(0u, 0u);
+        }
+      }
+      for (int u = lane; u < RPW * upr; u += 32) {
+        const int rr = u / upr, c4 = (u - rr * upr) * 4;
+        const int r = sub * RPW + rr, m = slab_row0 + r;
+        if (m >= p.M) {
+          if (p.chain) {
+            const int R = lane_grp * 32 + r;
+            if (F16) {
+              uint8_t* t = smem + p.a3_offset + (size_t)(c4 >> 6) * 2 * A_TILE_BYTES + R * 128 +
+                           ((((c4 & 63) >> 3) ^ (R & 7)) << 4) + ((c4 & 7) << 1);
               *reinterpret_cast<uint2*>(t) = make_uint2(0u, 0u);
               *reinterpret_cast<uint2*>(t + A_TILE_BYTES) = make_uint2(0u, 0u);
-            }
-          }
-          continue;
-        }
-        const float4 ga = __ldg(reinterpret_cast<const float4*>(p.gamma + c4));
-        const float4 be = __ldg(reinterpret_cast<const float4*>(p.beta + c4));
-        const float gs[4] = {ga.x, ga.y, ga.z, ga.w}, bs[4] = {be.x, be.y, be.z, be.w};
-#pragma unroll
-        for (int rr = 0; rr < 8; ++rr) {
-          const int m = slab_row0 + sub * 8 + rr;
-          if (m >= p.M) {
-            if (p.chain) {
-              const int R = lane_grp * 32 + sub * 8 + rr;
-              if (F16) {
-                uint8_t* t = smem + p.a3_offset + (size_t)(c4 >> 6) * 2 * A_TILE_BYTES + R * 128 +
-                             ((((c4 & 63) >> 3) ^ (R & 7)) << 4) + ((c4 & 7) << 1);
-                *reinterpret_cast<uint2*>(t) = make_uint2(0u, 0u);
-                *reinterpret_cast<uint2*>(t + A_TILE_BYTES) = make_uint2(0u, 0u);
-              } else {
-                const int kb = c4 >> 5, chunk = (c4 & 31) >> 2;
-                uint8_t* t = smem + p.a3_offset + (size_t)kb * 2 * A_TILE_BYTES + R * 128 + ((chunk ^ (R & 7)) << 4);
-                *reinterpret_cast<float4*>(t) = make_float4(0.f, 0.f, 0.f, 0.f);
-                *reinterpret_cast<float4*>(t + A_TILE_BYTES) = make_float4(0.f, 0.f, 0.f, 0.f);
-              }
-            }
-            continue;
-          }
-          float y[4];
-          if (NV == 1) {
-#pragma unroll
-            for (int i = 0; i < 4; ++i) y[i] = normalized ? g[rr][v][i] : (g[rr][v][i] - mean[rr]) * rstd[rr] * gs[i] + bs[i];
-          } else {
-            const float4 gv = *reinterpret_cast<const float4*>(slab + (sub * 8 + rr) * pitch + c4);
-            float4 ps = make_float4(0.f, 0.f, 0.f, 0.f);
-            if ((p.out_mask & OUT_HILO_POS) || (p.chain && p.pos))
-              ps = __ldg(reinterpret_cast<const float4*>(p.pos + (size_t)(m % p.HW) * C + c4));
-            y[0] = gv.x; y[1] = gv.y; y[2] = gv.z; y[3] = gv.w;
-            pe[rr][v][0] = ps.x; pe[rr][v][1] = ps.y; pe[rr][v][2] = ps.z; pe[rr][v][3] = ps.w;
-          }
-          const size_t o = (size_t)m * C + c4;
-          if (p.out_mask & OUT_F32) *reinterpret_cast<float4*>(out_f32 + o) = make_float4(y[0], y[1], y[2], y[3]);
-          if (p.out_mask & (OUT_HILO | OUT_HILO_POS)) {
-            float t[4];
-#pragma unroll
-            for (int i = 0; i < 4; ++i) t[i] = y[i] + pe[rr][v][i];
-            store_hilo4<F16>(p.out_hi, p.out_lo, o, t);
-          }
-          if (p.out_mask & OUT_HILO_CELU) {
-            const size_t o2 = (size_t)m * 2 * C + c4;
-            float t[4], t2[4];
-#pragma unroll
-            for (int i = 0; i < 4; ++i) {
-              t[i] = elu1(y[i]);
-              t2[i] = elu1(-y[i]);
-            }
-            store_hilo4<F16>(p.out_hi, p.out_lo, o2, t);
-            store_hilo4<F16>(p.out_hi, p.out_lo, o2 + C, t2);
-          }
-          if (p.chain) {
-            const int R = lane_grp * 32 + sub * 8 + rr;
-            if (F16) {
-              unsigned short h[4], l[4];
-#pragma unroll
-              for (int i = 0; i < 4; ++i) split_f16(y[i] + pe[rr][v][i], h[i], l[i]);
-              uint8_t* t = smem + p.a3_offset + (size_t)(c4 >> 6) * 2 * A_TILE_BYTES + R * 128 +
-                           ((((c4 & 63) >> 3) ^ (R & 7)) << 4) + ((c4 & 7) << 1);
-              *reinterpret_cast<uint2*>(t) = make_uint2((uint32_t)h[0] | ((uint32_t)h[1] << 16), (uint32_t)h[2] | ((uint32_t)h[3] << 16));
-              *reinterpret_cast<uint2*>(t + A_TILE_BYTES) =
-                  make_uint2((uint32_t)l[0] | ((uint32_t)l[1] << 16), (uint32_t)l[2] | ((uint32_t)l[3] << 16));
             } else {
               const int kb = c4 >> 5, chunk = (c4 & 31) >> 2;
-              float h[4], l[4];
-#pragma unroll
-              for (int i = 0; i < 4; ++i) split_tf32(y[i] + pe[rr][v][i], h[i], l[i]);
               uint8_t* t = smem + p.a3_offset + (size_t)kb * 2 * A_TILE_BYTES + R * 128 + ((chunk ^ (R & 7)) << 4);
-              *reinterpret_cast<float4*>(t) = make_float4(h[0], h[1], h[2], h[3]);
-              *reinterpret_cast<float4*>(t + A_TILE_BYTES) = make_float4(l[0], l[1], l[2], l[3]);
+              *reinterpret_cast<float4*>(t) = make_float4(0.f, 0.f, 0.f, 0.f);
+              *reinterpret_cast<float4*>(t + A_TILE_BYTES) = make_float4(0.f, 0.f, 0.f, 0.f);
             }
+          }
+          continue;
+        }
+        const float4 gv = *reinterpret_cast<const float4*>(slab + r * pitch + c4);
+        const float y[4] = {gv.x, gv.y, gv.z, gv.w};
+        float pe[4] = {0.f, 0.f, 0.f, 0.f};
+        if (with_pos) {
+          const float4 ps = __ldg(reinterpret_cast<const float4*>(p.pos + (size_t)(m % p.HW) * C + c4));
+          pe[0] = ps.x; pe[1] = ps.y; pe[2] = ps.z; pe[3] = ps.w;
+        }
+        const size_t o = (size_t)m * C + c4;
+        if (p.out_mask & OUT_F32) *reinterpret_cast<float4*>(out_f32 + o) = gv;
+        if (p.out_mask & (OUT_HILO | OUT_HILO_POS)) {
+          float t[4];
+#pragma unroll
+          for (int i = 0; i < 4; ++i) t[i] = y[i] + pe[i];
+          store_hilo4<F16>(p.out_hi, p.out_lo, o, t);
+        }
+        if (p.out_mask & OUT_HILO_CELU) {
+          const size_t o2 = (size_t)m * 2 * C + c4;
+          float t[4], t2[4];
+#pragma unroll
+          for (int i = 0; i < 4; ++i) {
+            t[i] = elu1(y[i]);
+            t2[i] = elu1(-y[i]);
+          }
+          store_hilo4<F16>(p.out_hi, p.out_lo, o2, t);
+          store_hilo4<F16>(p.out_hi, p.out_lo, o2 + C, t2);
+        }
+        if (p.chain) {
+          const int R = lane_grp * 32 + r;
+          if (F16) {
+            unsigned short h[4], l[4];
+#pragma unroll
+            for (int i = 0; i < 4; ++i) split_f16(y[i] + pe[i], h[i], l[i]);
+            uint8_t* t = smem + p.a3_offset + (size_t)(c4 >> 6) * 2 * A_TILE_BYTES + R * 128 +
+                         ((((c4 & 63) >> 3) ^ (R & 7)) << 4) + ((c4 & 7) << 1);
+            *reinterpret_cast<uint2*>(t) = make_uint2((uint32_t)h[0] | ((uint32_t)h[1] << 16), (uint32_t)h[2] | ((uint32_t)h[3] << 16));
+            *reinterpret_cast<uint2*>(t + A_TILE_BYTES) =
+                make_uint2((uint32_t)l[0] | ((uint32_t)l[1] << 16), (uint32_t)l[2] | ((uint32_t)l[3] << 16));
+          } else {
+            const int kb = c4 >> 5, chunk = (c4 & 31) >> 2;
+            float h[4], l[4];
+#pragma unroll
+            for (int i = 0; i < 4; ++i) split_tf32(y[i] + pe[i], h[i], l[i]);
+            uint8_t* t = smem + p.a3_offset + (size_t)kb * 2 * A_TILE_BYTES + R * 128 + ((chunk ^ (R & 7)) << 4);
+            *reinterpret_cast<float4*>(t) = make_float4(h[0], h[1], h[2], h[3]);
+            *reinterpret_cast<float4*>(t + A_TILE_BYTES) = make_float4(l[0], l[1], l[2], l[3]);
           }
         }
       }
@@ -807,7 +712,7 @@
         const int n2 = p.n2, pitch2 = n2 + 4;
         const float sc2 = F16 ? p.acc_scale2 : 1.f;
         float* slab2 = reinterpret_cast<float*>(smem) + lane_grp * (32 * pitch2);
-        for (int j = sub * 16; j < n2; j += 16 * (EPI_WARPS / 4)) {
+        for (int j = sub * 16; j < n2; j += 16 * SUBS) {
           float v16[16];
           tmem_ld16(trow + p.N + j, v16);
 #pragma unroll
@@ -815,11 +720,11 @@
             *reinterpret_cast<float4*>(slab2 + lane * pitch2 + j + i) =
                 make_float4(v16[i] * sc2, v16[i + 1] * sc2, v16[i + 2] * sc2, v16[i + 3] * sc2);
         }
-        asm volatile("bar.sync %0, 128;" ::"r"(bar_id) : "memory");
+        asm volatile("bar.sync %0, %1;" ::"r"(bar_id), "n"(32 * SUBS) : "memory");
         for (int c4 = lane * 4; c4 < n2; c4 += 128) {
 #pragma unroll
-          for (int rr = 0; rr < 8; ++rr) {
-            const int r = sub * 8 + rr, m = slab_row0 + r;
+          for (int rr = 0; rr < RPW; ++rr) {
+            const int r = sub * RPW + rr, m = slab_row0 + r;
             if (m >= p.M) break;
             *reinterpret_cast<float4*>(p.out2_f32 + (size_t)m * n2 + c4) = *reinterpret_cast<const float4*>(slab2 + r * pitch2 + c4);
           }
@@ -962,21 +867,70 @@
 using namespace flowk;
 using namespace flowk::tc;
 
-static int conv_gemm_impl(const flowk_conv_gemm_args* a, flowk_stream_t stream, int* plan_only);
+using GemmKernel = void (*)(CUtensorMap, CUtensorMap, CUtensorMap, CUtensorMap, CUtensorMap, CUtensorMap, Params);
+
+struct GemmPlan {
+  int ksplit;
+  GemmKernel kernel;
+  int threads, tmem_cols;
+  size_t smem_bytes;
+};
+
+static bool g_shared_sm = true;
+
+extern "C" void flowk_conv_gemm_set_shared_sm(int enable) { g_shared_sm = enable != 0; }
+
+static int conv_gemm_impl(const flowk_conv_gemm_args* a, flowk_stream_t stream, GemmPlan* plan, bool assume_ws);
 
 extern "C" int flowk_conv_gemm(const flowk_conv_gemm_args* a, flowk_stream_t stream) {
-  return conv_gemm_impl(a, stream, nullptr);
+  return conv_gemm_impl(a, stream, nullptr, false);
 }
 
 extern "C" int flowk_conv_gemm_splitk_slices(const flowk_conv_gemm_args* a) {
-  int ks = 1;
-  const int st = conv_gemm_impl(a, nullptr, &ks);
-  return st == FLOWK_OK ? ks : 1;
-}
-
-static int conv_gemm_impl(const flowk_conv_gemm_args* a, flowk_stream_t stream, int* plan_only) {
+  GemmPlan pl{};
+  const int st = conv_gemm_impl(a, nullptr, &pl, true);
+  return st == FLOWK_OK ? pl.ksplit : 1;
+}
+
+extern "C" int flowk_conv_gemm_footprint(const flowk_conv_gemm_args* a, flowk_sm_footprint* f) {
+  if (!f) return FLOWK_ERR_ARG;
+  GemmPlan pl{};
+  const int st = conv_gemm_impl(a, nullptr, &pl, false);
+  if (st != FLOWK_OK) return st;
+  return sm_footprint(reinterpret_cast<const void*>(pl.kernel), pl.threads, pl.smem_bytes, pl.tmem_cols, f);
+}
+
+static GemmKernel gemm_kernel(int pre, bool f16, bool pair, bool shared) {
+  if (shared) return pre == PRE_GLU_RES_LN ? conv_gemm_kernel<PRE_GLU_RES_LN, true, false, SHARED_EPI_WARPS>
+                                           : conv_gemm_kernel<PRE_BIAS, true, false, SHARED_EPI_WARPS>;
+  if (pre == PRE_LSTM) return f16 ? conv_gemm_kernel<PRE_LSTM, true> : conv_gemm_kernel<PRE_LSTM, false>;
+  if (pre == PRE_GLU_RES_LN) return f16 ? conv_gemm_kernel<PRE_GLU_RES_LN, true> : conv_gemm_kernel<PRE_GLU_RES_LN, false>;
+  if (pair) return conv_gemm_kernel<PRE_BIAS, true, true>;
+  return f16 ? conv_gemm_kernel<PRE_BIAS, true> : conv_gemm_kernel<PRE_BIAS, false>;
+}
+
+static cudaError_t gemm_smem_optin(GemmKernel k, size_t smem, bool shared) {
+  static GemmKernel keys[16];
+  static size_t set[16];
+  static int n = 0;
+  int i = 0;
+  while (i < n && keys[i] != k) ++i;
+  if (i == n) {
+    if (n == 16) return cudaErrorInvalidValue;
+    keys[n++] = k;
+    set[i] = 0;
+  }
+  if (smem <= set[i]) return cudaSuccess;
+  cudaError_t e = cudaFuncSetAttribute(k, cudaFuncAttributeMaxDynamicSharedMemorySize, (int)smem);
+  if (e == cudaSuccess && shared)
+    e = cudaFuncSetAttribute(k, cudaFuncAttributePreferredSharedMemoryCarveout, (int)cudaSharedmemCarveoutMaxShared);
+  if (e == cudaSuccess) set[i] = smem;
+  return e;
+}
+
+static int conv_gemm_impl(const flowk_conv_gemm_args* a, flowk_stream_t stream, GemmPlan* plan, bool assume_ws) {
   if (!a) return FLOWK_ERR_ARG;
-  if (!plan_only && (!a->a_hi || !a->a_lo || !a->w_hi || !a->w_lo)) return FLOWK_ERR_ARG;
+  if (!plan && (!a->a_hi || !a->a_lo || !a->w_hi || !a->w_lo)) return FLOWK_ERR_ARG;
   const int B = a->B, H = a->H, W = a->W, Cin = a->Cin, N = a->N;
   const bool f16 = a->operand_format == FLOWK_OPERAND_F16;
   if (a->operand_format != FLOWK_OPERAND_TF32 && !f16) return FLOWK_ERR_ARG;
@@ -987,7 +941,7 @@
   if (a->taps != 1 && a->taps != 9 && a->taps != 25) return FLOWK_ERR_ARG;
   const int dil = a->dilation > 0 ? a->dilation : 1;
   if (a->pre != PRE_BIAS && a->pre != PRE_GLU_RES_LN && a->pre != PRE_LSTM) return FLOWK_ERR_ARG;
-  if (!plan_only && !encode_fn()) return FLOWK_ERR_ARG;
+  if (!plan && !encode_fn()) return FLOWK_ERR_ARG;
   int wt = W, ht, bt;
   if (W > BLOCK_M || BLOCK_M % W) return FLOWK_ERR_SHAPE;
   if (H * W >= BLOCK_M) {
@@ -1070,12 +1024,8 @@
   if (p.n_chunk % 16 || p.n_chunk > 256) return FLOWK_ERR_SHAPE;
   p.ksplit = 1;
   if (a->pre == PRE_BIAS && p.n_chunks == 1 && (a->out_mask == OUT_NCHW || a->out_mask == OUT_F32) && !(N & 3) &&
-      (plan_only || a->splitk_ws))
+      (assume_ws || a->splitk_ws))
     p.ksplit = plan_ksplit((B * H * W + BLOCK_M - 1) / BLOCK_M, n_tiles, p.kblocks_per_tap, a->taps);
-  if (plan_only) {
-    *plan_only = p.ksplit;
-    return FLOWK_OK;
-  }
   if (p.ksplit > 1) {
     p.out_mask = OUT_F32;
     p.out_f32 = a->splitk_ws;
@@ -1088,10 +1038,6 @@
   int stages = (int)((220 * 1024 - 2048) / stage_bytes);
   if (stages > 6) stages = 6;
   if (stages < 1) return FLOWK_ERR_SHAPE;
-  static int smem_cap_kb = -1;
-  if (smem_cap_kb < 0) { const char* e = getenv("FLOWK_GEMM_SMEM_CAP_KB"); smem_cap_kb = e ? atoi(e) : 0; }
-  if (smem_cap_kb > 0 && p.tmem_cols <= 256)
-    while (stages > 1 && (size_t)stages * stage_bytes > (size_t)smem_cap_kb * 1024) --stages;
   p.dxsplit = (a->taps == 9 && dil == 1 && a->pre == PRE_BIAS && W <= 32 && 32 % W == 0 && p.n_chunks == 1 &&
                3 * p.n_chunk <= 512 && p.ksplit == 1) ? 1 : 0;
   p.pair = 0;
@@ -1157,9 +1103,47 @@
     p.tmem_cols = 512;
     p.chain = 1;
   }
+  bool shared = false;
+  if (g_shared_sm && f16 && !p.chain && !p.pair && p.ksplit == 1 && p.tmem_cols <= 256 &&
+      (a->pre == PRE_BIAS || (a->pre == PRE_GLU_RES_LN && N / 2 <= 128)) && epi_bytes <= (size_t)SHARED_REGION_BYTES) {
+    size_t ring = 0;
+    int sh_stages = 0, sh_a = 0, sh_w = 0;
+    if (p.dxsplit) {
+      const int w_slot_bytes = 6 * cols * ROW_BYTES;
+      sh_a = 2;
+      sh_w = (SHARED_REGION_BYTES - sh_a * 2 * A_TILE_BYTES) / w_slot_bytes;
+      if (sh_w < 2) {
+        sh_a = 1;
+        sh_w = (SHARED_REGION_BYTES - sh_a * 2 * A_TILE_BYTES) / w_slot_bytes;
+      }
+      if (sh_w > 4) sh_w = 4;
+      if (sh_w >= 1) ring = (size_t)sh_a * 2 * A_TILE_BYTES + (size_t)sh_w * w_slot_bytes;
+    } else {
+      sh_stages = SHARED_REGION_BYTES / stage_bytes;
+      if (sh_stages > 6) sh_stages = 6;
+      if (sh_stages >= 2 || (sh_stages == 1 && p.taps * p.kblocks_per_tap <= 4)) ring = (size_t)sh_stages * stage_bytes;
+    }
+    if (ring) {
+      shared = true;
+      if (!p.dxsplit) stages = sh_stages;
+      p.a_slots = sh_a;
+      p.w_slots = sh_w;
+      region = ring > epi_bytes ? ring : (epi_bytes + 1023) / 1024 * 1024;
+    }
+  }
   p.stages = stages;
   p.bar_offset = (int)region;
   const size_t smem_bytes = region + 1024 + 256;
+  const GemmKernel kernel = gemm_kernel(a->pre, f16, p.pair, shared);
+  const int threads = gemm_threads(shared ? SHARED_EPI_WARPS : EPI_WARPS);
+  if (plan) {
+    plan->ksplit = p.ksplit;
+    plan->kernel = kernel;
+    plan->threads = threads;
+    plan->tmem_cols = p.tmem_cols;
+    plan->smem_bytes = smem_bytes;
+    return FLOWK_OK;
+  }
 
   alignas(64) CUtensorMap ma_hi, ma_lo, mw_hi, mw_lo, mw2_hi, mw2_lo;
   const int Ktot = a->taps * p.kblocks_per_tap * bk;
@@ -1177,29 +1161,9 @@
   }
 
   dim3 grid((p.M + BLOCK_M - 1) / BLOCK_M, n_tiles, p.ksplit);
-#define FLOWK_LAUNCH_GEMM(PRE_, NV_, F16_, PAIR_)                                                                         \
-  do {                                                                                                              \
-    static size_t smem_set = 0;                                                                                     \
-    if (smem_bytes > smem_set) {                                                                                    \
-      FLOWK_CUDA_OK(cudaFuncSetAttribute(conv_gemm_kernel<PRE_, NV_, F16_, PAIR_>, cudaFuncAttributeMaxDynamicSharedMemorySize, \
-                                         (int)smem_bytes));                                                         \
-      smem_set = smem_bytes;                                                                                        \
-    }                                                                                                               \
-    FLOWK_CUDA_OK(launch_pdl_cluster(conv_gemm_kernel<PRE_, NV_, F16_, PAIR_>, grid, dim3(NUM_THREADS), smem_bytes, stream,          \
-                                     PAIR_ ? 2 : 1, ma_hi, ma_lo, mw_hi, mw_lo, mw2_hi, mw2_lo, p));               \
-  } while (0)
-  if (a->pre == PRE_LSTM) {
-    if (f16) FLOWK_LAUNCH_GEMM(PRE_LSTM, 1, true, false); else FLOWK_LAUNCH_GEMM(PRE_LSTM, 1, false, false);
-  } else if (a->pre == PRE_GLU_RES_LN && N / 2 > 128) {
-    if (f16) FLOWK_LAUNCH_GEMM(PRE_GLU_RES_LN, 2, true, false); else FLOWK_LAUNCH_GEMM(PRE_GLU_RES_LN, 2, false, false);
-  } else if (a->pre == PRE_GLU_RES_LN) {
-    if (f16) FLOWK_LAUNCH_GEMM(PRE_GLU_RES_LN, 1, true, false); else FLOWK_LAUNCH_GEMM(PRE_GLU_RES_LN, 1, false, false);
-  } else if (p.pair) {
-    FLOWK_LAUNCH_GEMM(PRE_BIAS, 1, true, true);
-  } else {
-    if (f16) FLOWK_LAUNCH_GEMM(PRE_BIAS, 1, true, false); else FLOWK_LAUNCH_GEMM(PRE_BIAS, 1, false, false);
-  }
-#undef FLOWK_LAUNCH_GEMM
+  FLOWK_CUDA_OK(gemm_smem_optin(kernel, smem_bytes, shared));
+  FLOWK_CUDA_OK(launch_pdl_cluster(kernel, grid, dim3(threads), smem_bytes, stream, p.pair ? 2 : 1, ma_hi, ma_lo, mw_hi,
+                                   mw_lo, mw2_hi, mw2_lo, p));
   if (p.ksplit > 1) {
     FLOWK_CUDA_OK(launch_pdl(splitk_reduce_kernel, dim3((p.M + 31) / 32, (N + 31) / 32), dim3(256), 0, stream, (const float*)a->splitk_ws, a->bias,
                              a->out_mask == OUT_F32 ? a->out_f32 : (float*)nullptr,
@@ -1292,11 +1256,11 @@
   do {                                                                                                                  \
     static size_t smem_set = 0;                                                                                         \
     if (smem_bytes > smem_set) {                                                                                        \
-      FLOWK_CUDA_OK(cudaFuncSetAttribute(conv_gemm_kernel<PRE_, 1, true, false>,                                        \
+      FLOWK_CUDA_OK(cudaFuncSetAttribute(conv_gemm_kernel<PRE_, true, false>,                                        \
                                          cudaFuncAttributeMaxDynamicSharedMemorySize, (int)smem_bytes));                \
       smem_set = smem_bytes;                                                                                            \
     }                                                                                                                   \
-    FLOWK_CUDA_OK(launch_pdl_cluster(conv_gemm_kernel<PRE_, 1, true, false>, grid, dim3(NUM_THREADS), smem_bytes,       \
+    FLOWK_CUDA_OK(launch_pdl_cluster(conv_gemm_kernel<PRE_, true, false>, grid, dim3(gemm_threads(EPI_WARPS)), smem_bytes,       \
                                      stream, 1, ma_hi, ma_lo, mw_hi, mw_lo, mw_hi, mw_lo, p));                          \
   } while (0)
   if (mode == FLOWK_MAR_EMBED) FLOWK_LAUNCH_MAR(PRE_MAR_EMBED);
diff --git a/gaussian-processes-after-pre-processing-with-normalising-flows-2_b200/tc.py b/gaussian-processes-after-pre-processing-with-normalising-flows-2_b200/tc.py
--- a/gaussian-processes-after-pre-processing-with-normalising-flows-2_b200/tc.py
+++ b/gaussian-processes-after-pre-processing-with-normalising-flows-2_b200/tc.py
@@ -65,11 +65,42 @@
     return None if t is None else t.data_ptr()
 
 
+GEMM_SHARED_SM = __import__("os").environ.get("FLOWK_GEMM_SHARED_SM", "1") != "0"
+_shared_sm_set = None
+
+
+def _sync_shared_sm():
+    global _shared_sm_set
+    if _shared_sm_set != GEMM_SHARED_SM:
+        _lib.lib.flowk_conv_gemm_set_shared_sm(int(GEMM_SHARED_SM))
+        _shared_sm_set = GEMM_SHARED_SM
+
+
+def conv_gemm_args(B, H, W, Cin, N, taps, pre, out_mask, f16=True, **ptrs):
+    a = _lib.ConvGemmArgs()
+    a.a_hi = a.a_lo = a.w_hi = a.w_lo = 16
+    for k, v in ptrs.items():
+        setattr(a, k, v)
+    a.B, a.H, a.W, a.Cin, a.N, a.taps, a.pre, a.out_mask = B, H, W, Cin, N, taps, pre, out_mask
+    a.operand_format = _lib.OPERAND_F16 if f16 else _lib.OPERAND_TF32
+    a.acc_scale = a.acc_scale2 = 1.0
+    a.dilation = 1
+    return a
+
+
+def conv_gemm_footprint(args):
+    _sync_shared_sm()
+    f = _lib.SmFootprint()
+    _lib.check(_lib.lib.flowk_conv_gemm_footprint(ctypes.addressof(args), ctypes.addressof(f)))
+    return f
+
+
 def conv_gemm(a_hi, a_lo, w_hi, w_lo, B, H, W, Cin, N, taps, pre, out_mask, bias=None, res=None, gamma=None,
               beta=None, pos=None, out_f32=None, out_hi=None, out_lo=None, out_nchw=None, status=None, trace=None,
               w2_hi=None, w2_lo=None, out2_f32=None, n2=0, split_k=False, acc_scale=None, dilation=1, acc_scale2=None,
               acc_scale_ptr=None):
     _lib.check_device(a_hi, "conv_gemm")
+    _sync_shared_sm()
     args = _lib.ConvGemmArgs(_p(a_hi), _p(a_lo), _p(w_hi), _p(w_lo), _p(bias), _p(res), _p(gamma), _p(beta), _p(pos),
                              _p(out_f32), _p(out_hi), _p(out_lo), _p(out_nchw), _p(status), _p(trace),
                              B, H, W, Cin, N, taps, pre, out_mask, _p(w2_hi), _p(w2_lo), _p(out2_f32), n2, None,
diff --git a/include/flowk.h b/include/flowk.h
--- a/include/flowk.h
+++ b/include/flowk.h
@@ -97,6 +97,16 @@
 int flowk_conv_gemm(const flowk_conv_gemm_args* args, flowk_stream_t stream);
 int flowk_conv_gemm_splitk_slices(const flowk_conv_gemm_args* args);
 
+typedef struct flowk_sm_footprint {
+  int threads;
+  int regs_per_thread;
+  int smem_bytes;
+  int tmem_cols;
+  int blocks_per_sm;
+} flowk_sm_footprint;
+int flowk_conv_gemm_footprint(const flowk_conv_gemm_args* args, flowk_sm_footprint* fp);
+void flowk_conv_gemm_set_shared_sm(int enable);
+
 enum { FLOWK_MAR_EMBED = 0, FLOWK_MAR_LSTM = 1, FLOWK_MAR_SAMPLE = 2 };
 typedef struct flowk_mar_step_args {
   const void* a_hi;
@@ -229,6 +239,7 @@
                               void* out_hi, void* out_lo, int B, int HW, int C, int heads, int* status, long long* trace,
                               flowk_stream_t stream);
 int flowk_attention_inproj_tc_occupancy(int HW, int C, int heads, int* blocks_per_sm, int* smem_bytes);
+int flowk_attention_tc_footprint(int kernel, int HW, int C, int heads, flowk_sm_footprint* fp);
 
 #ifdef __cplusplus
 }
diff --git a/profiles/coresidency_probe.py b/profiles/coresidency_probe.py
--- /dev/null
+++ b/profiles/coresidency_probe.py
@@ -0,0 +1,107 @@
+import os
+import subprocess
+import sys
+
+import torch
+
+sys.path.insert(0, os.path.dirname(os.path.dirname(os.path.abspath(__file__))))
+import flowk
+from flowk import tc
+
+REPS = 50
+
+
+def card():
+    try:
+        return subprocess.run(["nvidia-smi", "--query-gpu=name,power.limit,clocks.max.sm,clocks.sm",
+                               "--format=csv,noheader", "-i", "0"], capture_output=True, text=True,
+                              timeout=60).stdout.strip()
+    except (OSError, subprocess.SubprocessError):
+        return "unknown"
+
+
+def lane(dev, B, H, W, C, seed):
+    g = torch.Generator(device="cpu").manual_seed(seed)
+    M = B * H * W
+    a = torch.randn(M, C, generator=g).to(dev)
+    w = (torch.randn(2 * C, C, 1, 1, generator=g) / C ** 0.5).to(dev)
+    a_hi, a_lo = tc.split_rows_f16(a)
+    w_hi, w_lo, sc = tc.conv_weight_operand_f16(w)
+    kw = dict(bias=torch.randn(2 * C, generator=g).to(dev), res=torch.randn(M, C, generator=g).to(dev),
+              gamma=torch.ones(C, device=dev), beta=torch.zeros(C, device=dev), out_f32=torch.empty(M, C, device=dev),
+              out_hi=torch.empty(M, 2 * C, device=dev, dtype=torch.float16),
+              out_lo=torch.empty(M, 2 * C, device=dev, dtype=torch.float16), acc_scale=sc)
+    return lambda: tc.conv_gemm(a_hi, a_lo, w_hi, w_lo, B, H, W, C, 2 * C, 1, tc.PRE_GLU_RES_LN,
+                                tc.OUT_F32 | tc.OUT_HILO_CELU, **kw)
+
+
+def capture(fn, stream):
+    graph = torch.cuda.CUDAGraph()
+    with torch.cuda.stream(stream):
+        fn()
+        torch.cuda.synchronize()
+        with torch.cuda.graph(graph, stream=stream):
+            for _ in range(REPS):
+                fn()
+    return graph
+
+
+def timed(graphs, streams):
+    main = torch.cuda.current_stream()
+    start, end = torch.cuda.Event(enable_timing=True), torch.cuda.Event(enable_timing=True)
+    start.record(main)
+    done = []
+    for graph, s in zip(graphs, streams):
+        s.wait_event(start)
+        with torch.cuda.stream(s):
+            graph.replay()
+            ev = torch.cuda.Event()
+            ev.record(s)
+            done.append(ev)
+    for ev in done:
+        main.wait_event(ev)
+    end.record(main)
+    torch.cuda.synchronize()
+    return start.elapsed_time(end) * 1e3 / REPS
+
+
+def main():
+    out_path = sys.argv[1] if len(sys.argv) > 1 else None
+    rounds = int(sys.argv[2]) if len(sys.argv) > 2 else 5
+    dev = torch.device("cuda:0")
+    B, H, W, C = 64, 16, 16, 96
+    lines = ["device: " + card(), "cfg2 level-1 attention gate 1x1 %d -> %d + GLU + res + LN, B = %d (%d CTAs), %d launches "
+             "per graph" % (C, 2 * C, B, B * H * W // 128, REPS)]
+    s1, s2 = torch.cuda.Stream(), torch.cuda.Stream()
+    runs = {}
+    for shared in (False, True):
+        tc.GEMM_SHARED_SM = shared
+        fp = tc.conv_gemm_footprint(tc.conv_gemm_args(B, H, W, C, 2 * C, 1, tc.PRE_GLU_RES_LN, tc.OUT_F32 | tc.OUT_HILO_CELU,
+                                                      bias=16, res=16, gamma=16, beta=16, out_f32=16, out_hi=16,
+                                                      out_lo=16))
+        lines.append("%-9s threads %d, %d registers, %d B shared memory, %d TMEM columns, %d CTAs per SM" % (
+            "shared" if shared else "exclusive", fp.threads, fp.regs_per_thread, fp.smem_bytes, fp.tmem_cols,
+            fp.blocks_per_sm))
+        g1 = capture(lane(dev, B, H, W, C, 1), s1)
+        g2 = capture(lane(dev, B, H, W, C, 2), s2)
+        runs[shared] = (g1, g2, [], [])
+    for _ in range(rounds):
+        for shared in (False, True):
+            g1, g2, one, two = runs[shared]
+            one.append(timed([g1], [s1]))
+            two.append(timed([g1, g2], [s1, s2]))
+    for shared in (False, True):
+        _, _, one, two = runs[shared]
+        o, t = sorted(one)[len(one) // 2], sorted(two)[len(two) // 2]
+        lines.append("%-9s one stream %6.2f us/launch (%.2f-%.2f)  two streams %6.2f us per launch pair (%.2f-%.2f)  "
+                     "ratio %.2f" % ("shared" if shared else "exclusive", o, min(one), max(one), t, min(two), max(two),
+                                     t / o))
+    text = "\n".join(lines)
+    print(text)
+    if out_path:
+        with open(out_path, "w") as f:
+            f.write(text + "\n")
+
+
+if __name__ == "__main__":
+    main()
```
